# thomasdeppisch/eMagLS

Hardware: AMD Instinct MI355X
Metric: eMagLS filter sets/s (N=4, 2702 dirs, 512 taps) (higher is better)
Workload: dtype f64; 1 GPU; BASELINE config 3: getEMagLsFilters em32 r=4.2cm N=4 complex-SH, 2702 dirs, 512 taps, 48 kHz; one filter set per step, inputs resident in HBM; dirs=2702, taps=512, sim_order=19, bins=512, k_cut=43, designs_resident_per_gpu=128, designs_per_batch=32, batches_in_flight=4, distinct_hrir_sets_resident=20, parallelism=independent jobs per GPU, one RCCL gather

## Files before the change

emagls_amd/_lib.py:

```python
from __future__ import annotations

import ctypes as C
import os

_HERE = os.path.dirname(os.path.abspath(__file__))
LIB_PATH = os.environ.get("EMAGLS_LIB_PATH") or os.path.join(_HERE, "lib", "libemagls.so")

OK, ERR_ARG, ERR_UNSUPPORTED, ERR_HIP, ERR_NUMERIC = 0, 1, 2, 3, 4
BASIS = {"real": 0, "complex": 1}
KIND_LS, KIND_MAGLS, KIND_EMAGLS, KIND_EMAGLS2, KIND_FROM_ATF, KIND_EMA_CH, KIND_MAGLS_2D, KIND_EMA_SH = range(8)
RADIAL = {"tikhonov": 0, "softlimit": 1, "full": 2, "none": 3}
LAYOUT = {"sh": 0, "ch": 1}
MODEL = {"sh": 0, "emagls": 1, "emagls2": 2, "atf": 3, "ema_ch": 5, "ema_sh": 6}

c_dp = C.POINTER(C.c_double)
c_i64 = C.c_int64


class DesignDesc(C.Structure):
    _fields_ = [("kind", C.c_int), ("basis", C.c_int), ("order", C.c_int), ("fs", C.c_double), ("len", c_i64),
                ("nsamp", c_i64), ("ndirs", c_i64), ("mic_radius", C.c_double), ("nmics", c_i64),
                ("f_trans", C.c_double), ("atf_taps", c_i64), ("natf", c_i64), ("custom_basis", C.c_int),
                ("diffuseness", C.c_int), ("sim_order_pad", C.c_int)]

# ... 112 lines not shown
    "emagls_binaural_decode_render_fs_device": (C.c_int, [C.c_void_p, C.c_int, c_i64, c_i64, C.c_void_p, C.c_void_p, C.c_int, c_i64,
                                                          C.c_int, C.c_int, C.c_void_p, c_i64, C.c_void_p, c_i64, C.c_void_p, c_i64,
                                                          C.c_void_p, c_i64, C.c_double, C.c_double, C.c_double, C.c_void_p,
                                                          C.c_void_p, C.c_void_p]),
    "emagls_decode_stream_create": (C.c_int, [c_i64, C.c_void_p, C.c_void_p, C.c_int, c_i64, C.c_int, C.c_int, C.c_int, c_i64,
                                              C.POINTER(C.c_void_p)]),
    "emagls_decode_stream_push": (C.c_int, [C.c_void_p, C.c_void_p, c_i64, C.c_void_p, c_i64, C.c_void_p, c_i64, C.c_void_p, c_i64,
                                            C.c_void_p]),
    "emagls_decode_stream_push_device": (C.c_int, [C.c_void_p, C.c_void_p, c_i64, C.c_void_p, c_i64, C.c_void_p, c_i64, C.c_void_p, c_i64,
                                                   C.c_void_p, C.c_void_p]),
    "emagls_decode_stream_reset": (C.c_int, [C.c_void_p]),
    "emagls_decode_stream_info": (C.c_int, [C.c_void_p, C.POINTER(c_i64), C.POINTER(c_i64), C.POINTER(c_i64), C.POINTER(c_i64),
                                            C.POINTER(C.c_int)]),
    "emagls_decode_stream_destroy": (C.c_int, [C.c_void_p]),
    "emagls_decode_stream_create_bank": (C.c_int, [c_i64, c_i64, C.c_void_p, C.c_void_p, C.c_int, c_i64, C.c_int, C.c_int, C.c_int, c_i64,
                                                   C.POINTER(C.c_void_p)]),
    "emagls_decode_stream_push_sets": (C.c_int, [C.c_void_p, C.c_void_p, c_i64, C.c_void_p, c_i64, C.c_void_p, c_i64, C.c_void_p, c_i64,
                                                 C.c_void_p, c_i64, C.c_void_p]),
    "emagls_decode_stream_push_sets_device": (C.c_int, [C.c_void_p, C.c_void_p, c_i64, C.c_void_p, c_i64, C.c_void_p, c_i64, C.c_void_p,
                                                        c_i64, C.c_void_p, c_i64, C.c_void_p, C.c_void_p]),
    "emagls_decode_stream_sets": (C.c_int, [C.c_void_p, C.POINTER(c_i64)]),
    "emagls_decode_group_create": (C.c_int, [c_i64, c_i64, C.c_void_p, C.c_void_p, C.c_int, c_i64, C.c_int, C.c_int, C.c_int, c_i64, c_i64,
                                             C.POINTER(C.c_void_p)]),
    "emagls_decode_group_push": (C.c_int, [C.c_void_p, C.c_void_p, c_i64, C.c_void_p, c_i64, C.c_void_p, c_i64, C.c_void_p, c_i64,
                                           C.c_void_p, c_i64, C.c_void_p]),
    "emagls_decode_group_push_device": (C.c_int, [C.c_void_p, C.c_void_p, c_i64, C.c_void_p, c_i64, C.c_void_p, c_i64, C.c_void_p, c_i64,
                                                  C.c_void_p, c_i64, C.c_void_p, C.c_void_p]),
    "emagls_decode_group_reset": (C.c_int, [C.c_void_p, c_i64]),
    "emagls_decode_group_info": (C.c_int, [C.c_void_p, C.POINTER(c_i64), C.POINTER(c_i64), C.POINTER(c_i64), C.POINTER(c_i64),
                                           C.POINTER(c_i64), C.POINTER(C.c_int)]),
    "emagls_decode_group_destroy": (C.c_int, [C.c_void_p]),
    "emagls_decode_stream_create_encoded": (C.c_int, [c_i64, C.c_void_p, C.c_int, c_i64, c_i64, C.c_void_p, C.c_void_p, C.c_int, c_i64, C.c_int,
                                                      C.c_int, c_i64, C.POINTER(C.c_void_p)]),
    "emagls_decode_group_create_encoded": (C.c_int, [c_i64, C.c_void_p, C.c_int, c_i64, c_i64, C.c_void_p, C.c_void_p, C.c_int, c_i64, C.c_int,
                                                     C.c_int, c_i64, c_i64, C.POINTER(C.c_void_p)]),
    "emagls_field_stream_create": (C.c_int, [c_i64, c_i64, C.c_void_p, C.c_int, c_i64, c_i64, C.POINTER(C.c_void_p)]),
    "emagls_field_stream_push": (C.c_int, [C.c_void_p, C.c_void_p, c_i64, C.c_void_p]),
    "emagls_field_stream_push_device": (C.c_int, [C.c_void_p, C.c_void_p, c_i64, C.c_void_p, C.c_void_p]),
    "emagls_field_stream_reset": (C.c_int, [C.c_void_p]),
    "emagls_field_stream_info": (C.c_int, [C.c_void_p, C.POINTER(c_i64), C.POINTER(c_i64), C.POINTER(c_i64), C.POINTER(c_i64),
                                           C.POINTER(C.c_int)]),
    "emagls_field_stream_destroy": (C.c_int, [C.c_void_p]),
    "emagls_field_stream_create_bank": (C.c_int, [c_i64, c_i64, c_i64, C.c_void_p, C.c_int, c_i64, c_i64, C.POINTER(C.c_void_p)]),
    "emagls_field_stream_push_sets": (C.c_int, [C.c_void_p, C.c_void_p, c_i64, C.c_void_p, c_i64, C.c_void_p]),
    "emagls_field_stream_push_sets_device": (C.c_int, [C.c_void_p, C.c_void_p, c_i64, C.c_void_p, c_i64, C.c_void_p, C.c_void_p]),
    "emagls_field_stream_sets": (C.c_int, [C.c_void_p, C.POINTER(c_i64)]),
    "emagls_get_magls_filters_dc": (C.c_int, [C.c_void_p, C.c_void_p, c_i64, c_i64, C.c_void_p, C.c_void_p, C.c_int,
                                              C.c_double, c_i64, C.c_int, C.c_int, C.c_void_p, C.c_void_p]),
    "emagls_get_emagls_filters_dc": (C.c_int, [C.c_void_p, C.c_void_p, c_i64, c_i64, C.c_void_p, C.c_void_p, C.c_double,
                                               C.c_void_p, C.c_void_p, c_i64, C.c_int, C.c_double, c_i64, C.c_int, C.c_int,
                                               C.c_void_p, C.c_void_p]),
    "emagls_get_emagls2_filters_dc": (C.c_int, [C.c_void_p, C.c_void_p, c_i64, c_i64, C.c_void_p, C.c_void_p, C.c_double,
                                                C.c_void_p, C.c_void_p, c_i64, C.c_int, C.c_double, c_i64, C.c_int, C.c_int,
                                                C.c_void_p, C.c_void_p]),
    "emagls_get_magls_filters_2d": (C.c_int, [C.c_void_p, C.c_void_p, c_i64, c_i64, C.c_void_p, C.c_int, C.c_double, c_i64, C.c_int,
                                              C.c_void_p, C.c_void_p]),
    "emagls_get_radial_filter": (C.c_int, [C.c_int, C.c_double, C.c_double, c_i64, C.c_int, C.c_int, C.c_double, C.c_double, C.c_void_p]),
    "emagls_apply_radial_filter_rows": (c_i64, [c_i64, c_i64, C.c_int]),
    "emagls_apply_radial_filter": (C.c_int, [C.c_void_p, c_i64, C.c_int, C.c_double, C.c_double, c_i64, C.c_int, C.c_int, C.c_double,
                                             C.c_double, C.c_void_p]),
    "emagls_sh_encode": (C.c_int, [C.c_void_p, c_i64, c_i64, C.c_void_p, C.c_void_p, C.c_int, C.c_int, C.c_void_p]),
    "emagls_ch_basis": (C.c_int, [C.c_int, c_i64, C.c_void_p, C.c_int, C.c_void_p]),
    "emagls_get_smair_matrix": (C.c_int, [C.c_int, C.c_double, c_i64, C.c_int, C.c_double, C.c_void_p, C.c_void_p, c_i64, C.c_int, C.c_int,
                                          C.c_int, C.c_double, C.c_double, C.c_void_p, C.POINTER(C.c_int)]),
    "emagls_rendered_hrtfs": (C.c_int, [C.c_int, C.c_void_p, C.c_void_p, C.c_int, c_i64, c_i64, c_i64, C.c_void_p, C.c_void_p, c_i64, C.c_double,
                                        C.c_int, C.c_int, C.c_double, C.c_void_p, C.c_void_p, c_i64, C.c_void_p, c_i64, c_i64, C.c_void_p,
                                        C.c_void_p, c_i64, c_i64, C.c_void_p, C.c_void_p, C.c_void_p, C.c_void_p, C.c_void_p, C.c_void_p]),
    "emagls_array_irs": (C.c_int, [C.c_double, C.c_double, C.c_int, C.c_void_p, C.c_void_p, c_i64, C.c_void_p, C.c_int, c_i64, c_i64, C.c_void_p,
                                   C.c_void_p, C.c_void_p, C.c_void_p, C.c_void_p, C.c_double, c_i64, c_i64, C.c_void_p]),
    "emagls_array_irs_kernel_time": (C.c_int, [C.POINTER(C.c_double)]),
    "emagls_shoebox_components": (C.c_int, [C.c_void_p, C.c_void_p, C.c_void_p, c_i64, C.c_void_p, C.c_double, C.c_double, C.c_int, c_i64,
                                            C.c_void_p, C.c_void_p, C.c_void_p, C.c_void_p, C.c_void_p]),
    "emagls_array_room_irs": (C.c_int, [C.c_double, C.c_double, C.c_int, C.c_void_p, C.c_void_p, c_i64, C.c_void_p, C.c_int, c_i64, C.c_void_p,
                                        C.c_void_p, C.c_void_p, c_i64, C.c_void_p, C.c_double, C.c_int, C.c_double, c_i64, c_i64, C.c_void_p,
                                        C.c_void_p]),
    "emagls_shoebox_kernel_time": (C.c_int, [C.POINTER(C.c_double)]),
    "emagls_array_irs_spectral": (C.c_int, [C.c_double, C.c_double, C.c_int, C.c_void_p, C.c_void_p, c_i64, C.c_void_p, C.c_int, c_i64, c_i64,
                                            C.c_void_p, C.c_void_p, C.c_void_p, C.c_void_p, C.c_void_p, c_i64, C.c_void_p, C.c_void_p, C.c_void_p,
                                            C.c_void_p, C.c_double, c_i64, c_i64, C.c_void_p]),
    "emagls_shoebox_images": (C.c_int, [C.c_void_p, C.c_void_p, c_i64, C.c_void_p, C.c_double, C.c_double, C.c_int, c_i64, C.c_void_p,
                                        C.c_void_p, C.c_void_p, C.c_void_p, C.c_void_p, C.c_void_p, C.c_void_p]),
    "emagls_array_room_irs_spectral": (C.c_int, [C.c_double, C.c_double, C.c_int, C.c_void_p, C.c_void_p, c_i64, C.c_void_p, C.c_int, c_i64,
                                                 C.c_void_p, C.c_void_p, C.c_void_p, C.c_void_p, c_i64, C.c_void_p, C.c_double, C.c_int, C.c_double,
                                                 c_i64, c_i64, C.c_void_p, C.c_void_p]),
    "emagls_array_irs_point": (C.c_int, [C.c_double, C.c_double, C.c_int, C.c_void_p, C.c_void_p, c_i64, C.c_void_p, C.c_int, c_i64, c_i64,
                                         C.c_void_p, C.c_void_p, C.c_void_p, C.c_void_p, C.c_void_p, c_i64, C.c_void_p, C.c_void_p, C.c_void_p,
                                         C.c_void_p, C.c_void_p, C.c_double, c_i64, c_i64, C.c_void_p]),
    "emagls_shoebox_components_dist": (C.c_int, [C.c_void_p, C.c_void_p, C.c_void_p, c_i64, C.c_void_p, C.c_double, C.c_double, C.c_int, c_i64,
                                                 C.c_void_p, C.c_void_p, C.c_void_p, C.c_void_p, C.c_void_p, C.c_void_p]),
    "emagls_array_room_irs_point": (C.c_int, [C.c_double, C.c_double, C.c_int, C.c_void_p, C.c_void_p, c_i64, C.c_void_p, C.c_int, c_i64,
                                              C.c_void_p, C.c_void_p, C.c_int, C.c_void_p, C.c_void_p, c_i64, C.c_void_p, C.c_double, C.c_int,
                                              C.c_double, c_i64, c_i64, C.c_void_p, C.c_void_p]),
    "emagls_array_irs_directive": (C.c_int, [C.c_double, C.c_double, C.c_int, C.c_void_p, C.c_void_p, c_i64, C.c_void_p, C.c_int, c_i64, c_i64,
                                             C.c_void_p, C.c_void_p, C.c_void_p, C.c_void_p, C.c_void_p, c_i64, C.c_void_p, C.c_void_p, C.c_void_p,
                                             C.c_void_p, C.c_void_p, C.c_void_p, C.c_void_p, C.c_int, C.c_void_p, C.c_double, c_i64, c_i64,
                                             C.c_void_p]),
    "emagls_shoebox_emission": (C.c_int, [C.c_void_p, C.c_void_p, C.c_void_p, c_i64, C.c_void_p, C.c_double, C.c_double, C.c_int, c_i64,
                                          C.c_void_p, C.c_void_p]),
    "emagls_array_room_irs_directive": (C.c_int, [C.c_double, C.c_double, C.c_int, C.c_void_p, C.c_void_p, c_i64, C.c_void_p, C.c_int, c_i64,
                                                  C.c_void_p, C.c_void_p, C.c_int, C.c_void_p, C.c_void_p, c_i64, C.c_void_p, C.c_double, C.c_int,
                                                  C.c_int, C.c_void_p, C.c_int, C.c_void_p, C.c_double, c_i64, c_i64, C.c_void_p, C.c_void_p]),
    "emagls_eq_filter_nfft": (c_i64, [c_i64]),
    "emagls_get_magls_spherical_head_filter": (C.c_int, [C.c_double, C.c_int, C.c_double, c_i64, C.c_void_p, C.c_void_p]),
    "emagls_get_magls_array_diffuse_filter": (C.c_int, [C.c_double, C.c_void_p, C.c_void_p, c_i64, C.c_int, C.c_double, c_i64, C.c_int,
                                                        C.c_void_p, C.c_void_p]),
    "emagls_plan_create": (C.c_int, [C.POINTER(DesignDesc), C.POINTER(C.c_void_p)]),
    "emagls_plan_destroy": (C.c_int, [C.c_void_p]),
    "emagls_plan_set_hrir_grid": (C.c_int, [C.c_void_p, C.c_void_p, C.c_void_p]),
    "emagls_plan_set_mic_grid": (C.c_int, [C.c_void_p, C.c_void_p, C.c_void_p]),
    "emagls_plan_set_hrirs": (C.c_int, [C.c_void_p, C.c_void_p, C.c_void_p]),
    "emagls_plan_set_atfs": (C.c_int, [C.c_void_p, C.c_void_p, C.c_void_p, C.c_void_p]),
    "emagls_plan_execute": (C.c_int, [C.c_void_p]),
    "emagls_plan_synchronize": (C.c_int, [C.c_void_p]),
    "emagls_plan_get_filters": (C.c_int, [C.c_void_p, C.c_void_p, C.c_void_p]),
    "emagls_plan_get_info": (C.c_int, [C.c_void_p, C.POINTER(PlanInfo)]),
    "emagls_plan_sweep_form_in_batch": (C.c_int, [C.c_void_p, C.c_int, C.POINTER(C.c_int)]),
    "emagls_plan_set_profiling": (C.c_int, [C.c_void_p, C.c_int]),
    "emagls_plan_set_streams": (C.c_int, [C.c_void_p, C.c_int]),
    "emagls_plan_num_stages": (C.c_int, [C.c_void_p]),
    "emagls_plan_stage_name": (C.c_char_p, [C.c_void_p, C.c_int]),
    "emagls_plan_stage_times": (C.c_int, [C.c_void_p, c_dp, C.c_int]),
    "emagls_plan_sweep_kernel_time": (C.c_int, [C.c_void_p, c_dp, C.POINTER(C.c_int)]),
    "emagls_plan_debug_buffer": (C.c_int, [C.c_void_p, C.c_char_p, C.c_void_p, C.POINTER(C.c_size_t)]),
    "emagls_plan_stream": (C.c_void_p, [C.c_void_p]),
    "emagls_batch_create": (C.c_int, [C.POINTER(C.c_void_p), C.c_int, C.POINTER(C.c_void_p)]),
    "emagls_batch_execute": (C.c_int, [C.c_void_p]),
    "emagls_batch_synchronize": (C.c_int, [C.c_void_p]),
    "emagls_batch_get_filters": (C.c_int, [C.c_void_p, C.POINTER(C.c_void_p), C.POINTER(C.c_void_p)]),
    "emagls_batch_set_profiling": (C.c_int, [C.c_void_p, C.c_int]),
    "emagls_batch_lane_mode": (C.c_int, [C.c_void_p, C.POINTER(C.c_int)]),
    "emagls_batch_set_stream": (C.c_int, [C.c_void_p, C.c_void_p]),
    "emagls_set_batch_max": (C.c_int, [C.c_int, C.POINTER(C.c_int)]),
    "emagls_batch_shares_atf_side": (C.c_int, [C.c_void_p, C.POINTER(C.c_int)]),
    "emagls_design_hrir_sets": (C.c_int, [C.c_int, C.c_void_p, C.c_void_p, C.c_int64, C.c_int64, C.c_int64, C.c_void_p, C.c_void_p, C.c_double,
                                          C.c_void_p, C.c_void_p, C.c_int64, C.c_int, C.c_double, C.c_int64, C.c_int, C.c_void_p, C.c_void_p]),
    "emagls_from_atf_hrir_sets": (C.c_int, [C.c_void_p, C.c_void_p, C.c_int64, C.c_int64, C.c_int64, C.c_void_p, C.c_void_p, C.c_void_p, C.c_int64,
                                            C.c_int64, C.c_int64, C.c_void_p, C.c_void_p, C.c_double, C.c_int64, C.c_double, C.c_void_p, C.c_void_p,
                                            C.POINTER(C.c_double)]),
    "emagls_jobs_run": (C.c_int, [C.POINTER(Job), C.c_int64, C.c_int, C.c_int, C.c_int]),
    "emagls_design_out_shape": (C.c_int, [C.POINTER(DesignDesc), C.POINTER(c_i64), C.POINTER(c_i64), C.POINTER(C.c_int)]),
    "emagls_jobs_shard": (C.c_int, [C.POINTER(Job), C.c_int64, C.c_int, C.c_int, C.POINTER(C.c_int), C.POINTER(C.c_int), C.POINTER(C.c_int)]),
    "emagls_jobs_run_devices": (C.c_int, [C.POINTER(Job), C.c_int64, C.POINTER(C.c_int), C.c_int, C.c_int, C.c_int, C.c_int]),
    "emagls_jobs_set_profiling": (C.c_int, [C.c_int]),
    "emagls_jobs_sweep_times": (C.c_int, [C.POINTER(C.c_double), C.POINTER(C.c_int), C.c_int, C.POINTER(C.c_int)]),
    "emagls_batch_set_geometry_sharing": (C.c_int, [C.c_void_p, C.c_int]),
    "emagls_batch_shares_geometry": (C.c_int, [C.c_void_p, C.POINTER(C.c_int)]),
    "emagls_batch_geometry_runs": (C.c_int, [C.c_void_p, C.POINTER(C.c_longlong), C.POINTER(C.c_longlong)]),
    "emagls_jobs_geometry_runs": (C.c_int, [C.POINTER(C.c_longlong), C.POINTER(C.c_longlong), C.POINTER(C.c_longlong)]),
    "emagls_jobs_would_share_geometry": (C.c_int, [C.c_void_p, C.c_int, C.POINTER(C.c_int)]),
    "emagls_batch_set_side_stream": (C.c_int, [C.c_void_p, C.c_void_p]),
    "emagls_batch_set_streams": (C.c_int, [C.c_void_p, C.c_int]),
    "emagls_batch_set_stage_order": (C.c_int, [C.c_void_p, C.c_int]),
    "emagls_batch_sweep_time": (C.c_int, [C.c_void_p, C.POINTER(C.c_double)]),
    "emagls_batch_destroy": (C.c_int, [C.c_void_p]),
}


class EmaglsError(RuntimeError):
    def __init__(self, code, msg):
        super().__init__("emagls error %d: %s" % (code, msg))
        self.code = code


_lib = None


def load():
    global _lib
    if _lib is not None:
        return _lib
    if not os.path.exists(LIB_PATH):
        raise ImportError("HIP library not built: %s is missing (run `python -m emagls_amd.build`)" % LIB_PATH)
    lib = C.CDLL(LIB_PATH, mode=C.RTLD_GLOBAL)
    for name, (res, args) in SYMBOLS.items():
        fn = getattr(lib, name)
        fn.restype = res
        fn.argtypes = args
    _lib = lib
    return lib


def check(rc):
    if rc != OK:
        raise EmaglsError(rc, load().emagls_last_error().decode("utf-8", "replace"))
```

emagls_amd/csrc/batch_run.hip:

```cpp
#include "host_internal.hpp"

void emagls_batch_forget(emagls_batch* b, emagls_plan* p) {
    for (auto& q : b->plans) if (q == p) q = nullptr;
}

namespace {
void batch_sweep_stage(emagls_batch& b) {
    const int nb = (int)b.plans.size();
    std::vector<HalfSweepArgs> ha((size_t)nb);
    for (int j = 0; j < nb; ++j) ha[j] = emagls_half_args(*b.plans[j]);
    if (b.atf_share || b.geo_share)
        for (int j = 1; j < nb; ++j) {
            ha[j].G = ha[0].G; ha[j].Yri = ha[0].Yri; ha[j].Mw = ha[0].Mw; ha[j].cond_ok = ha[0].cond_ok;
            ha[j].bsc = ha[0].bsc; ha[j].smap = ha[0].smap;
            ha[j].skip_flag = ha[0].skip_flag;
        }
    const bool reg = b.plans[0]->sweep_persist && reg_sweep_wanted(b.plans.data(), nb);
    for (auto* q : b.plans) q->reg_sweep = reg;
    if (!reg && nb > SWEEP_MULTI_MAX) throw Error(EMAGLS_ERR_UNSUPPORTED, "internal: more than 16 designs in a batch need the register-resident sweep");
    HalfSweepMulti h{};
    h.n = std::min(nb, SWEEP_MULTI_MAX);
    for (int j = 0; j < h.n; ++j) h.a[j] = ha[j];
    emagls_plan& q0 = *b.plans[0];
    const int kk0 = std::max(q0.kcut0, 1);
    if (kk0 >= q0.P) return;
    if (q0.sweep_persist) {
        hipStream_t ss = b.stream;
        {
            SweepGate gate(ss, reg ? reg_sweep_gate_cost((int)q0.D, nb) : 0);
            if (b.lanes) { BatchScope sc(nb, b.stride); launch_zero(q0.get("ll"), q0.bufs["ll"].bytes, ss); }
            else for (auto* q : b.plans) launch_zero(q->get("ll"), q->bufs["ll"].bytes, ss);
            if (reg) {
                if (!b.sweep_args_dev.get()) b.sweep_args_dev.alloc(sizeof(HalfSweepArgs) * (size_t)REG_SWEEP_MAX);
                reg_args_upload(ha.data(), nb, b.sweep_args_dev.get(), b.sweep_args_last, ss);
            }
            if (b.prof_level >= 1) HIP_CHECK(hipEventRecord(b.sweep_ev[0], ss));
            if (reg) launch_sweep_reg(b.sweep_args_dev.get<const HalfSweepArgs>(), ha[0], nb, ss);
            else if (q0.synth) launch_sweep_synth(h, ss); else launch_sweep_persist(h, ss);
            if (b.prof_level >= 1) HIP_CHECK(hipEventRecord(b.sweep_ev[1], ss));
        }
        if (ss != b.stream) b.depend(b.stream, ss);
        return;
    }
    for (int kb = kk0; kb < q0.P; ++kb) launch_sweep_half(h, kb, b.stream);
    launch_sweep_half_finalize(h, q0.P - 1, b.stream);
}

bool batch_defers_hh(const emagls_batch& b) {
    if (!b.lanes || !(b.alone || sw_int<Sw::DEFER_HH>() == 2) || b.geo_share || b.atf_share) return false;
    for (const emagls_plan* p : b.plans) if (!p || !plan_defers_hh_route(*p)) return false;
    return true;
}
void batch_lanes_part(emagls_batch& b, int part, int first, int count, hipStream_t st, int group = 0) {
    emagls_plan& p0 = *b.plans[first];
    const int ns = (part == 0 && b.groups == 1) ? b.nstreams : 1;
    int order = 0;
    if (part == 0 && ns == 1 && sw_on<Sw::STAGGER>()) order = b.groups > 1 ? 1 + group % 2 : (b.order_hint ? 1 + (b.order_hint - 1) % 2 : 0);
    Scoped stream(p0.stream, st);
    Scoped nstreams(p0.nstreams, ns);
    Scoped stage_order(p0.stage_order, order);
    Scoped side0(p0.side[0], ns > 1 ? b.side[0] : p0.side[0]), side1(p0.side[1], ns > 1 ? b.side[1] : p0.side[1]),
        side2(p0.side[2], ns > 1 ? b.side[2] : p0.side[2]);
    Scoped pre_phase(p0.pre_phase, part == 3 ? 2 : (part == 0 && b.defer_hh) ? 1 : 0);
    BatchScope sc(count, b.stride);
    if (part == 0) plan_pre_stage(p0); else if (part == 3) emagls_pre_sweep(p0); else emagls_post_sweep(p0);
}
void mark_executed(emagls_batch& b, int launches) {
    for (auto* p : b.plans) { p->executed = true; p->sweep_launches = launches; }
}
int sweep_launch_count(const emagls_plan& p0) { return p0.sweep_persist ? 1 : p0.P - std::max(p0.kcut0, 1); }
int batch_group_first(const emagls_batch& b, int g) { const int n = (int)b.plans.size(), h = (n + b.groups - 1) / b.groups; return std::min(n, g * h); }
void batch_execute_lanes(emagls_batch& b) {
    const bool replay = b.use_graph && b.eager_runs >= 1 && !(b.groups == 1 && b.nstreams > 1);
    const int n = (int)b.plans.size();
    const int ng = b.groups;
    for (int g = 1; g < ng; ++g) if (!b.side[g - 1]) b.side[g - 1] = emagls::pool_stream_take();
    hipStream_t gs[4] = {b.stream, b.stream, b.stream, b.stream};
    for (int g = 1; g < ng; ++g) gs[g] = b.side[g - 1];
    if (!replay || !b.group[0]) b.defer_hh = batch_defers_hh(b);
    const bool defer = b.defer_hh;
    if (defer) for (int g = 0; g < ng; ++g) if (!b.hh_stream[g]) b.hh_stream[g] = emagls::pool_stream_take();
    if (replay && !b.group[0]) {
        for (int g = 0; g < ng; ++g) {
            const int f = batch_group_first(b, g), c = batch_group_first(b, g + 1) - f;
            b.group[g].capture(gs[g], [&] { batch_lanes_part(b, 0, f, c, gs[g], g); });
            if (defer) b.group_hh[g].capture(b.hh_stream[g], [&] { batch_lanes_part(b, 3, f, c, b.hh_stream[g], g); });
        }
        b.post.capture(b.stream, [&] { batch_lanes_part(b, 2, 0, n, b.stream); });
    }
    b.used = 0;
    for (int g = 1; g < ng; ++g) b.depend(gs[g], b.stream);
    if (replay && ng > 1) {
        hipError_t err[4] = {hipSuccess, hipSuccess, hipSuccess, hipSuccess};
        const int dev = b.device;
        std::vector<std::thread> th;
        for (int g = 1; g < ng; ++g)
            th.emplace_back([&, g] { err[g] = hipSetDevice(dev); if (err[g] == hipSuccess) err[g] = hipGraphLaunch(b.group[g].exec, gs[g]); });
        err[0] = hipGraphLaunch(b.group[0].exec, gs[0]);
        for (auto& t : th) t.join();
        for (int g = 0; g < ng; ++g) HIP_CHECK(err[g]);
    } else {
        for (int g = 0; g < ng; ++g) {
            const int f = batch_group_first(b, g), c = batch_group_first(b, g + 1) - f;
            if (replay) b.group[g].launch(gs[g]); else batch_lanes_part(b, 0, f, c, gs[g], g);
        }
    }
    if (defer) for (int g = 0; g < ng; ++g) b.depend(b.hh_stream[g], gs[g]);
    for (int g = 1; g < ng; ++g) b.depend(b.stream, gs[g]);
    batch_sweep_stage(b);
    if (defer) {
        for (int g = 0; g < ng; ++g) {
            const int f = batch_group_first(b, g), c = batch_group_first(b, g + 1) - f;
            if (replay) b.group_hh[g].launch(b.hh_stream[g]); else batch_lanes_part(b, 3, f, c, b.hh_stream[g], g);
            b.depend(b.stream, b.hh_stream[g]);
        }
    }
    if (replay) b.post.launch(b.stream); else batch_lanes_part(b, 2, 0, n, b.stream);
    mark_executed(b, sweep_launch_count(*b.plans[0]));
    if (!replay) ++b.eager_runs;
}

bool batch_inputs_same(emagls_batch& b, std::initializer_list<const char*> names, uint64_t& checked_version, bool& same) {
    uint64_t ver = 0;
    for (auto* p : b.plans) ver = ver * 1000003ull + p->atf_side_version;
    if (ver == checked_version) return same;
    if (!b.cmp_flag.get()) b.cmp_flag.alloc(16);
    HIP_CHECK(hipStreamSynchronize(b.stream));
    HIP_CHECK(hipMemsetAsync(b.cmp_flag.get(), 0, 16, b.stream));
    emagls_plan& p0 = *b.plans[0];
    for (size_t j = 1; j < b.plans.size(); ++j)
        for (const char* name : names) launch_compare_words(p0.get(name), b.plans[j]->get(name), p0.bufs[name].bytes, b.cmp_flag.get<int>(), b.stream);
    int differ = 0;
    HIP_CHECK(hipMemcpyAsync(&differ, b.cmp_flag.get(), sizeof differ, hipMemcpyDeviceToHost, b.stream));
    HIP_CHECK(hipStreamSynchronize(b.stream));
    checked_version = ver;
    return same = differ == 0;
}
void batch_set_sharing(emagls_batch& b, bool& field, bool share) {
    if (share == field) return;
    for (auto* p : b.plans) drop_plan_graphs(*p);
    drop_batch_graphs(b);
    if (&field == &b.geo_share || &field == &b.geo_ls_shared) batch_geo_forget(b);
    field = share;
}
void batch_run_two_graphs(emagls_batch& b, CapturedGraph& pre, void (*stage)(emagls_batch&, int), int pre_part, int launches) {
    const bool replay = b.use_graph && b.eager_runs >= 1;
    if (replay && !pre) pre.capture(b.stream, [&] { stage(b, pre_part); });
    if (replay && !b.post) b.post.capture(b.stream, [&] { stage(b, 2); });
    b.used = 0;
    if (replay) pre.launch(b.stream); else stage(b, pre_part);
    batch_sweep_stage(b);
    if (replay) b.post.launch(b.stream); else stage(b, 2);
    mark_executed(b, launches);
    if (!replay) ++b.eager_runs;
}
template <typename Pre> void batch_run_per_plan(emagls_batch& b, bool replay, Pre pre, void (*post)(emagls_plan&), int launches) {
    emagls_plan& p0 = *b.plans[0];
    if (replay && !p0.pre) {
        for (auto* p : b.plans) p->pre.capture(p->stream, [&] { pre(*p); });
        if (!p0.sweep_persist) b.group[0].capture(b.stream, [&] { batch_sweep_stage(b); });
    }
    b.used = 0;
    for (auto* p : b.plans) b.depend(p->stream, b.stream);
    for (auto* p : b.plans) {
        if (replay) p->pre.launch(p->stream); else pre(*p);
        b.depend(b.stream, p->stream);
    }
    if (b.atf_share)
        for (size_t j = 1; j < b.plans.size(); ++j) from_atf_ls_rows(*b.plans[j], p0, b.stream);
    if (p0.sweep_persist) batch_sweep_stage(b);
    else if (replay) b.group[0].launch(b.stream); else batch_sweep_stage(b);
    for (auto* p : b.plans) {
        b.depend(p->stream, b.stream);
        post(*p);
        b.depend(b.stream, p->stream);
    }
    mark_executed(b, launches);
    if (!replay) ++b.eager_runs;
}

void batch_atf_decide_sharing(emagls_batch& b) {
    const bool same = batch_inputs_same(b, {"atf", "atf_azi", "atf_zen", "hrir_azi", "hrir_zen"}, b.atf_checked_version, b.atf_inputs_same);
    bool routes_ok = true;
    for (auto* p : b.plans) routes_ok = routes_ok && p->gram_from == 1 && p->sweep_persist == b.plans[0]->sweep_persist;
    batch_set_sharing(b, b.atf_share, same && routes_ok && b.plans.size() > 1);
}
void from_atf_subject_pre_stage(emagls_plan& p) {
    subject_reset(p, p.stream);
    from_atf_subject_stage(p);
}
// ... 473 lines not shown
```

emagls_amd/csrc/capi.hip:

```cpp
#include "host_internal.hpp"

namespace {

struct CachedPlan {
    std::unique_ptr<emagls_plan> plan;
    emagls_design_desc desc{};
    int device = 0;
    bool busy = false;
    uint64_t last_use = 0;
};
std::mutex g_cache_mu;
std::vector<CachedPlan> g_cache;
uint64_t g_cache_tick = 0;

int one_shot(const emagls_design_desc& desc, const double* hL, const double* hR, const double* azi, const double* zen,
             const double* mic_azi, const double* mic_zen, const double* atf, const double* atf_azi, const double* atf_zen,
             void* wL, void* wR, double* mean_dev, const void* Y_hrir = nullptr, const void* Y_mic = nullptr) {
    return guarded([&] {
        int dev = 0;
        HIP_CHECK(hipGetDevice(&dev));
        emagls_plan* p = nullptr;
        std::unique_ptr<emagls_plan> fresh;
        bool cached = false;
        {
// ... 473 lines not shown
            if (!array_kind(p->d.kind) && p->d.kind != EMAGLS_KIND_FROM_ATF && !magls_kind(p->d.kind) && p->d.kind != EMAGLS_KIND_LS)
                throw Error(EMAGLS_ERR_UNSUPPORTED, "batches take eMagLS / eMagLS2 / EMAinCH / EMAinSH plans, LS / MagLS / MagLS-2D plans, or FromAtf plans "
                                                    "(subjects of one ATF set)");
            if ((p->d.kind == EMAGLS_KIND_LS) != (plans[0]->d.kind == EMAGLS_KIND_LS) ||
                (p->d.kind == EMAGLS_KIND_LS && (p->cplx_basis != plans[0]->cplx_basis || p->d.order != plans[0]->d.order || p->d.nsamp != plans[0]->d.nsamp)))
                throw Error(EMAGLS_ERR_ARG, "LS plans share a batch only with LS plans of the same order, basis and HRIR length");
            if ((p->d.kind == EMAGLS_KIND_FROM_ATF) != (plans[0]->d.kind == EMAGLS_KIND_FROM_ATF))
                throw Error(EMAGLS_ERR_ARG, "FromAtf plans cannot share a batch with array designs");
            if (magls_kind(p->d.kind) != magls_kind(plans[0]->d.kind) || (magls_kind(p->d.kind) && p->d.kind != plans[0]->d.kind))
                throw Error(EMAGLS_ERR_ARG, "MagLS plans share a batch only with MagLS plans of the same kind");
            if (magls_kind(p->d.kind) && (p->diffuse != plans[0]->diffuse || p->cplx_basis != plans[0]->cplx_basis || p->d.order != plans[0]->d.order))
                throw Error(EMAGLS_ERR_ARG, "all designs of a batch must have the same shape (order, basis, constraint)");
            if (p->wide) throw Error(EMAGLS_ERR_UNSUPPORTED, "designs with more than 32 channels run one at a time");
            if (p->owner) throw Error(EMAGLS_ERR_ARG, "a plan belongs to another batch (destroy that batch first)");
            if (p->device != plans[0]->device) throw Error(EMAGLS_ERR_ARG, "the plans of a batch must live on one device");
            for (int i = 0; i < j; ++i) if (plans[i] == p) throw Error(EMAGLS_ERR_ARG, "the same plan appears twice in the batch");
            const emagls_plan* q = plans[0];
            if (p->P != q->P || p->kcut0 != q->kcut0 || p->C != q->C || p->nWG_dense != q->nWG_dense || p->D != q->D || p->sweep_persist != q->sweep_persist ||
                p->Dm != q->Dm || p->d.natf != q->d.natf || p->d.atf_taps != q->d.atf_taps || p->d.len != q->d.len)
                throw Error(EMAGLS_ERR_ARG, "all designs of a batch must have the same shape (directions, channels, bins, k_cut)");
            b->plans.push_back(p);
        }
        b->device = b->plans[0]->device;
        DeviceGuard dg(b->device);
        b->stream = StreamPool::get().take();
        b->use_graph = !sw_on<Sw::NO_GRAPH>();
        const bool array_batch = b->plans[0]->d.kind != EMAGLS_KIND_FROM_ATF && !magls_kind(b->plans[0]->d.kind) && b->plans[0]->d.kind != EMAGLS_KIND_LS;
        for (auto* p : b->plans) HIP_CHECK(hipStreamSynchronize(p->stream));
        trace_mark("batch create: plans synchronised");
        if (array_batch) batch_unify_synth(*b);
        trace_mark("batch create: sweep form unified");
        batch_decide_residency(*b);
        trace_mark("batch create: residency decided");
        if (nplans > SWEEP_MULTI_MAX && !(b->plans[0]->synth && b->plans[0]->sweep_persist && reg_sweep_wanted(b->plans.data(), nplans)))
            throw Error(EMAGLS_ERR_UNSUPPORTED, "more than 16 designs per batch: only array designs that take the register-resident sweep (built-in SH basis, "
                                                "microphone grids set, at most 18 antipodal pairs + single microphones, a launch the device can hold)");
        for (auto* p : b->plans) {
            p->nstreams = 1;
            p->prof_level = 0;
            p->sync_stream = b->stream;
            p->owner = b.get();
        }
        b->atf = b->plans[0]->d.kind == EMAGLS_KIND_FROM_ATF;
        b->magls = magls_kind(b->plans[0]->d.kind) || b->plans[0]->d.kind == EMAGLS_KIND_LS;
        if (!b->atf && !b->magls) { batch_unify_synth(*b); batch_try_lanes(*b); }
        trace_mark("batch create: lanes tried");
        *batch = b.release();
    });
}
int emagls_batch_execute(emagls_batch* b) {
    return guarded([&] {
        DeviceGuard dg(b ? b->device : -1);
        if (!b) throw Error(EMAGLS_ERR_ARG, "null pointer");
        batch_execute(*b);
    });
}
int emagls_batch_synchronize(emagls_batch* b) {
    return guarded([&] {
        DeviceGuard dg(b ? b->device : -1);
        if (!b) throw Error(EMAGLS_ERR_ARG, "null pointer");
        HIP_CHECK(hipStreamSynchronize(b->stream));
    });
}
int emagls_batch_get_filters(emagls_batch* b, void* const* wL, void* const* wR) {
    return guarded([&] {
        DeviceGuard dg(b ? b->device : -1);
        if (!b || !wL || !wR) throw Error(EMAGLS_ERR_ARG, "null pointer");
        const size_t n = b->plans.size();
        for (size_t j = 0; j < n; ++j) {
            if (!wL[j] || !wR[j]) throw Error(EMAGLS_ERR_ARG, "null pointer");
            if (!b->plans[j]) throw Error(EMAGLS_ERR_ARG, "a plan of this batch has been destroyed");
            if (!b->plans[j]->executed) throw Error(EMAGLS_ERR_ARG, "batch has not been executed");
        }
        emagls_plan& p0 = *b->plans[0];
        const size_t bytes = (p0.out_cplx ? sizeof(cplx) : sizeof(double)) * (size_t)p0.out_rows * p0.out_cols;
        std::vector<int> flags(NFLAG * n, 0);
        for (int attempt = 0; attempt < 3; ++attempt) {
            if (b->lanes)
                HIP_CHECK(hipMemcpy2DAsync(flags.data(), NFLAG * sizeof(int), p0.get("flag"), b->stride, NFLAG * sizeof(int), n,
                                           hipMemcpyDeviceToHost, b->stream));
            else
                for (size_t j = 0; j < n; ++j)
                    HIP_CHECK(hipMemcpyAsync(&flags[NFLAG * j], b->plans[j]->get("flag"), NFLAG * sizeof(int), hipMemcpyDeviceToHost, b->stream));
            bool scattered = false;
            if (b->lanes && n <= 32 && bytes % 16 == 0) {
                bool dev_dst = true;
                for (size_t j = 0; j < n && dev_dst; ++j)
                    for (void* q : {wL[j], wR[j]}) {
                        hipPointerAttribute_t at{};
                        if (hipPointerGetAttributes(&at, q) != hipSuccess) { (void)hipGetLastError(); dev_dst = false; break; }
                        if (at.type != hipMemoryTypeDevice || at.device != b->device || ((uintptr_t)q & 15)) { dev_dst = false; break; }
                    }
                if (dev_dst) {
                    LanePtrs lp{};
                    for (size_t j = 0; j < n; ++j) { lp.p[2 * j] = wL[j]; lp.p[2 * j + 1] = wR[j]; }
                    launch_scatter_lanes(p0.get("wL"), p0.get("wR"), b->stride, bytes, (int)n, lp, b->stream);
                    scattered = true;
                }
            }
            if (!scattered)
                for (size_t j = 0; j < n; ++j) {
                    HIP_CHECK(hipMemcpyAsync(wL[j], b->plans[j]->get("wL"), bytes, hipMemcpyDefault, b->stream));
                    HIP_CHECK(hipMemcpyAsync(wR[j], b->plans[j]->get("wR"), bytes, hipMemcpyDefault, b->stream));
                }
            HIP_CHECK(hipStreamSynchronize(b->stream));
            bool redo = false;
            for (size_t j = 0; j < n; ++j) redo = plan_recover(*b->plans[j], &flags[NFLAG * j], false) || redo;
            if (!redo) break;
            batch_redo(*b, flags);
        }
        for (auto* q : b->plans)
            if (q->persist_suspended) { q->persist_suspended = false; q->sweep_persist = true; }
        for (size_t j = 0; j < n; ++j) throw_fatal_flags(&flags[NFLAG * j]);
        if (b->geo_cold_pending) { b->geo_kept_version = b->geo_ran_version; b->geo_cold_pending = false; }
    });
}
int emagls_batch_geometry_runs(emagls_batch* b, long long* cold, long long* warm) {
    return guarded([&] {
        if (!b || !cold || !warm) throw Error(EMAGLS_ERR_ARG, "null pointer");
        *cold = b->geo_cold_runs;
        *warm = b->geo_warm_runs;
    });
}
int emagls_batch_lane_mode(emagls_batch* b, int* lanes) {
    return guarded([&] {
        DeviceGuard dg(b ? b->device : -1);
        if (!b || !lanes) throw Error(EMAGLS_ERR_ARG, "null pointer");
        *lanes = b->lanes ? 1 : 0;
    });
}
int emagls_set_batch_max(int max_designs, int* previous) {
    return guarded([&] {
        if (max_designs < 1 || max_designs > REG_SWEEP_MAX) throw Error(EMAGLS_ERR_ARG, "a batch holds 1..32 designs (more than 16: array designs on the register-resident sweep)");
        const int prev = g_batch_max.exchange(max_designs);
        if (previous) *previous = prev;
    });
}
int emagls_batch_set_geometry_sharing(emagls_batch* b, int enable) {
    return guarded([&] {
        DeviceGuard dg(b ? b->device : -1);
        if (!b) throw Error(EMAGLS_ERR_ARG, "null pointer");
        HIP_CHECK(hipStreamSynchronize(b->stream));
        b->geo_want = enable != 0;
        b->geo_checked_version = ~0ull;
        batch_geo_forget(*b);
    });
}
int emagls_batch_shares_geometry(emagls_batch* b, int* shared) {
    return guarded([&] {
        if (!b || !shared) throw Error(EMAGLS_ERR_ARG, "null pointer");
        *shared = b->geo_share ? 1 : 0;
    });
}
int emagls_batch_shares_atf_side(emagls_batch* b, int* shared) {
    return guarded([&] {
        if (!b || !shared) throw Error(EMAGLS_ERR_ARG, "null pointer");
        *shared = b->atf_share ? 1 : 0;
    });
}
int emagls_batch_set_stream(emagls_batch* b, void* stream) {
    return guarded([&] {
        DeviceGuard dg(b ? b->device : -1);
        if (!b || !stream) throw Error(EMAGLS_ERR_ARG, "null pointer");
        HIP_CHECK(hipStreamSynchronize(b->stream));
        if (b->own_stream) emagls::pool_stream_give(b->stream);
        b->stream = (hipStream_t)stream;
        b->own_stream = false;
        for (auto* p : b->plans) if (p) p->sync_stream = b->stream;
    });
}
int emagls_batch_set_streams(emagls_batch* b, int nstreams) {
    return guarded([&] {
        DeviceGuard dg(b ? b->device : -1);
        if (!b) throw Error(EMAGLS_ERR_ARG, "null pointer");
        if (nstreams < 1 || nstreams > 4) throw Error(EMAGLS_ERR_ARG, "nstreams must be 1..4");
        HIP_CHECK(hipStreamSynchronize(b->stream));
        for (int i = 0; i < nstreams - 1; ++i) if (!b->side[i]) b->side[i] = emagls::pool_stream_take();
        if (nstreams != b->nstreams) drop_batch_graphs(*b);
        b->nstreams = nstreams;
    });
}
int emagls_batch_set_stage_order(emagls_batch* b, int order) {
    return guarded([&] {
        DeviceGuard dg(b ? b->device : -1);
        if (!b) throw Error(EMAGLS_ERR_ARG, "null pointer");
        if (order < 0 || order > 2) throw Error(EMAGLS_ERR_ARG, "stage order must be 0, 1 or 2");
        HIP_CHECK(hipStreamSynchronize(b->stream));
        if (order != b->order_hint) drop_batch_graphs(*b);
        b->order_hint = order;
    });
}
int emagls_batch_set_side_stream(emagls_batch* b, void* stream) {
    return guarded([&] {
        DeviceGuard dg(b ? b->device : -1);
        if (!b || !stream) throw Error(EMAGLS_ERR_ARG, "null pointer");
        HIP_CHECK(hipStreamSynchronize(b->stream));
        if (b->side[0] && !b->side0_external) { HIP_CHECK(hipStreamSynchronize(b->side[0])); emagls::pool_stream_give(b->side[0]); }
        b->side[0] = (hipStream_t)stream;
        b->side0_external = true;
    });
}
int emagls_batch_set_profiling(emagls_batch* b, int level) {
    return guarded([&] {
        DeviceGuard dg(b ? b->device : -1);
        if (!b) throw Error(EMAGLS_ERR_ARG, "null pointer");
        HIP_CHECK(hipStreamSynchronize(b->stream));
        if (level >= 1)
            for (auto& e : b->sweep_ev) if (!e) HIP_CHECK(hipEventCreate(&e));
        b->prof_level = level;
    });
}
int emagls_batch_sweep_time(emagls_batch* b, double* ms) {
    return guarded([&] {
        DeviceGuard dg(b ? b->device : -1);
        if (!b || !ms) throw Error(EMAGLS_ERR_ARG, "null pointer");
        if (b->prof_level < 1 || !b->sweep_ev[0]) throw Error(EMAGLS_ERR_ARG, "batch profiling is off");
        HIP_CHECK(hipStreamSynchronize(b->stream));
        float t = 0.f;
        HIP_CHECK(hipEventElapsedTime(&t, b->sweep_ev[0], b->sweep_ev[1]));
        *ms = t;
    });
}
int emagls_batch_destroy(emagls_batch* b) {
    return guarded([&] {
        DeviceGuard dg(b ? b->device : -1);
        delete b;
    });
}

int emagls_get_ls_filters(const double* hL, const double* hR, int64_t nsamp, int64_t ndirs, const double* azi,
                          const double* zen, int order, int basis, void* wL, void* wR) {
    emagls_design_desc d{};
    d.kind = EMAGLS_KIND_LS; d.basis = basis; d.order = order; d.nsamp = nsamp; d.ndirs = ndirs;
    return one_shot(d, hL, hR, azi, zen, nullptr, nullptr, nullptr, nullptr, nullptr, wL, wR, nullptr);
}
int emagls_get_magls_filters(const double* hL, const double* hR, int64_t nsamp, int64_t ndirs, const double* azi,
                             const double* zen, int order, double fs, int64_t len, int basis, void* wL, void* wR) {
    emagls_design_desc d{};
    d.kind = EMAGLS_KIND_MAGLS; d.basis = basis; d.order = order; d.fs = fs; d.len = len; d.nsamp = nsamp; d.ndirs = ndirs;
    return one_shot(d, hL, hR, azi, zen, nullptr, nullptr, nullptr, nullptr, nullptr, wL, wR, nullptr);
}
int emagls_get_emagls_filters(const double* hL, const double* hR, int64_t nsamp, int64_t ndirs, const double* azi,
                              const double* zen, double mic_radius, const double* mic_azi, const double* mic_zen,
                              int64_t nmics, int order, double fs, int64_t len, int basis, void* wL, void* wR) {
    emagls_design_desc d{};
    d.kind = EMAGLS_KIND_EMAGLS; d.basis = basis; d.order = order; d.fs = fs; d.len = len; d.nsamp = nsamp; d.ndirs = ndirs;
    d.mic_radius = mic_radius; d.nmics = nmics;
    if (!mic_azi || !mic_zen) { g_last_error = "null microphone grid"; return EMAGLS_ERR_ARG; }
    return one_shot(d, hL, hR, azi, zen, mic_azi, mic_zen, nullptr, nullptr, nullptr, wL, wR, nullptr);
}
int emagls_get_emagls2_filters(const double* hL, const double* hR, int64_t nsamp, int64_t ndirs, const double* azi,
                               const double* zen, double mic_radius, const double* mic_azi, const double* mic_zen,
                               int64_t nmics, int order, double fs, int64_t len, int basis, void* wL, void* wR) {
    emagls_design_desc d{};
    d.kind = EMAGLS_KIND_EMAGLS2; d.basis = basis; d.order = order; d.fs = fs; d.len = len; d.nsamp = nsamp; d.ndirs = ndirs;
    d.mic_radius = mic_radius; d.nmics = nmics;
    if (!mic_azi || !mic_zen) { g_last_error = "null microphone grid"; return EMAGLS_ERR_ARG; }
    return one_shot(d, hL, hR, azi, zen, mic_azi, mic_zen, nullptr, nullptr, nullptr, wL, wR, nullptr);
}
int emagls_get_emagls_filters_ema_in_ch(const double* hL, const double* hR, int64_t nsamp, int64_t ndirs, const double* azi,
                                        const double* zen, double mic_radius, const double* mic_azi, int64_t nmics, int order,
                                        double fs, int64_t len, int basis, void* wL, void* wR) {
    emagls_design_desc d{};
    d.kind = EMAGLS_KIND_EMA_CH; d.basis = basis; d.order = order; d.fs = fs; d.len = len; d.nsamp = nsamp; d.ndirs = ndirs;
    d.mic_radius = mic_radius; d.nmics = nmics;
    if (!mic_azi || nmics < 1) { g_last_error = "invalid array geometry"; return EMAGLS_ERR_ARG; }
    std::vector<double> mic_zen((size_t)nmics, kPi / 2.0);
    return one_shot(d, hL, hR, azi, zen, mic_azi, mic_zen.data(), nullptr, nullptr, nullptr, wL, wR, nullptr);
}
int emagls_get_emagls_filters_ema_in_sh(const double* hL, const double* hR, int64_t nsamp, int64_t ndirs, const double* azi,
                                        const double* zen, double mic_radius, const double* mic_azi, int64_t nmics, int order,
                                        double fs, int64_t len, int basis, void* wL, void* wR) {
    emagls_design_desc d{};
    d.kind = EMAGLS_KIND_EMA_SH; d.basis = basis; d.order = order; d.fs = fs; d.len = len; d.nsamp = nsamp; d.ndirs = ndirs;
    d.mic_radius = mic_radius; d.nmics = nmics;
    if (!mic_azi || nmics < 1) { g_last_error = "invalid array geometry"; return EMAGLS_ERR_ARG; }
    std::vector<double> mic_zen((size_t)nmics, kPi / 2.0);
    return one_shot(d, hL, hR, azi, zen, mic_azi, mic_zen.data(), nullptr, nullptr, nullptr, wL, wR, nullptr);
}
int emagls_get_emagls_filters_from_atf(const double* hL, const double* hR, int64_t nsamp, int64_t ndirs,
                                       const double* azi, const double* zen, const double* atf_irs, int64_t atf_taps,
                                       int64_t nmics, int64_t natf, const double* atf_azi, const double* atf_zen, double fs,
                                       int64_t filter_len, double f_trans, double* wL, double* wR, double* mean_dev) {
    emagls_design_desc d{};
    d.kind = EMAGLS_KIND_FROM_ATF; d.basis = EMAGLS_BASIS_REAL; d.fs = fs; d.len = filter_len; d.nsamp = nsamp; d.ndirs = ndirs;
    d.nmics = nmics; d.f_trans = f_trans; d.atf_taps = atf_taps; d.natf = natf;
    if (!atf_irs || !atf_azi || !atf_zen) { g_last_error = "null ATF set"; return EMAGLS_ERR_ARG; }
    return one_shot(d, hL, hR, azi, zen, nullptr, nullptr, atf_irs, atf_azi, atf_zen, wL, wR, mean_dev);
}

int emagls_get_magls_filters_dc(const double* hL, const double* hR, int64_t nsamp, int64_t ndirs, const double* azi, const double* zen,
                                int order, double fs, int64_t len, int apply_dc, int basis, void* wL, void* wR) {
    emagls_design_desc d{};
    d.kind = EMAGLS_KIND_MAGLS; d.basis = basis; d.order = order; d.fs = fs; d.len = len; d.nsamp = nsamp; d.ndirs = ndirs;
    d.diffuseness = apply_dc != 0;
    return one_shot(d, hL, hR, azi, zen, nullptr, nullptr, nullptr, nullptr, nullptr, wL, wR, nullptr);
}
static int emagls_array_dc(int kind, const double* hL, const double* hR, int64_t nsamp, int64_t ndirs, const double* azi, const double* zen,
                           double mic_radius, const double* mic_azi, const double* mic_zen, int64_t nmics, int order, double fs, int64_t len,
                           int apply_dc, int basis, void* wL, void* wR) {
    emagls_design_desc d{};
    d.kind = kind; d.basis = basis; d.order = order; d.fs = fs; d.len = len; d.nsamp = nsamp; d.ndirs = ndirs;
    d.mic_radius = mic_radius; d.nmics = nmics; d.diffuseness = apply_dc != 0;
    return one_shot(d, hL, hR, azi, zen, mic_azi, mic_zen, nullptr, nullptr, nullptr, wL, wR, nullptr);
}
int emagls_get_emagls_filters_dc(const double* hL, const double* hR, int64_t nsamp, int64_t ndirs, const double* azi, const double* zen,
// ... 74 lines not shown
```

emagls_amd/csrc/host_internal.hpp:

```cpp
#pragma once
#include <atomic>
#include <chrono>
#include <cstdlib>
#include <cstring>
#include <deque>
#include <map>
#include <memory>
#include <mutex>
#include <shared_mutex>
#include <string>
#include <thread>
#include <utility>
#include <vector>

#include "../../include/emagls.h"
#include "array_model.hpp"
#include "device_mem.hpp"
#include "kernels.hpp"

using namespace emagls;

struct emagls_batch;
void emagls_batch_forget(emagls_batch* b, emagls_plan* p);

// ... 208 lines not shown
    bool synth_want = false, synth = false;
    int synth_units = 0;
    bool reg_sweep = false;
    std::vector<char> sweep_args_last;
    bool synth_block = false;
    const emagls_plan* geo_from = nullptr;
    emagls_batch* owner = nullptr;
    bool have_hrir_grid = false, have_mic_grid = false, have_hrirs = false, have_atfs = false, have_basis = false;
    uint64_t atf_side_version = 0;
    bool diffuse = false;
    bool custom_basis = false;
    bool wide = false;
    int prof_level = 0;
    std::vector<std::string> stage_names;
    std::vector<hipEvent_t> stage_events;
    std::vector<double> stage_ms;
    std::vector<hipEvent_t> sweep_events;
    int sweep_launches = 0;
    bool executed = false;
    CapturedGraph graph;
    int eager_runs = 0;
    bool use_graph = true;
    CapturedGraph pre;
    int nstreams = 1;
    int stage_order = 0;
    int pre_phase = 0;
    bool geo_keep = false;
    bool geo_skip = false;
    uint64_t geo_done_version = ~0ull;
    uint64_t geo_run_version = ~0ull;
    uint64_t solo_runs = 0;
    bool defer_hh = false;
    bool alone = false;
    hipStream_t hh_stream = nullptr;
    hipStream_t sync_stream = nullptr;
    hipStream_t side[3] = {nullptr, nullptr, nullptr};
    bool owns_stream = true;
    void need_sides(int n) { for (int i = 0; i < n - 1 && i < 3; ++i) if (!side[i]) side[i] = StreamPool::get().take(); }
    std::vector<hipEvent_t> sync_events;
    size_t sync_used = 0;
    hipEvent_t next_sync_event() {
        if (sync_used == sync_events.size()) {
            hipEvent_t e;
            HIP_CHECK(hipEventCreateWithFlags(&e, hipEventDisableTiming));
            sync_events.push_back(e);
        }
        return sync_events[sync_used++];
    }
    void depend(hipStream_t waiter, hipStream_t signaller) {
        if (waiter == signaller) return;
        hipEvent_t e = next_sync_event();
        HIP_CHECK(hipEventRecord(e, signaller));
        HIP_CHECK(hipStreamWaitEvent(waiter, e, 0));
    }

    ~emagls_plan() {
        if (owner) emagls_batch_forget(owner, this);
        if (stream) hipStreamSynchronize(stream);
        for (auto st : side) if (st) hipStreamSynchronize(st);
        if (hh_stream) hipStreamSynchronize(hh_stream);
        (void)hipGetLastError();
        for (auto& kv : bufs) if (kv.second.p && kv.second.owned) hipFree(kv.second.p);
        release_slabs();
        for (auto e : stage_events) hipEventDestroy(e);
        for (auto e : sweep_events) hipEventDestroy(e);
        for (auto e : sync_events) hipEventDestroy(e);
        for (auto st : side) StreamPool::get().give(st);
        StreamPool::get().give(hh_stream);
        if (owns_stream) StreamPool::get().give(stream);
    }
    void* alloc(const std::string& name, size_t bytes, bool zero = true) {
        if (bytes == 0) bytes = 16;
        auto it = bufs.find(name);
        if (it != bufs.end()) {
            if (it->second.bytes >= bytes) {
                total_bytes -= (int64_t)(it->second.bytes - bytes);
                it->second.bytes = bytes;
                return it->second.p;
            }
            if (it->second.owned) HIP_CHECK(hipFree(it->second.p));
            total_bytes -= (int64_t)it->second.bytes;
        }
        DevBuf b;
        b.p = slab_take((bytes + 15) / 16 * 16);
        b.bytes = bytes;
        b.owned = false;
        if (zero && !slab_zeroed) HIP_CHECK(hipMemsetAsync(b.p, 0, bytes, stream));
        bufs[name] = b;
        total_bytes += (int64_t)bytes;
        return b.p;
    }
    template <typename T = void> T* get(const std::string& name) {
        auto it = bufs.find(name);
        if (it == bufs.end()) throw Error(EMAGLS_ERR_ARG, "internal: unknown buffer " + name);
        return reinterpret_cast<T*>(it->second.p);
    }
    bool has(const std::string& name) const { return bufs.count(name) != 0; }
    void upload(const std::string& name, const void* src, size_t bytes) {
        auto it = bufs.find(name);
        if (it == bufs.end() || it->second.bytes < bytes) throw Error(EMAGLS_ERR_ARG, "internal: upload size mismatch for " + name);
        HIP_CHECK(hipMemcpyAsync(it->second.p, src, bytes, hipMemcpyDefault, stream));
    }
    void mark(const char* name) {
        if (prof_level < 1) return;
        const size_t i = stage_names.size();
        stage_names.push_back(name);
        if (stage_events.size() <= i) {
            hipEvent_t e;
            HIP_CHECK(hipEventCreate(&e));
            stage_events.push_back(e);
        }
        HIP_CHECK(hipEventRecord(stage_events[i], stream));
    }
};

struct emagls_batch {
    std::vector<emagls_plan*> plans;
    int device = -1;
    bool lanes = false;
    size_t stride = 0;
    hipStream_t stream = nullptr;
    bool own_stream = true;
    bool atf = false, atf_share = false, atf_inputs_same = false;
    uint64_t atf_checked_version = ~0ull;
    bool magls = false;
    bool geo_want = false, geo_share = false, geo_inputs_same = false;
    uint64_t geo_checked_version = ~0ull;
    uint64_t geo_kept_version = ~0ull;
    uint64_t geo_ran_version = ~0ull;
    bool geo_cold_pending = false;
    CapturedGraph warm;
    int last_form = 0;
    long long geo_cold_runs = 0, geo_warm_runs = 0;
    bool geo_ls_shared = false;
    emagls::DevMem yls, zls;
    emagls::DevMem cmp_flag;
    int nstreams = 1;
    hipStream_t side[3] = {nullptr, nullptr, nullptr};
    CapturedGraph group[4];
    int prof_level = 0;
    hipEvent_t sweep_ev[2] = {nullptr, nullptr};
    CapturedGraph post;
    bool side0_external = false;
    int order_hint = 0;
    int groups = 1;
    CapturedGraph group_hh[4];
    hipStream_t hh_stream[4] = {nullptr, nullptr, nullptr, nullptr};
    bool defer_hh = false;
    bool alone = true;
    int eager_runs = 0;
    bool use_graph = true;
    emagls::DevMem sweep_args_dev;
    std::vector<char> sweep_args_last;
    std::vector<hipEvent_t> events;
    size_t used = 0;
    hipEvent_t next_event() {
        if (used == events.size()) {
            hipEvent_t e;
            HIP_CHECK(hipEventCreateWithFlags(&e, hipEventDisableTiming));
            events.push_back(e);
        }
        return events[used++];
    }
    void depend(hipStream_t waiter, hipStream_t signaller) {
        hipEvent_t e = next_event();
        HIP_CHECK(hipEventRecord(e, signaller));
        HIP_CHECK(hipStreamWaitEvent(waiter, e, 0));
    }
    ~emagls_batch() {
        if (stream) hipStreamSynchronize(stream);
        for (auto e : events) hipEventDestroy(e);
        for (int i = 0; i < 4; ++i)
            if (hh_stream[i]) { hipStreamSynchronize(hh_stream[i]); emagls::pool_stream_give(hh_stream[i]); }
        for (auto e : sweep_ev) if (e) hipEventDestroy(e);
        if (stream && own_stream) emagls::pool_stream_give(stream);
        for (int i = 0; i < 3; ++i) if (side[i] && !(i == 0 && side0_external)) { hipStreamSynchronize(side[i]); emagls::pool_stream_give(side[i]); }
        for (auto* p : plans) if (p) { p->sync_stream = nullptr; p->owner = nullptr; }
    }
};

namespace emagls {

struct StreamLoan {
    const std::vector<emagls_plan*>& plans;
    std::vector<hipStream_t> keep;
    StreamLoan(const std::vector<emagls_plan*>& ps, hipStream_t st) : plans(ps) {
        keep.reserve(ps.size());
        for (auto* p : ps) { keep.push_back(p->stream); p->stream = st; }
    }
    StreamLoan(const StreamLoan&) = delete;
    StreamLoan& operator=(const StreamLoan&) = delete;
    ~StreamLoan() { for (size_t j = 0; j < keep.size(); ++j) plans[j]->stream = keep[j]; }
};

template <typename F> int guarded(F&& f) {
    return guarded_call([&] { f(); });
}

constexpr double GRAM_COND_EST = 3.0e3;

inline bool forks_streams(const emagls_plan& p) { return p.nstreams >= 2; }

extern thread_local hipStream_t g_plan_stream_shared;
void plan_routes(emagls_plan& p);
void synth_pairing(const double* azi, const double* zen, int M, int* smap);
void plan_alloc_routes(emagls_plan& p);
void plan_setup(emagls_plan& p);

void stage_prologue(emagls_plan& p, int mode, const int64_t* didx, int64_t Dh);
void execute_ls(emagls_plan& p);
void magls_post_sweep(emagls_plan& p);
bool plan_defers_hh_route(const emagls_plan& p);
void hrir_spectra(emagls_plan& h, const emagls_plan& g, hipStream_t st, bool transposed = true);
FactorArgs hh_factor_args(emagls_plan& h, emagls_plan& g, int* sweeps_out, double* cond_ok);
void hrir_hh_rows(emagls_plan& h, emagls_plan& g, hipStream_t st);
void hrir_hh_back(const FactorArgs& fa, const emagls_plan& g, hipStream_t st);
void hrir_gram_ls_rows(emagls_plan& h, emagls_plan& g, const emagls_plan& src, bool lanes_share, hipStream_t st);
void subject_reset(emagls_plan& p, hipStream_t st);
void emagls_pre_sweep(emagls_plan& p);
HalfSweepArgs emagls_half_args(emagls_plan& p);
struct SweepGate {
    struct Entry { hipEvent_t ev; int slots; };
    struct State { std::deque<Entry> inflight; std::vector<hipEvent_t> pool; int capacity = 0; };
    static std::mutex& mutex();
    static State& state();
    std::unique_lock<std::mutex> lock;
    hipStream_t st;
    int slots;
    SweepGate(hipStream_t s, int slots_per_xcd);
    ~SweepGate();
};
bool reg_sweep_wanted(emagls_plan* const* plans, int n);
void reg_args_upload(const HalfSweepArgs* host, int n, void* dev, std::vector<char>& last, hipStream_t st);
void emagls_post_sweep(emagls_plan& p);
void from_atf_subject_stage(emagls_plan& p);
void from_atf_ls_rows(emagls_plan& p, emagls_plan& sh, hipStream_t st);
void from_atf_post_sweep(emagls_plan& p);
void plan_pre_stage(emagls_plan& p);
void plan_execute(emagls_plan& p);
void drop_plan_graphs(emagls_plan& p);
bool plan_recover(emagls_plan& p, const int* flag, bool apply);
void throw_fatal_flags(const int* flag);

void batch_geo_forget(emagls_batch& b);
bool batch_geo_next_is_warm(const emagls_batch& b);
void batch_execute(emagls_batch& b);
void drop_batch_graphs(emagls_batch& b);
void batch_unify_synth(emagls_batch& b);
void batch_decide_residency(emagls_batch& b);
void batch_try_lanes(emagls_batch& b);
void batch_redo(emagls_batch& b, const std::vector<int>& flags);
void plan_check_flags(emagls_plan& p);

bool same_desc(const emagls_design_desc& a, const emagls_design_desc& b);
extern thread_local int g_batch_max_override;

}
```

emagls_amd/csrc/kernels.hpp:

```cpp
#pragma once
#include <algorithm>
#include <functional>

#include "common.hpp"

namespace emagls {

void launch_zero(void* p, size_t bytes, hipStream_t st);
void launch_compare_words(const void* a, const void* b, size_t bytes, int* differ, hipStream_t st);
void launch_broadcast_lanes(const void* src, size_t bytes, size_t stride, int nlanes, hipStream_t st);
struct LanePtrs { void* p[64]; };
void launch_scatter_lanes(const void* srcL, const void* srcR, size_t stride, size_t bytes, int n, const LanePtrs& dst, hipStream_t st);
void launch_gather_buffers(const LanePtrs& src, const LanePtrs& dst, int nbuf, size_t bytes, hipStream_t st);
struct BufferMoves { const void* src[96]; void* dst[96]; size_t bytes[96]; int n; };
void launch_move_buffers(const BufferMoves& m, hipStream_t st);
void launch_ch_basis(int N, int M, const double* azi, bool cplx_basis, void* out, int ld, hipStream_t st, bool out_real = false);
void launch_sh_coeff(int N, double* tab, hipStream_t st);
inline size_t esz(bool c) { return c ? sizeof(cplx) : sizeof(double); }
inline size_t sh_coeff_count(int N) { return (size_t)2 * (N + 1) * (N + 1) + 2 * (N + 1); }
void launch_sh_basis(int N, int64_t D, const double* azi, const double* zen, const double* tab, bool cplx_basis,
                     void* Y, int64_t ld, hipStream_t st);
void launch_transpose_conj(const void* Y, int64_t D, int64_t S, int64_t ldY, void* Yt, int64_t Dpad, int64_t ldYt,
                           bool is_cplx, bool conj_it, hipStream_t st);

void launch_modal_bn(int N, int64_t nfreq, const double* kr, double kr_scale, double out_scale, void* bn,
                     int64_t stride_k, int64_t stride_n, hipStream_t st, const int* n_valid = nullptr);

void launch_twiddles(int nfft, void* tw, hipStream_t st);
int hrir_dirsum_chunks(int64_t D);
void launch_hrir_grpdelay(const double* hL, const double* hR, int64_t L, int64_t D, int nfft, const void* tw,
                          double* partial, double* grpd, hipStream_t st);
void launch_hrir_fft(const double* hL, const double* hR, int64_t L, int64_t D, const int64_t* didx, int nfft,
                     const void* tw, const double* grpd, int mode, int n_c, int kabs0, void* Hc, double* Habs,
                     int64_t ldD, hipStream_t st, double* HcT = nullptr, int ldT = 0);
void launch_real_fft_gather(const double* x, int64_t L, int64_t ncols, const int64_t* colidx, int nfft, const void* tw,
                            void* out, int64_t ldo, int64_t inner, int64_t ld_inner, hipStream_t st);
void launch_filter_epilogue(const void* W, int C, int nfft, int len, const void* tw, const double* grpd, int conj_mode,
                            int dc_rule, int shift_mode, int out_cplx, void* outL, void* outR, hipStream_t st, int n_ears = 2,
                            double fade_rel = 0.15);
void twiddles_debug(int nfft, void* tw);
void filter_epilogue_debug(const void* W, int C, int nfft, int len, const double* grpd, int conj_mode, int dc_rule, int shift_mode, int out_cplx,
                           int n_ears, double fade_rel, void* outL, void* outR);
void hrir_spectra_debug(const double* hL, const double* hR, int64_t L, int64_t D_src, int64_t D, const int64_t* didx, int nfft, int mode, int n_c, int kabs0,
                        const double* grpd_in, int64_t ldD, int ldT, double* grpd_out, void* phs, void* Hc, double* Habs, double* HcT);
void real_spectra_debug(const double* x, int64_t L, int64_t ncols_src, int64_t ncols, const int64_t* colidx, int nfft, int64_t ldo, int64_t inner,
                        int64_t ld_inner, void* out);

int gram_ksplit(int64_t D, int S);
int64_t gram_dpad(int64_t D, int S);
void launch_gram(const void* Yc, int64_t D, int S, int64_t ld, bool is_cplx, void* Gp, void* G, void* R, int Sh, hipStream_t st);
void launch_cholesky(void* G, int S, bool is_cplx, int* flag, hipStream_t st);
void launch_qform(const void* Yc, const void* R, void* Rinv, int S, int64_t D, int64_t ld, bool is_cplx, void* Q, hipStream_t st);
void launch_zsolve_flagged(void* Z, int ldS, const void* R, const void* Rinv, const double* cond_ok, int S, int C, int P, int k0,
                           hipStream_t st);
void launch_tn(const void* R, const void* E, int S, int C, int ldE, int nOrders, bool is_cplx, void* Tn, int64_t ldS,
               hipStream_t st);
void launch_small_gemm(const void* A, int lda, bool a_cplx, const void* B, int ldb, bool b_cplx, void* Cm, int ldc,
                       bool c_cplx, int M, int N, int K, hipStream_t st);

void launch_magls_m(const void* R, int C, bool is_cplx, int P, void* Mw, double* cond_ok, int* status, hipStream_t st);

struct FactorArgs;
void launch_factor(const FactorArgs& a, int nbins, bool tn_cplx, hipStream_t st, int phases = 3);
void launch_factor_jacobi_gram(const FactorArgs& a, int nbins, hipStream_t st);

void launch_gram_kmat(const void* Gy, const void* E, int S, int ldE, int C, int nOrd, bool is_cplx, void* F, int64_t ldF, double* Kmat, int ldK,
                      hipStream_t st);
void launch_gram_gemm(const void* bn, int nOrd, int P, int kb0, int nbins, double* Cf, int ldC, const double* Kmat, int ldK, int C, double* Apk,
                      int ldA, hipStream_t st);
void launch_gram_solve(const double* Apk, int ldA, int C, int kb0, int nbins, double reg_c, void* Mw, void* R2w, double* sv, int* route,
                       int* sweeps_out, hipStream_t st);
size_t hy_mfma_workspace_doubles(int n_c, int S, bool y_cplx);
int hy_mfma_kpad(int D);
void launch_hy_conj_mfma(const double* HcT, int ldT, int n_c, const void* Yc, int64_t ldY, bool y_cplx, int D, int S, double* Pw, void* out,
                         int ldS, hipStream_t st);
void launch_ls_gram(const void* Hc, int64_t ldH, int n_c, const void* G, int64_t g_stride, int64_t ldD, const void* Mw, int D, int C, int P,
                    int kb_lo, int kb_hi, void* W, hipStream_t st);

struct DenseSweepArgs;
struct HalfSweepArgs;
struct HalfSweepMulti;
void launch_sweep_dense(const DenseSweepArgs& a, int kb, bool x_cplx, hipStream_t st);
int dense_sweep_nwg(int D, int C);
void launch_sweep_half(const HalfSweepMulti& m, int kb, hipStream_t st);
void launch_sweep_half_finalize(const HalfSweepMulti& m, int kb_last, hipStream_t st);
int persist_sweep_nwg(int D);
bool persist_sweep_supported(int D, int C);
size_t persist_sweep_ll_bytes(int D, int C);
void launch_sweep_persist(const HalfSweepMulti& m, hipStream_t st);
int persist_sweep_dpw(int D);
int sweep_cu_budget();
bool persist_sweep_fits(int D, int C, int ndesigns);
bool synth_sweep_fits(int D, int nmics, int nOrd, int ndesigns);
bool synth_sweep_supported(int D, int nmics, int nOrd);
int synth_nord_pad(int nOrd);
void launch_synth_prepare(const void* bn, int nOrd, int P, void* bsc, const void* Zlo, int ldZ, int nOut, int M, const int* smap, double* Pm, hipStream_t st);
void launch_synth_mt(const void* Mw, const double* Pm, int nOut, int M, int k0, int P, const void* W, void* Mt, void* Winit, hipStream_t st);
void launch_synth_winit(const void* W, const void* Pm, int nOut, int M, int k0, int P, void* Winit, hipStream_t st, bool shared_geometry);
void launch_synth_rows(const void* U, int nchunks, const void* Pm, const void* Mw, int nOut, int M, int k_lo, int k_hi, int P, void* W, hipStream_t st,
                       bool shared_geometry = false);
int synth_ls_chunks(int D);
void launch_synth_ls(const void* Hc, int64_t ldH, int n_c, const void* bsc, int nord_pad, const double* dir_azi, const double* dir_zen, const double* mic_azi,
                     const double* mic_zen, const int* smap, int D, int M, int P, int kb_lo, int kb_hi, void* Upart, hipStream_t st, bool shared_geometry = false);
void launch_sweep_synth(const HalfSweepMulti& m, hipStream_t st);
void launch_yls_gram(const void* bsc, int nord_pad, const double* dir_azi, const double* dir_zen, const double* mic_azi, const double* mic_zen,
                     const int* smap, const double* Pm, const void* Mw, int D, int nOut, int kb_lo, int kb_hi, void* Yls, int64_t ldD, hipStream_t st);
void launch_ls_shared_rows(const void* Hc, int64_t ldH, int ls_end, const void* Yls, int64_t ldD, int D, int C, int P, void* W, hipStream_t st);
void synth_cosines_debug(const double* dir_azi, const double* dir_zen, int64_t ndirs, const double* mic_azi, const double* mic_zen, int nmics, double* x2);
void synth_operand_debug(const void* bsc, int nbins, int nord_pad, const double* x, int64_t nx, int gs, void* g_plus, void* g_minus);
int reg_sweep_max_units();
bool reg_sweep_supported(int D, int nmics, int nunits, int nOrd);
size_t reg_sweep_ll_bytes(int D, int nmics);
int reg_sweep_capacity(int D);
int reg_sweep_slots_per_xcd();
int reg_sweep_pick_waves(int D, int ndesigns);
int reg_sweep_gate_cost(int D, int ndesigns);
bool reg_sweep_fits(int D, int nmics, int nunits, int nOrd, int ndesigns);
void launch_sweep_reg(const HalfSweepArgs* args_dev, const HalfSweepArgs& a0, int n, hipStream_t st);
double reg_contract_selftest();
double gram_tile_selftest(bool four);
void store_sweep_args(const HalfSweepArgs* host, int n, HalfSweepArgs* dev, hipStream_t st);
void launch_sweep_finalize(const void* Wpart, void* W, int nWG, int C, int P, int kb_last, hipStream_t st);
void launch_hy_conj(const void* Hc, int64_t ldD, int nrows, const void* Yc, int64_t ldY, bool y_cplx, int D, int S, void* Pw, void* out,
                    int ldS, hipStream_t st);
size_t hy_workspace_elems(int nrows, int ldS);
void launch_ypinv(const void* Q, int64_t ldQ, bool q_cplx, const void* Zb, int ldS, int D, int S, int C, void* Ypinv,
                  int64_t ldD, hipStream_t st);
void launch_ls_apply(const void* Hc, int64_t ldH, int n_c, const void* Zf, bool z_cplx, int64_t ldD, int D, int C, int P,
                     int kb_lo, int kb_hi, void* W, hipStream_t st);
void launch_ls_filters(const double* hL, const double* hR, int64_t L, int D, const void* Yp, bool cplx_basis, int64_t ldD,
                       int C, void* wL, void* wR, hipStream_t st);
void launch_conj_copy(const void* in, void* out, int64_t n, bool is_cplx, hipStream_t st);
void launch_sh_rows_to_complex(void* W, int C, int nrows, int order, hipStream_t st);
void launch_widen(const void* in, int64_t ldi, bool in_cplx, void* out, int64_t ldo, int rows, int cols, bool transpose,
                  bool upper_only, hipStream_t st);

void launch_gram_inverse(const void* R, int S, bool is_cplx, void* M, int* status, hipStream_t st, void* work = nullptr);
void launch_ypinv_gram(const void* Ycm, int64_t ldD, bool is_cplx, const void* M, int S, int D, void* Ypinv, hipStream_t st);
void launch_sweep_wide(const DenseSweepArgs& a, int kb, bool x_cplx, hipStream_t st);
void launch_sweep_wide_finalize(const void* Wpart, void* W, int nWG, int C, int P, int kb_last, hipStream_t st);

void launch_wa_assemble(const void* Tn, const void* bn, int nOrd, int S, int C, int ldS, int P, int kb0, int nbins, void* B, hipStream_t st);
void launch_wa_factor(void* B, void* Vw, int S, int C, int ldS, int nbins, double reg_c, double* tauw, void* R2w, void* Nw, double* sv, int* sweeps,
                      void* Z, hipStream_t st);
struct WaTiling { int leaves, leaf_h, ldT; size_t off_stack, off_vt, off_zt, off_tau, bytes; };
WaTiling wa_tiling(int S, int C, int nbins);
void launch_wa_factor_tiled(void* B, void* Vw, int S, int C, int ldS, int nbins, double reg_c, double* tauw, void* R2w, void* Nw, double* sv,
                            int* sweeps, void* Z, void* ws, hipStream_t st);
void launch_wa_yri(const void* Q, int64_t ldQ, const void* Z, int S, int C, int ldS, int D, int64_t ldD, int nbins, void* Yri, hipStream_t st);
void launch_wa_ls(const void* Hc, int64_t ldH, int n_c, const void* Yri, int64_t ldD, int D, int C, int P, int kb_first, int kb_end, void* W, hipStream_t st);
void launch_wa_lo_gram(const void* Ycm, int M, int nOut, double* Ag, hipStream_t st);
void launch_wa_e(const void* Ycm, int M, int nOut, int S, const void* Minv, void* E, int ldE, hipStream_t st);

void launch_qt(const void* Yc, int64_t ldY, const void* E, int ldE, int D, int S, int C, int nOrders, bool is_cplx, void* QT,
               int64_t ldD, hipStream_t st);
void launch_dspace_g(const void* QT, int64_t ldD, bool is_cplx, const void* bn, int nOrders, int D, int C, int P, int k0, void* G,
                     hipStream_t st, int real_mode = 0, int sh_order = -1, int k_end = -1);
void launch_cond_flags(const double* sv, int C, int P, int hh_end, double* cond_ok, hipStream_t st);
void launch_yri_accurate(const void* Q, int64_t ldQ, bool is_cplx, const void* Z, int ldS, const double* cond_ok, int D, int S,
                         int C, int P, int k0, void* Yri, int64_t ldD, hipStream_t st, const void* Ycm = nullptr, int64_t ldYcm = 0);

void launch_grid_match(const double* aziA, const double* zenA, int64_t nA, const double* aziB, const double* zenB,
                       int64_t nB, double* cartB, int64_t* idx, double* dev_deg, double* mean_dev, hipStream_t st);
void launch_atf_colidx(const int64_t* idx, int64_t nA, int M, int64_t* colidx, hipStream_t st);

double measure_fp64_peak(int which, int reps, bool burst = false, double* mhz = nullptr);

void binaural_decode_real(const double* sig, int64_t n, int C, const double* wL, const double* wR, int64_t len,
                          double* out , hipStream_t st,
                          const cplx* sigc = nullptr );
bool decode_wave_form(int64_t len);
void binaural_decode_complex(const void* sig, bool sig_cplx, int64_t n, int C, const void* wL, const void* wR, bool w_cplx, int64_t len,
                             double* sig2, double* w2L, double* w2R, double* out, double* imag_abs, double* d_tmp, hipStream_t st,
                             int64_t imag_skip = 0 );
void decode_cache_clear();
void launch_abs_sum_cols(const double* x, int64_t n, int64_t skip, int ncols, double* out, hipStream_t st);

int rotate_order(int layout, int64_t C);
void launch_rotate_yaw(const void* in, bool in_cplx, int64_t n, int C, int layout, bool cplx_basis, const double* yaw, bool per_sample,
                       bool transpose, void* out, hipStream_t st, int64_t ld_in = 0, int64_t ld_out = 0, int L = 1, int64_t la = 0,
                       int64_t lo = 0);
int rotate3_max_order();
void launch_rotate3(const void* in, bool in_cplx, int64_t n, int C, bool cplx_basis, const double* yaw, bool yaw_ps, const double* pitch,
                    bool pitch_ps, const double* roll, bool roll_ps, bool transpose, void* out, hipStream_t st, int64_t ld_in = 0,
                    int64_t ld_out = 0, int L = 1, const int64_t* la = nullptr, int64_t lo = 0);
void launch_rotate3_matrix(int N, bool cplx_basis, double yaw, double pitch, double roll, void* out, hipStream_t st);
void rotate3_cache_clear();
struct EncodeBlock { const double* enc; bool enc_cplx; int M; const double* x; int64_t ldx; };
void launch_rotate_yaw_encoded(const EncodeBlock& e, int64_t n, int C, int layout, bool cplx_basis, const double* yaw, bool per_sample, void* out,
                               hipStream_t st, int64_t ld_out = 0, int L = 1, int64_t la = 0, int64_t lo = 0);
void launch_rotate3_encoded(const EncodeBlock& e, int64_t n, int C, bool cplx_basis, const double* yaw, bool yaw_ps, const double* pitch, bool pitch_ps,
                            const double* roll, bool roll_ps, void* out, hipStream_t st, int64_t ld_out = 0, int L = 1, const int64_t* la = nullptr,
                            int64_t lo = 0);
void launch_encode_block(const EncodeBlock& e, int64_t n, int C, void* out, int64_t ld_out, hipStream_t st);
constexpr int64_t kResampleMaxRatio = 65536;
int64_t resample_length(int64_t n, int64_t p, int64_t q);
void launch_resample(const void* in, bool cplx_in, int64_t n, int64_t nch, int64_t p, int64_t q, void* out, hipStream_t st);
void resample_cache_clear();

struct DecodeStreamState {
    int C = 0;
    bool planes2 = false;
    int B = 0, P = 0;
    int S = 1;
    int L = 1;
    cplx* Wf = nullptr;
    cplx* ring = nullptr;
    void* hist = nullptr;
    int* pos = nullptr;
};
bool decode_stream_block_ok(int64_t B);
void launch_decode_stream_filters(const double* wpl, int Cp, int64_t len, int B, int P, int64_t S, cplx* Wf, hipStream_t st);
void launch_partition_spectra(const double* wpl, int Cp, int64_t len, int B, int P, int64_t Z, cplx* Wf, hipStream_t st);
void launch_decode_stream_block(const DecodeStreamState& s, const void* x, bool x_cplx, int64_t ldx, const int* set, int standing, double* out,
                                int64_t ldo, hipStream_t st, int64_t lsx = 0, int lset = 0, int64_t lso = 0);

struct FieldStreamState {
    int nsrc = 0;
    int planes = 0;
    bool out_c = false;
    int B = 0, P = 0;
    cplx* Rf = nullptr;
    cplx* ring = nullptr;
    double* hist = nullptr;
    int* pos = nullptr;
    int S = 1;
    int* tag = nullptr;
    int* sel = nullptr;
};
constexpr int kFieldStreamEntries = 3;
constexpr int kFieldStreamMaxSources = 16;
void launch_field_stream_block(const FieldStreamState& s, const double* src, int64_t lds, const int* set, int64_t lset, void* out, int64_t ldo,
                               hipStream_t st);
constexpr int kFieldStreamLaunches = 2;

void decode_family_cache_clear();

void filter_channels_by_order(const double* sig, int64_t n_in, int64_t n, int C, const double* ir , int nOrd, int64_t len,
                              int64_t skip, double* out , hipStream_t st);

void launch_ema_sh_e0(const void* Ech, int ldS, const void* Ypts, int C, int S, bool cb, void* E0, hipStream_t st);
void launch_rot_points(const double* azi, const double* zen, int D, int npts, double* azr, double* znr, hipStream_t st);
void launch_rot_from_points(const void* A, int64_t ldA, const void* Z, int ldP, int C, int npts, const double* zen, int D, bool cb, void* Rot,
                            hipStream_t st);
void launch_qt_rotate(void* QT, int64_t ldD, int nOrd, int C, int N, int D, const void* Rot, bool cb, hipStream_t st);
void launch_gram_from_g(const void* G, int64_t g_stride, int64_t ldD, int D, int C, int kb0, int nbins, int g0, double* Apk, int ldK,
                        hipStream_t st);

void launch_radial_filter(const void* bn, int nOrd, int P, int type, double regul, double g, bool nyq_abs, bool zero_nan,
                          void* out_kn, void* out_cm, hipStream_t st);
void launch_diffuse_field(const void* bn, int nOrd, int n_lo, int P, double* df_hi, double* df_lo, hipStream_t st);
void launch_array_diffuse(const void* bn, int nOrd, const void* Y, bool y_cplx, int ldY, int S, int M, int nOut, int P,
                          double* df_lo, hipStream_t st);
void launch_eq_spectrum(const double* df_hi, const double* df_lo, const double* df_arr, int P, int mode, void* W, double* W_full,
                        hipStream_t st);
void launch_diffuse_constraint(void* W, const void* G, bool g_cplx, int64_t g_stride, int g0, const void* H, int D, int C, int64_t ldD,
                               int P, hipStream_t st);
void launch_smair(const void* E, bool e_cplx, int ldS, const void* bn, int nOrd, const void* rad, int nRad, int rows, int S, int P, void* out,
                  hipStream_t st);
void launch_sh_encode(const double* sig, int64_t n, int M, const void* Z, int ldZ, int nOut, bool out_cplx, void* out, hipStream_t st);

int rh_num_metrics();
int rh_bins_padded(int P);
int rh_gemm_tiles(int64_t D);
int rh_atf_tiles(int64_t D);
void launch_rh_split(const void* in, int64_t ncols, int64_t len, double* out, hipStream_t st);
void launch_rh_join(const void* F, int64_t n, void* W, hipStream_t st);
void launch_rh_modes(const void* W, int C, int P, int nsets, const void* A, bool a_cplx, int ldA, const void* bn, int nOrd, int S, bool y_cplx,
                     double* Tt, int64_t ldR, hipStream_t st);
void launch_rh_order_rows(const void* W, int C, int P, int nsets, const void* bn, int nOrd, bool q_cplx, double* Tt, int64_t ldR, hipStream_t st);
void launch_rh_interleave(const void* Y, int64_t ldi, int S, int64_t D, double* Yk, int64_t ldo, hipStream_t st);
// ... 76 lines not shown
```

emagls_amd/csrc/plan_run.hip:

```cpp
#include "host_internal.hpp"

namespace {
void stage_hrir_basis(emagls_plan& p) {
    hipStream_t st = p.stream;
    const bool cb = p.cplx_basis;
    if (p.d.kind == EMAGLS_KIND_MAGLS_2D) {
        launch_ch_basis(p.d.order, (int)p.D, p.get<double>("hrir_azi"), cb, p.get("Ycm"), (int)p.ldD, st, !cb);
    } else if (!p.custom_basis) {
        launch_sh_coeff(p.simOrder, p.get<double>("sh_tab"), st);
        launch_sh_basis(p.simOrder, p.D, p.get<double>("hrir_azi"), p.get<double>("hrir_zen"), p.get<double>("sh_tab"), cb,
                        p.get("Ycm"), p.ldD, st);
    }
    launch_transpose_conj(p.get("Ycm"), p.D, p.S, p.ldD, p.get("Yc"), p.Dpad, p.ldS, cb, true, st);
    p.mark("sh_basis");
    launch_gram(p.get("Yc"), p.D, p.S, p.ldS, cb, p.get("Gp"), nullptr, p.get("R"), p.S, st);
    p.mark("gram_mfma");
    launch_cholesky(p.get("R"), p.S, cb, p.get<int>("flag"), st);
    p.mark("cholesky");
    if (p.wide) return;
    launch_qform(p.get("Yc"), p.get("R"), p.get("Rinv"), p.S, p.D, p.ldS, cb, p.get("Q"), st);
    p.mark("qform");
}

void record_sweep_event(emagls_plan& p, size_t i) {
    if (p.sweep_events.size() <= i) {
        hipEvent_t e;
        HIP_CHECK(hipEventCreate(&e));
        p.sweep_events.push_back(e);
    }
    HIP_CHECK(hipEventRecord(p.sweep_events[i], p.stream));
}

PinvWs plan_pinv_ws(emagls_plan& p, const char* Xd, const char* Z, const char* Vws, const char* tauw, const char* R2w, const char* Nw) {
    return PinvWs{p.get<cplx>(Xd), p.get<cplx>(Z), p.get<cplx>(Vws), p.get<double>(tauw), p.get<cplx>(R2w), p.get<cplx>(Nw)};
}
PinvWs plan_lo_ws(emagls_plan& p) { return plan_pinv_ws(p, "Ylo_c", "Zlo", "Vlo", "tau_lo", "R2_lo", "N_lo"); }

void run_pinv_of_R(emagls_plan& p) {
    hipStream_t st = p.stream;
    const bool cb = p.cplx_basis;
    if (p.wide) {
        launch_gram_inverse(p.get("R"), p.S, cb, p.get("Mg"), p.get<int>("flag"), st, p.has("Mgw") ? p.get("Mgw") : nullptr);
        launch_ypinv_gram(p.get("Ycm"), p.ldD, cb, p.get("Mg"), p.S, (int)p.D, p.get("Ypinv"), st);
        p.mark("pinv");
        return;
    }
    launch_widen(p.get("R"), p.S, cb, p.get("Rb"), p.ldS, p.C, p.S, true, true, st);
    pinv_matrix(plan_pinv_ws(p, "Rb", "Zb", "Vws", "tauw", "R2w", "Nw"), p.S, p.C, p.ldS, (double)std::max<int64_t>(p.D, p.C), p.get<double>("sv"), st);
    launch_ypinv(p.get("Q"), p.ldS, cb, p.get("Zb"), p.ldS, (int)p.D, p.S, p.C, p.get("Ypinv"), p.ldD, st);
    p.mark("pinv");
}

void magls_pre_sweep(emagls_plan& p) {
    hipStream_t st = p.stream;
    const bool cb = p.cplx_basis;
    stage_hrir_basis(p);
    run_pinv_of_R(p);
    launch_conj_copy(p.get("Ycm"), p.get("Xc"), (int64_t)p.S * p.ldD, cb, st);
    stage_prologue(p, 0, nullptr, p.D);
    launch_ls_apply(p.get("Hc"), p.ldD, std::min(p.kcut0, p.P), p.get("Ypinv"), cb, p.ldD, (int)p.D, p.C, p.P, 0,
                    std::min(p.kcut0, p.P), p.get("W"), st);
    p.mark("ls_bins");
    if (p.sweep_persist) {
        launch_widen(p.get("Xc"), p.ldD, cb, p.get("Gm"), p.ldD, p.C, (int)p.D, false, false, st);
        launch_magls_m(p.get("R"), p.S, cb, p.P, p.get("Mw"), p.get<double>("cond_ok"), p.get<int>("flag"), st);
        p.mark("sweep_operands");
    }
}
void emagls_run_sweep(emagls_plan& p) {
    hipStream_t s0 = p.stream;
    const int k0 = std::max(p.kcut0, 1);
    HalfSweepMulti m{};
    m.n = 1;
    m.a[0] = emagls_half_args(p);
    p.sweep_launches = 0;
    if (k0 < p.P && p.sweep_persist) {
        emagls_plan* self = &p;
        p.reg_sweep = reg_sweep_wanted(&self, 1);
        SweepGate gate(s0, p.reg_sweep ? reg_sweep_gate_cost((int)p.D, 1) : 0);
        launch_zero(p.get("ll"), p.bufs["ll"].bytes, s0);
        if (p.reg_sweep) reg_args_upload(&m.a[0], 1, p.get("sweep_args"), p.sweep_args_last, s0);
        if (p.prof_level >= 2) record_sweep_event(p, 0);
        if (p.reg_sweep) launch_sweep_reg(p.get<HalfSweepArgs>("sweep_args"), m.a[0], 1, s0);
        else if (p.synth) launch_sweep_synth(m, s0); else launch_sweep_persist(m, s0);
        if (p.prof_level >= 2) record_sweep_event(p, 1);
        p.sweep_launches = 1;
    } else if (k0 < p.P) {
        for (int kb = k0; kb < p.P; ++kb) {
            if (p.prof_level >= 2) record_sweep_event(p, 2 * (size_t)p.sweep_launches);
            launch_sweep_half(m, kb, s0);
            if (p.prof_level >= 2) record_sweep_event(p, 2 * (size_t)p.sweep_launches + 1);
            ++p.sweep_launches;
        }
        launch_sweep_half_finalize(m, p.P - 1, s0);
    }
    p.mark("magls_sweep");
}
void execute_magls(emagls_plan& p) {
    hipStream_t st = p.stream;
    const bool cb = p.cplx_basis;
    magls_pre_sweep(p);
    if (p.sweep_persist) {
        emagls_run_sweep(p);
        magls_post_sweep(p);
        return;
    }
    DenseSweepArgs a{};
    a.D = (int)p.D; a.C = p.C; a.ldD = (int)p.ldD; a.P = p.P;
    a.X = p.get("Xc"); a.x_stride = 0; a.Zd = p.get("Ypinv"); a.z_stride = 0;
    a.Habs = p.get<double>("Habs"); a.ldH = p.ldD; a.kabs0 = p.kcut0;
    a.Wpart = p.get<cplx>("Wpart"); a.W = p.get<cplx>("W"); a.nWG = p.nWG; a.dpw = 0; a.kfirst = p.kcut0;
    p.sweep_launches = 0;
    for (int kb = p.kcut0; kb < p.P; ++kb) {
        if (p.prof_level >= 2) record_sweep_event(p, 2 * (size_t)p.sweep_launches);
        if (p.wide) launch_sweep_wide(a, kb, cb, st); else launch_sweep_dense(a, kb, cb, st);
        if (p.prof_level >= 2) record_sweep_event(p, 2 * (size_t)p.sweep_launches + 1);
        ++p.sweep_launches;
    }
    if (p.kcut0 < p.P) {
        if (p.wide) launch_sweep_wide_finalize(p.get("Wpart"), p.get("W"), p.nWG, p.C, p.P, p.P - 1, st);
        else launch_sweep_finalize(p.get("Wpart"), p.get("W"), p.nWG, p.C, p.P, p.P - 1, st);
    }
    p.mark("magls_sweep");
    magls_post_sweep(p);
}

int jacobi_run_length(const emagls_plan& p) {
    if (const int forced = sw_int<Sw::JACOBI_RUN>()) return forced;
    return (batch_ctx().n >= 2 && p.nstreams <= 1) ? 2 : 1;
}

void ema_sh_operands(emagls_plan& p) {
    const emagls_design_desc& d = p.d;
    const bool cb = p.cplx_basis;
    hipStream_t st = p.stream;
    const int M = (int)d.nmics, N = d.order, nOrd = p.simOrder + 1;
    const int ls_end = std::min(p.kcut0, p.P);
    p.sync_used = 0;
    launch_twiddles(p.nfft, p.get("tw"), st);
    launch_hrir_grpdelay(p.get<double>("hL"), p.get<double>("hR"), d.nsamp, d.ndirs, p.nfft, p.get("tw"), p.get<double>("dirsum"),
                         p.get<double>("grpd"), st);
    launch_hrir_fft(p.get<double>("hL"), p.get<double>("hR"), d.nsamp, p.D, nullptr, p.nfft, p.get("tw"), p.get<double>("grpd"), 0, ls_end,
                    p.kcut0, p.get("Hc"), p.get<double>("Habs"), p.ldD, st);
    if (p.diffuse)
        launch_hrir_fft(p.get<double>("hL"), p.get<double>("hR"), d.nsamp, p.D, nullptr, p.nfft, p.get("tw"), p.get<double>("grpd"), 0, p.P,
                        p.P, p.get("Hfull"), p.get<double>("Habs"), p.ldD, st);
    p.mark("hrir_prologue");
    launch_sh_coeff(p.simOrder, p.get<double>("sh_tab"), st);
    launch_sh_basis(p.simOrder, M, p.get<double>("mic_azi"), p.get<double>("mic_zen"), p.get<double>("sh_tab"), cb, p.get("Ymic_cm"), M, st);
    array_encoder(Encoder::CH_PINV, p.get("Ymic_cm"), M, p.S, p.ldS, cb, N, p.get<double>("mic_azi"), p.get("Ymic_rm"), plan_lo_ws(p), p.get("Ech"), st);
    ema_sh_e0(N, p.C, p.S, p.ldS, cb, p.get<double>("nnm_azi"), p.get<double>("nnm_zen"), p.get<double>("sh_tab_lo"), p.get("Ypts"), p.get("Ech"),
              p.get("E"), st);
    launch_modal_bn(p.simOrder, p.P, p.get<double>("kr"), 1.0, -1.0, p.get("bn"), nOrd, 1, st, p.get<int>("nvalid"));
    p.mark("array_model");
    {
        EmaShRot r{p.get<double>("rot_azi"), p.get<double>("rot_zen"), p.get("Arot"), plan_pinv_ws(p, "Bc", "Zb", "Vb", "tau_b", "R2_b", "N_b"),
                   p.get<double>("sv"), p.get<int>("jsweeps"), p.get("Rot")};
        ema_sh_rotations(r, N, p.C, (int)p.D, cb, p.get<double>("hrir_azi"), p.get<double>("hrir_zen"), p.get<double>("sh_tab_lo"), st);
    }
    p.mark("sh_rotations");
    ema_sh_order_terms(p.simOrder, N, (int)p.D, p.C, p.S, p.ldS, cb, p.get<double>("hrir_azi"), p.get<double>("hrir_zen_eq"), p.get<double>("sh_tab"),
                       p.get("Ycm"), p.ldD, p.get("Yc"), p.Dpad, p.get("E"), p.get("Rot"), p.get("QT"), st);
    launch_dspace_g(p.get("QT"), p.ldD, cb, p.get("bn"), nOrd, (int)p.D, p.C, p.P, p.g0, p.get("G"), st, 0, -1);
    p.mark("order_terms+G");
}
void ema_sh_pre_sweep(emagls_plan& p) {
    ema_sh_operands(p);
    const bool cb = p.cplx_basis;
    hipStream_t st = p.stream;
    const int ls_end = std::min(p.kcut0, p.P);
    const int64_t g_stride = (int64_t)p.C * p.ldD;
    (void)cb;
    const int ldK = round_up(p.C * p.C, 64), gf = 1, nb = p.P - 1;
    launch_gram_from_g(p.get("G"), g_stride, p.ldD, (int)p.D, p.C, gf, nb, p.g0, p.get<double>("Apk"), ldK, st);
    launch_gram_solve(p.get<double>("Apk"), ldK, p.C, gf, nb, SVD_REGUL_CONST, p.get("Mw"), p.get("R2w"), p.get<double>("sv"),
                      p.get<int>("route"), p.get<int>("jsweeps"), st);
    {
        FactorArgs fg{};
        fg.S = p.C; fg.C = p.C; fg.ldS = round_up(p.C, 64); fg.kb0 = gf; fg.P = p.P;
        fg.reg_mode = 0; fg.reg_c = SVD_REGUL_CONST;
        fg.sv = p.get<double>("sv"); fg.route = p.get<int>("route"); fg.status = p.get<int>("flag");
        fg.cond_limit = 10.0 * GRAM_COND_EST;
        fg.sweeps_out = p.get<int>("jsweeps");
        fg.tauw = p.get<double>("tauw"); fg.R2w = p.get<cplx>("R2w"); fg.Nw = p.get<cplx>("Nw"); fg.Mw = p.get<cplx>("Mw");
        fg.jrun = jacobi_run_length(p);
        launch_factor_jacobi_gram(fg, nb, st);
    }
    launch_cond_flags(p.get<double>("sv"), p.C, p.P, 1, p.get<double>("cond_ok"), st);
    p.mark("gram_route");
    if (ls_end > 1)
        launch_ls_gram(p.get("Hc"), p.ldD, ls_end, (const cplx*)p.get("G") - (int64_t)p.g0 * g_stride, g_stride, p.ldD, p.get("Mw"), (int)p.D, p.C,
                       p.P, 1, ls_end, p.get("W"), st);
    p.mark("ls_bins");
}

void execute_ema_sh_wide(emagls_plan& p) {
    hipStream_t st = p.stream;
    const int nb = p.P - 1, ls_end = std::min(p.kcut0, p.P), k0 = std::max(p.kcut0, 1);
    const int64_t g_stride = (int64_t)p.C * p.ldD;
    ema_sh_operands(p);
    cplx* G = p.get<cplx>("G");
    cplx* Yri = p.get<cplx>("Yri");
    HIP_CHECK(hipMemcpyAsync(p.get("Bw"), G, sizeof(cplx) * (size_t)nb * g_stride, hipMemcpyDeviceToDevice, st));
    launch_wa_factor(p.get("Bw"), p.get("Vw"), (int)p.D, p.C, (int)p.ldD, nb, SVD_REGUL_CONST, p.get<double>("tauw"), p.get("R2w"), p.get("Nw"),
                     p.get<double>("sv") + p.C, p.get<int>("jsweeps") + 1, Yri, st);
    p.mark("factor_bins");
    launch_wa_ls(p.get("Hc"), p.ldD, ls_end, Yri, p.ldD, (int)p.D, p.C, p.P, 1, ls_end, p.get("W"), st);
    p.mark("ls_bins");
    DenseSweepArgs a{};
    a.D = (int)p.D; a.C = p.C; a.ldD = (int)p.ldD; a.P = p.P;
    a.X = G - g_stride; a.x_stride = g_stride;
    a.Zd = Yri - g_stride; a.z_stride = g_stride;
    a.Habs = p.get<double>("Habs"); a.ldH = p.ldD; a.kabs0 = p.kcut0;
    a.Wpart = p.get<cplx>("Wpart"); a.W = p.get<cplx>("W"); a.nWG = p.nWG; a.dpw = 0; a.kfirst = k0;
    p.sweep_launches = 0;
    for (int kb = k0; kb < p.P; ++kb) { launch_sweep_wide(a, kb, true, st); ++p.sweep_launches; }
    if (k0 < p.P) launch_sweep_wide_finalize(p.get("Wpart"), p.get("W"), p.nWG, p.C, p.P, p.P - 1, st);
    p.mark("magls_sweep");
    launch_filter_epilogue(p.get("W"), p.C, p.nfft, (int)p.d.len, p.get("tw"), p.get<double>("grpd"), p.req_cplx ? 1 : 0, 1, 0,
                           p.out_cplx ? 1 : 0, p.get("wL"), p.get("wR"), st);
    p.mark("epilogue");
}

void execute_emagls_wide(emagls_plan& p) {
    if (p.d.kind == EMAGLS_KIND_EMA_SH) { execute_ema_sh_wide(p); return; }
    const emagls_design_desc& d = p.d;
    hipStream_t st = p.stream;
    const bool raw = d.kind == EMAGLS_KIND_EMAGLS2;
    const int M = (int)d.nmics, nOrd = p.simOrder + 1, nb = p.P - 1;
    const int ls_end = std::min(p.kcut0, p.P), k0 = std::max(p.kcut0, 1);
    const int64_t g_stride = (int64_t)p.C * p.ldD;
    const bool geo = !p.geo_skip;
    if (geo) {
    launch_sh_coeff(p.simOrder, p.get<double>("sh_tab"), st);
    launch_sh_basis(p.simOrder, p.D, p.get<double>("hrir_azi"), p.get<double>("hrir_zen"), p.get<double>("sh_tab"), false, p.get("Ycm"), p.ldD, st);
    launch_transpose_conj(p.get("Ycm"), p.D, p.S, p.ldD, p.get("Yc"), p.Dpad, p.ldS, false, true, st);
// ... 766 lines not shown
```

emagls_amd/csrc/sweep_reg.hip:

```cpp
#include "device_mem.hpp"
#include "persist_common.hpp"
#include "synth_common.hpp"

#include <algorithm>
#include <map>
#include <mutex>

namespace emagls {

namespace {

constexpr int RG_MLD = 36;

constexpr int DPP_ROR4 = 0x124, DPP_ROR8 = 0x128;
__device__ __forceinline__ int rg_slot_set(int i, int x) { return i < 4 ? 0 : i < 8 ? 1 : x >> 1; }
__device__ __forceinline__ int rg_slot_unit(int i, int x) { return i < 8 ? 4 * (i & 3) + x : 16 + (x & 1); }

template <int NUL>
__device__ __forceinline__ void rg_contract(const cplx (&E)[NUL], const cplx (&O)[NUL], const cplx (&ts)[2], int lane, bool slot8, double* wp) {
    static_assert(NUL == 9, "quad layout of 18 units");
    const int x = lane & 3;
    double ar[2], ai[2];
#pragma unroll
    for (int s = 0; s < 2; ++s) { ar[s] = (x & 1) ? ts[s].y : ts[s].x; ai[s] = (x & 1) ? -ts[s].x : ts[s].y; }
    double aE[5], aO[5];
#pragma unroll
    for (int r = 0; r < 5; ++r) { aE[r] = 0.0; aO[r] = 0.0; }
#pragma unroll
    for (int s = 0; s < 2; ++s)
#pragma unroll
        for (int c = 0; c < 2; ++c) {
            const double a = c ? ai[s] : ar[s];
#pragma unroll
            for (int r = 0; r < 4; ++r) {
                aE[r] = __builtin_amdgcn_mfma_f64_4x4x4f64(a, c ? E[4 * s + r].y : E[4 * s + r].x, aE[r], 0, 0, 0);
                aO[r] = __builtin_amdgcn_mfma_f64_4x4x4f64(a, c ? O[4 * s + r].y : O[4 * s + r].x, aO[r], 0, 0, 0);
            }
        }
    if (slot8) {
#pragma unroll
        for (int s = 0; s < 2; ++s) {
            const bool mine = (x >> 1) == s;
#pragma unroll
            for (int c = 0; c < 2; ++c) {
                const double a = c ? ai[s] : ar[s];
                aE[4] = __builtin_amdgcn_mfma_f64_4x4x4f64(a, mine ? (c ? E[8].y : E[8].x) : 0.0, aE[4], 0, 0, 0);
                aO[4] = __builtin_amdgcn_mfma_f64_4x4x4f64(a, mine ? (c ? O[8].y : O[8].x) : 0.0, aO[4], 0, 0, 0);
            }
        }
    }
    const int nacc = slot8 ? 5 : 4;
#pragma unroll
    for (int r = 0; r < 5; ++r) {
        if (r >= nacc) break;
        aE[r] += dpp_d<DPP_ROR4>(aE[r]); aE[r] += dpp_d<DPP_ROR8>(aE[r]);
        aO[r] += dpp_d<DPP_ROR4>(aO[r]); aO[r] += dpp_d<DPP_ROR8>(aO[r]);
    }
    if (slot8) { aE[4] += dpp_d<DPP_XOR2>(aE[4]); aO[4] += dpp_d<DPP_XOR2>(aO[4]); }
    if ((lane & 12) == 0) {
        const int y = lane >> 4;
#pragma unroll
        for (int r = 0; r < 4; ++r) { wp[8 * (4 * r + x) + y] = aE[r]; wp[8 * (4 * r + x) + 4 + y] = aO[r]; }
        if (slot8 && x < 2) { wp[8 * (16 + x) + y] = aE[4]; wp[8 * (16 + x) + 4 + y] = aO[4]; }
    }
}

template <int U0, int GS, int NUL, int NT>
__device__ __forceinline__ void synth_units(const double* xcol, cplx (&E)[NUL], cplx (&O)[NUL], const cplx* bs, int nord_pad) {
    double x2[GS], pa[GS], pb[GS];
#pragma unroll
    for (int i = 0; i < GS; ++i) x2[i] = xcol[(U0 + i) * NT];
#pragma unroll
    for (int i = 0; i < GS; ++i) { pa[i] = 1.0; pb[i] = 0.5 * x2[i]; E[U0 + i] = mk(0.0, 0.0); O[U0 + i] = mk(0.0, 0.0); }
    const unsigned bs0 = lds_addr(bs);
    d2_t b0, b1, c0, c1;
    auto request = [&](int n, d2_t& q0, d2_t& q1) __attribute__((always_inline)) {
        const int nn = n < nord_pad ? n : nord_pad - 2;
        lds_read16_async(q0, bs0 + 16 * nn, pa[0]); lds_read16_async(q1, bs0 + 16 * nn + 16, pa[0]);
    };
    auto pass = [&](const d2_t& q0, const d2_t& q1) __attribute__((always_inline)) {
#pragma unroll
        for (int i = 0; i < GS; ++i) {
            E[U0 + i].x = fma(q0.x, pa[i], E[U0 + i].x); E[U0 + i].y = fma(q0.y, pa[i], E[U0 + i].y);
            O[U0 + i].x = fma(q1.x, pb[i], O[U0 + i].x); O[U0 + i].y = fma(q1.y, pb[i], O[U0 + i].y);
            pa[i] = fma(x2[i], pb[i], -pa[i]);
            pb[i] = fma(x2[i], pa[i], -pb[i]);
        }
    };
    request(0, b0, b1);
    lds_wait2(b0, b1, pa[0]);
    for (int n = 0; n < nord_pad; n += 4) {
        request(n + 2, c0, c1);
        pass(b0, b1);
        lds_wait2(c0, c1, pb[GS - 1]);
        if (n + 2 >= nord_pad) break;
        request(n + 4, b0, b1);
        pass(c0, c1);
        lds_wait2(b0, b1, pb[GS - 1]);
    }
}

__device__ __forceinline__ int launder(int v) { asm volatile("" : "+v"(v)); return v; }

#define RG_GLOBAL(T, p) ((T __attribute__((address_space(1)))*)(p))
typedef const double __attribute__((address_space(1)))* gcd_t;
typedef const cplx __attribute__((address_space(1)))* gcc_t;
typedef u64 __attribute__((address_space(1)))* gu64_t;
typedef unsigned u32x4_t __attribute__((ext_vector_type(4)));
__device__ __forceinline__ cplx ldg(gcc_t p) { return mk(p->x, p->y); }
__device__ __forceinline__ u64 gll_load(gu64_t p) { return __hip_atomic_load(p, __ATOMIC_RELAXED, __HIP_MEMORY_SCOPE_AGENT); }
__device__ __forceinline__ void gll_put(gu64_t dst, u64 word, bool local) {
    if (local) __hip_atomic_store(dst, word, __ATOMIC_RELAXED, __HIP_MEMORY_SCOPE_WORKGROUP);
    else __hip_atomic_store(dst, word, __ATOMIC_RELAXED, __HIP_MEMORY_SCOPE_AGENT);
}
__device__ __forceinline__ void gll_load16_async(u32x4_t& out, gu64_t p) { asm volatile("global_load_dwordx4 %0, %1, off sc1" : "=v"(out) : "v"(p) : "memory"); }

constexpr int RG_POLL = 12;
__device__ __forceinline__ void rg_wait_loads(u32x4_t (&g)[RG_POLL]) {
    asm volatile("s_waitcnt vmcnt(0)" : "+v"(g[0]), "+v"(g[1]), "+v"(g[2]), "+v"(g[3]), "+v"(g[4]), "+v"(g[5]), "+v"(g[6]), "+v"(g[7]), "+v"(g[8]), "+v"(g[9]),
                 "+v"(g[10]), "+v"(g[11]) :: "memory");
}
constexpr int RG_NUL = 9;
constexpr int RG_NEX = 4 * PS_CMAX;
constexpr int RG_SVC = 256;

template <int NUL, int NW>
__global__ void __launch_bounds__(64 * NW) __attribute__((amdgpu_waves_per_eu(3))) sweep_reg_kernel(const HalfSweepArgs* __restrict__ args, int n, int nWG, int spread, int prio) {
    constexpr int NT = 64 * NW, DPW = 32 * NW;
    constexpr int NU2 = 2 * NUL;
    constexpr int NVW = 8 * NU2;
    constexpr int GA = (NUL + 1) / 2, GB = NUL - GA;
    static_assert(GB >= 1 && NW % 2 == 0 && NT >= RG_SVC, "layout");
    extern __shared__ __attribute__((aligned(16))) char dyn[];
    cplx* ring = reinterpret_cast<cplx*>(dyn);
    cplx* ms = ring + 2 * SY_NORD;
    cplx* WE = ms + PS_CMAX * RG_MLD;
    cplx* WO = WE + 2 * NU2;
    double* vt = reinterpret_cast<double*>(WO + 2 * NU2);
    double* wpart = vt + 2 * RG_NEX;
    double* xs = wpart + NW * NVW;
    __shared__ int s_abort, s_local;

    int design, member;
    if (spread) {
        design = (int)blockIdx.x / nWG;
        member = (int)blockIdx.x - design * nWG;
    } else {
        const int xcd = blockIdx.x & 7, rest = blockIdx.x >> 3;
        const int sub = rest / nWG;
        member = rest - sub * nWG;
        design = xcd + 8 * sub;
    }
    if (design >= n) return;
    if (prio) __builtin_amdgcn_s_setprio(3);
    const HalfSweepArgs& a = args[design];
    const int tid = threadIdx.x;
    const int C = a.C, P = a.P, D = a.D, kfirst = a.kfirst, kabs0 = a.kabs0;
    const int64_t ldH = a.ldH;
    const int nord_pad = a.nord_pad;
    const gcd_t Habs = RG_GLOBAL(const double, a.Habs);
    const gcc_t Mw = RG_GLOBAL(const cplx, a.Mw);
    const gcc_t bsc = RG_GLOBAL(const cplx, a.bsc);
    const gcd_t Winit = RG_GLOBAL(const double, a.Winit);
    cplx __attribute__((address_space(1)))* const Uout = RG_GLOBAL(cplx, a.U);
    long long* const timing = a.timing;
    int* const abort_flag = a.abort_flag;
    const long long wait_ticks = a.wait_ticks;
    const int* smap = a.smap;
    const int npr = smap[32], nsg = smap[33], nun = npr + nsg;
    const gu64_t part_ll = RG_GLOBAL(u64, a.ll);
    const gu64_t xcc_ll = part_ll + (size_t)2 * nWG * RG_NEX * 2;
    if (tid == 0) { s_abort = 0; s_local = 0; }
    const int d0 = member * DPW;
    auto dir_of = [&](int t, int s) __attribute__((always_inline)) { return d0 + 32 * (t >> 6) + 16 * s + ((t & 63) >> 2); };

    {
        const size_t ncplx = (size_t)2 * SY_NORD + PS_CMAX * RG_MLD + 4 * NU2;
        for (size_t i = tid; i < ncplx; i += NT) ring[i] = mk(0, 0);
        for (int i = tid; i < 2 * RG_NEX + NW * NVW; i += NT) vt[i] = 0.0;
        double sd[2], cd[2], daz[2];
#pragma unroll
        for (int s = 0; s < 2; ++s) {
            const int dgi = dir_of(tid, s) < D ? dir_of(tid, s) : D - 1;
            synth_zen(a.dir_zen[dgi], sd[s], cd[s]);
            daz[s] = a.dir_azi[dgi];
        }
#pragma unroll 1
        for (int i = 0; i < NUL; ++i) {
            const int u = rg_slot_unit(i, tid & 3), s = rg_slot_set(i, tid & 3);
            double v = 0.0;
            if (u < nun) {
                const int jm = smap[u < npr ? 2 * u : 2 * npr + (u - npr)];
                double sm, cm;
                synth_zen(a.mic_zen ? a.mic_zen[jm] : 1.5707963267948966, sm, cm);
                v = synth_x2(s ? sd[1] : sd[0], s ? cd[1] : cd[0], sm, cm, (s ? daz[1] : daz[0]) - a.mic_azi[jm]);
            }
            xs[i * NT + tid] = v;
        }
    }
    __syncthreads();

    if (tid < nord_pad) {
        ring[(kfirst & 1) * SY_NORD + tid] = ldg(bsc + (int64_t)kfirst * nord_pad + tid);
        const int k1 = kfirst + 1 < P ? kfirst + 1 : P - 1;
        ring[((kfirst + 1) & 1) * SY_NORD + tid] = ldg(bsc + (int64_t)k1 * nord_pad + tid);
    }
    constexpr int NLM = 4;
    cplx mReg[NLM];
    auto fetch_m = [&](int kbm, int t) __attribute__((always_inline)) {
        const int r = t >> 3, c0 = (t & 7) * 4;
        const gcc_t M = Mw + (int64_t)kbm * C * C + r * C + c0;
#pragma unroll
        for (int i = 0; i < NLM; ++i) mReg[i] = ldg(M + i);
    };
    auto stage_m = [&](int t) __attribute__((always_inline)) {
        const int r = t >> 3, c0 = (t & 7) * 4;
#pragma unroll
        for (int i = 0; i < NLM; ++i) ms[r * RG_MLD + c0 + i] = (r < C && c0 + i < C) ? mReg[i] : mk(0, 0);
    };
    double hCur[2], hNext[2] = {0.0, 0.0};
    auto fetch_h = [&](int kb, double (&h)[2], int t) __attribute__((always_inline)) {
        const int kbg = (kb < P ? kb : P - 1) - kabs0;
        const gcd_t He = Habs + ((int64_t)((t >> 1) & 1) * (P - kabs0) + kbg) * ldH;
#pragma unroll
        for (int s = 0; s < 2; ++s) h[s] = He[dir_of(t, s) < D ? dir_of(t, s) : D - 1];
    };
    fetch_h(kfirst, hCur, tid);
    if (tid < RG_SVC) { fetch_m(kfirst, tid); stage_m(tid); }

    if (tid < 64) {
        const int lane = tid;
        const unsigned xcc = read_xcc_id();
        const unsigned tag0 = 0x58434300u;
        if (lane == 0) gll_put(xcc_ll + member, ((u64)tag0 << 32) | xcc, false);
        bool alive = true, same = true;
        for (int base = 0; base < nWG && alive; base += 64) {
            u64 w = 0;
            alive = ll_wait([&] {
                if (base + lane >= nWG) return true;
                w = gll_load(xcc_ll + base + lane);
                return ll_ok(w, tag0);
            }, abort_flag, wait_ticks);
            same = same && __builtin_amdgcn_ballot_w64(base + lane < nWG && (unsigned)w != xcc) == 0;
        }
        if (lane == 0) {
            s_local = alive && same && a.force_global == 0;
            if (!alive) s_abort = 1;
            if (timing && member == 1) timing[15] = s_local;
        }
    }
    __syncthreads();
    const bool local = s_local != 0;
    if (s_abort) return;

    const bool slot8 = nun > 16 || GB < 2;
    cplx E[NUL], O[NUL];
#pragma unroll
    for (int u = 0; u < NUL; ++u) { E[u] = mk(0, 0); O[u] = mk(0, 0); }

#define RSTAMP(i) do { if (timing && member == 1 && tid == 0 && kb < P) timing[(int64_t)kb * 16 + (i)] = (long long)wall_clock64(); } while (0)
    for (int kb = kfirst; kb <= P; ++kb) {
        const bool first = (kb == kfirst);
        const bool last = (kb == P);
        const bool nyq = (kb == P - 1);
        RSTAMP(7);
        if (!last) {
            const cplx* bs = ring + (kb & 1) * SY_NORD;
            const double* xcol = xs + launder(tid);
            synth_units<0, GA, NUL, NT>(xcol, E, O, bs, nord_pad);
            __builtin_amdgcn_sched_barrier(0);
            if (slot8) synth_units<GA, GB, NUL, NT>(xcol, E, O, bs, nord_pad);
            else synth_units<GA, GB - 1, NUL, NT>(xcol, E, O, bs, nord_pad);
            __builtin_amdgcn_sched_barrier(0);
        }
        RSTAMP(0);
        if (launder(tid) < RG_SVC) {
            const int t = launder(tid);
            const int j = t & (RG_NEX - 1), half = t >> 7;
            if (first) {
                vt[t] = half == 0 ? Winit[j] : 0.0;
            } else {
                const unsigned tag = (unsigned)(kb - 1);
                const gu64_t src = part_ll + ((size_t)((kb - 1) & 1) * nWG * RG_NEX + j) * 2;
                double sum = 0.0;
                const bool alive = ll_wait([&] {
                    bool ok = true;
                    double s = 0.0;
                    for (int base = half; base < nWG; base += 2 * RG_POLL) {
                        u32x4_t g[RG_POLL];
#pragma unroll
                        for (int i = 0; i < RG_POLL; ++i) {
                            const int w = base + 2 * i < nWG ? base + 2 * i : half;
                            gll_load16_async(g[i], src + (size_t)w * RG_NEX * 2);
                        }
                        rg_wait_loads(g);
#pragma unroll
                        for (int i = 0; i < RG_POLL; ++i) {
                            ok = ok && g[i].y == tag && g[i].w == tag;
                            if (base + 2 * i < nWG) s += __hiloint2double((int)g[i].z, (int)g[i].x);
                        }
                    }
                    sum = s;
                    return ok;
                }, abort_flag, wait_ticks);
                vt[t] = sum;
                if (!alive && (t & 63) == 0) s_abort = 1;
            }
        }
        RSTAMP(2);
        __syncthreads();
        if (s_abort) break;
        if (launder(tid) < RG_SVC) {
            const int t = launder(tid);
            const int part = t & 3, pair = t >> 2, e = pair >> 5, c = pair & 31;
            const cplx* vc = reinterpret_cast<const cplx*>(vt) + e * PS_CMAX;
            cplx acc = mk(0, 0);
            if (first) {
                if (part == 0) acc = vc[c];
            } else {
#pragma unroll
                for (int i = 0; i < PS_CMAX / 4; ++i)
                    cfma(acc, vc[part + 4 * i] + vc[RG_NEX / 2 + part + 4 * i], conj(ms[(part + 4 * i) * RG_MLD + c]));
            }
            acc = group_sum<4>(acc);
            const cplx other = shfl_xor_c(acc, 4);
            if (part == 0 && c < C) {
                if (c < 2 * npr) {
                    if ((c & 1) == 0) { WE[e * NU2 + (c >> 1)] = acc + other; WO[e * NU2 + (c >> 1)] = acc - other; }
                } else {
                    WE[e * NU2 + npr + (c - 2 * npr)] = acc; WO[e * NU2 + npr + (c - 2 * npr)] = acc;
                }
                if (member == 0 && !first) {
                    cplx __attribute__((address_space(1)))* dst = Uout + ((int64_t)e * P + (kb - 1)) * PS_CMAX + c;
                    const cplx v = vc[c] + vc[RG_NEX / 2 + c];
                    dst->x = v.x; dst->y = v.y;
                }
            }
        }
        if (last) break;
        __syncthreads();
        RSTAMP(3);
        const bool svc = launder(tid) < RG_SVC;
        if (svc) fetch_m(kb, launder(tid));
        cplx ts[2];
        {
            const int t = launder(tid);
            const int x = t & 3;
            cplx p[2][2];
#pragma unroll
            for (int s = 0; s < 2; ++s) { p[s][0] = mk(0, 0); p[s][1] = mk(0, 0); }
#pragma unroll
            for (int r = 0; r < 4; ++r) {
                const int u = 4 * r + x;
                const cplx we0 = WE[u], wo0 = WO[u], we1 = WE[NU2 + u], wo1 = WO[NU2 + u];
#pragma unroll
                for (int s = 0; s < 2; ++s) {
                    cfma(p[s][0], we0, E[4 * s + r]); cfma(p[s][0], wo0, O[4 * s + r]);
                    cfma(p[s][1], we1, E[4 * s + r]); cfma(p[s][1], wo1, O[4 * s + r]);
                }
            }
            if (slot8) {
                const int u = 16 + (x & 1);
                cplx q0 = mk(0, 0), q1 = mk(0, 0);
                cfma(q0, WE[u], E[8]); cfma(q0, WO[u], O[8]);
                cfma(q1, WE[NU2 + u], E[8]); cfma(q1, WO[NU2 + u], O[8]);
                const bool s1 = (x & 2) != 0;
                const cplx z = mk(0, 0);
                p[0][0] = p[0][0] + (s1 ? z : q0); p[0][1] = p[0][1] + (s1 ? z : q1);
                p[1][0] = p[1][0] + (s1 ? q0 : z); p[1][1] = p[1][1] + (s1 ? q1 : z);
            }
            if (svc) stage_m(t);
            RSTAMP(8);
#pragma unroll
            for (int s = 0; s < 2; ++s) {
                const cplx pe0 = group_sum<4>(p[s][0]), pe1 = group_sum<4>(p[s][1]);
                const cplx pe = (x & 2) ? pe1 : pe0;
                ts[s] = dir_of(t, s) < D ? unit_phase(hCur[s], pe, nyq) : mk(0, 0);
            }
        }
        __builtin_amdgcn_sched_barrier(0);
        {
            const int t = launder(tid);
            rg_contract<NUL>(E, O, ts, t & 63, slot8, wpart + (t >> 6) * NVW);
        }
        {
            const int t = launder(tid);
            fetch_h(kb + 1, hNext, t);
            if (t < nord_pad) ring[(kb & 1) * SY_NORD + t] = ldg(bsc + (int64_t)(kb + 2 < P ? kb + 2 : P - 1) * nord_pad + t);
        }
        __syncthreads();
        RSTAMP(4);
        if (launder(tid) < RG_NEX) {
            const int t = launder(tid);
            const int xe = t >> 6, xr = (t >> 1) & 31, xri = t & 1;
            double v = 0.0;
            if (xr < C) {
                const int xu = xr < 2 * npr ? (xr >> 1) : npr + (xr - 2 * npr);
                const bool xneg = xr < 2 * npr && (xr & 1);
                const double* wE = wpart + 8 * xu + 2 * xe + xri;
                double sE = 0.0, sO = 0.0;
#pragma unroll
                for (int w = 0; w < NW; ++w) { sE += wE[w * NVW]; sO += wE[w * NVW + 4]; }
                v = xneg ? sE - sO : sE + sO;
            }
            const gu64_t dst = part_ll + (((size_t)(kb & 1) * nWG + member) * RG_NEX + t) * 2;
            const u64 bits = (u64)__double_as_longlong(v), tg = (u64)(unsigned)kb << 32;
            gll_put(dst, tg | (bits & 0xffffffffull), local);
            gll_put(dst + 1, tg | (bits >> 32), local);
        }
        RSTAMP(5);
        hCur[0] = hNext[0]; hCur[1] = hNext[1];
    }
#undef RSTAMP
}

__global__ void __launch_bounds__(64) reg_contract_selftest_kernel(const cplx* __restrict__ t, const cplx* __restrict__ g, double* __restrict__ out) {
    const int lane = threadIdx.x, x = lane & 3;
    cplx E[RG_NUL], O[RG_NUL], ts[2];
#pragma unroll
    for (int i = 0; i < RG_NUL; ++i) {
        const int d = 16 * rg_slot_set(i, x) + (lane >> 2), u = rg_slot_unit(i, x);
        E[i] = ldc(g + (d * 18 + u) * 2);
        O[i] = ldc(g + (d * 18 + u) * 2 + 1);
    }
#pragma unroll
    for (int s = 0; s < 2; ++s) ts[s] = ldc(t + (16 * s + (lane >> 2)) * 2 + (x >> 1));
    rg_contract<RG_NUL>(E, O, ts, lane, true, out);
}

__global__ void __launch_bounds__(64) store_args_kernel(HalfSweepMulti m, HalfSweepArgs* dst) {
    const int nw = (int)(sizeof(HalfSweepArgs) / 8);
    for (int j = 0; j < m.n; ++j) {
        const unsigned long long* src = reinterpret_cast<const unsigned long long*>(&m.a[j]);
        unsigned long long* d = reinterpret_cast<unsigned long long*>(dst + j);
        for (int i = threadIdx.x; i < nw; i += 64) d[i] = src[i];
    }
}
static_assert(sizeof(HalfSweepArgs) % 8 == 0, "argument block in whole words");

size_t reg_dyn_bytes(int nul, int nw) {
    const size_t nu2 = 2 * (size_t)nul, nvw = 8 * nu2;
    return sizeof(cplx) * ((size_t)2 * SY_NORD + PS_CMAX * RG_MLD + 4 * nu2) +
           sizeof(double) * (2 * RG_NEX + (size_t)nw * nvw + (size_t)nul * 64 * nw);
}
constexpr int RG_WAVES[] = {4, 6, 8, 10, 12};
const void* reg_kernel_ptr(int nw) {
    switch (nw) {
        case 4: return reinterpret_cast<const void*>(sweep_reg_kernel<RG_NUL, 4>);
        case 6: return reinterpret_cast<const void*>(sweep_reg_kernel<RG_NUL, 6>);
        case 8: return reinterpret_cast<const void*>(sweep_reg_kernel<RG_NUL, 8>);
        case 10: return reinterpret_cast<const void*>(sweep_reg_kernel<RG_NUL, 10>);
        default: return reinterpret_cast<const void*>(sweep_reg_kernel<RG_NUL, 12>);
    }
}
void reg_set_attributes() {
    static PerDeviceOnce attr_once;
    if (attr_once.first())
        for (int nw : RG_WAVES) HIP_CHECK(hipFuncSetAttribute(reg_kernel_ptr(nw), hipFuncAttributeMaxDynamicSharedMemorySize, 150 * 1024));
}
int reg_nwg(int D, int nw) { return (int)ceil_div(D, 32 * nw); }
int reg_occupancy(int nw) {
    static std::mutex mu;
    static std::map<std::pair<int, int>, int> cache;
    int dev = 0;
    HIP_CHECK(hipGetDevice(&dev));
    std::lock_guard<std::mutex> lk(mu);
    auto it = cache.find({dev, nw});
    if (it != cache.end()) return it->second;
    reg_set_attributes();
    int nb = 0;
    if (hipOccupancyMaxActiveBlocksPerMultiprocessor(&nb, reg_kernel_ptr(nw), 64 * nw, reg_dyn_bytes(RG_NUL, nw)) != hipSuccess) { (void)hipGetLastError(); nb = 0; }
    cache[{dev, nw}] = nb;
    return nb;
}
int reg_wg_cost(int nw) { return nw == 4 ? 1 : 3; }

}

int reg_sweep_max_units() { return 2 * RG_NUL; }
bool reg_sweep_supported(int D, int nmics, int nunits, int nOrd) {
    return nmics >= 2 && nmics <= PS_CMAX && nunits >= 1 && nunits <= 2 * RG_NUL && D >= 1 && reg_nwg(D, 12) <= 32 && nOrd <= SY_NORD;
}
size_t reg_sweep_ll_bytes(int D, int nmics) {
    const size_t nwg = (size_t)reg_nwg(D, 4);
    (void)nmics;
    return sizeof(u64) * ((size_t)2 * nwg * RG_NEX * 2 + nwg + 64);
}
int reg_sweep_slots_per_xcd() { return 3 * (sweep_cu_budget() / 8); }
int reg_sweep_pick_waves(int D, int ndesigns) {
    if (ndesigns < 1 || ndesigns > REG_SWEEP_MAX) return 0;
    const int nsub = (int)ceil_div(ndesigns, 8), cus = sweep_cu_budget() / 8;
    if (const int nw = sw_int<Sw::REG_WAVES>()) {
        if ((nw == 4 || nw == 6 || nw == 8 || nw == 10 || nw == 12) && nsub * reg_nwg(D, nw) * reg_wg_cost(nw) <= 3 * cus && reg_occupancy(nw) >= (nw == 4 ? 3 : 1)) return nw;
    }
    for (int nw : RG_WAVES) if (nsub * reg_nwg(D, nw) <= cus && reg_occupancy(nw) >= 1) return nw;
    return (nsub * reg_nwg(D, 4) <= 3 * cus && reg_occupancy(4) >= 3) ? 4 : 0;
}
int reg_sweep_spread_waves(int D, int ndesigns) {
    const int mode = sw_int<Sw::REG_SPREAD>();
    if (mode == 0 || ndesigns < 1 || ndesigns > REG_SWEEP_MAX || sw_int<Sw::REG_WAVES>() != 0) return 0;
    const int cus = sweep_cu_budget(), local = reg_sweep_pick_waves(D, ndesigns);
    for (int nw : RG_WAVES)
        if (ndesigns * reg_nwg(D, nw) <= cus && reg_occupancy(nw) >= 1) return (mode == 1 || local == 0 || nw < local) ? nw : 0;
    return 0;
}
int reg_sweep_gate_cost(int D, int ndesigns) {
    if (const int ns = reg_sweep_spread_waves(D, ndesigns)) return (int)ceil_div((int64_t)ndesigns * reg_nwg(D, ns), 8) * reg_wg_cost(ns);
    const int nw = reg_sweep_pick_waves(D, ndesigns);
    return nw ? (int)ceil_div(ndesigns, 8) * reg_nwg(D, nw) * reg_wg_cost(nw) : 0;
}
int reg_sweep_capacity(int D) {
    int n = 0;
    for (int k = 8; k <= REG_SWEEP_MAX; k += 8) if (reg_sweep_pick_waves(D, k)) n = k;
    return n;
}
bool reg_sweep_fits(int D, int nmics, int nunits, int nOrd, int ndesigns) {
    return reg_sweep_supported(D, nmics, nunits, nOrd) && reg_sweep_pick_waves(D, ndesigns) != 0;
}

void launch_sweep_reg(const HalfSweepArgs* args_dev, const HalfSweepArgs& a0, int n, hipStream_t st) {
    const int ns = reg_sweep_spread_waves(a0.D, n);
    const int nw = ns ? ns : reg_sweep_pick_waves(a0.D, n);
    if (!nw) throw Error(2, "register-resident sweep: the launch cannot be resident");
    const int nWG = reg_nwg(a0.D, nw), spread = ns ? 1 : 0;
    const unsigned nblocks = spread ? (unsigned)(n * nWG) : 8u * (unsigned)nWG * (unsigned)ceil_div(n, 8);
    const size_t dyn = reg_dyn_bytes(RG_NUL, nw);
    reg_set_attributes();
    const int prio = sw_int<Sw::REG_PRIO>();
    switch (nw) {
        case 4: sweep_reg_kernel<RG_NUL, 4><<<dim3(nblocks), 256, dyn, st>>>(args_dev, n, nWG, spread, prio); break;
        case 6: sweep_reg_kernel<RG_NUL, 6><<<dim3(nblocks), 384, dyn, st>>>(args_dev, n, nWG, spread, prio); break;
        case 8: sweep_reg_kernel<RG_NUL, 8><<<dim3(nblocks), 512, dyn, st>>>(args_dev, n, nWG, spread, prio); break;
        case 10: sweep_reg_kernel<RG_NUL, 10><<<dim3(nblocks), 640, dyn, st>>>(args_dev, n, nWG, spread, prio); break;
        default: sweep_reg_kernel<RG_NUL, 12><<<dim3(nblocks), 768, dyn, st>>>(args_dev, n, nWG, spread, prio); break;
    }
    KERNEL_CHECK();
}

double reg_contract_selftest() {
    constexpr int ND = 32, NU = 2 * RG_NUL, NO = 8 * NU;
    cplx h_t[ND * 2], h_g[ND * NU * 2];
    double h_out[NO], want[NO] = {0};
    unsigned long long x = 88172645463325252ull;
    auto rnd = [&] { x ^= x << 13; x ^= x >> 7; x ^= x << 17; return (double)(x % 2000001ull) / 1000000.0 - 1.0; };
    for (cplx& v : h_t) { v.x = rnd(); v.y = rnd(); }
    for (cplx& v : h_g) { v.x = rnd(); v.y = rnd(); }
    for (int d = 0; d < ND; ++d)
        for (int u = 0; u < NU; ++u)
            for (int eo = 0; eo < 2; ++eo)
                for (int e = 0; e < 2; ++e) {
                    const cplx tv = h_t[d * 2 + e], gv = h_g[(d * NU + u) * 2 + eo];
                    want[8 * u + 4 * eo + 2 * e] += tv.x * gv.x + tv.y * gv.y;
                    want[8 * u + 4 * eo + 2 * e + 1] += tv.y * gv.x - tv.x * gv.y;
                }
    DevMem m_t(sizeof h_t), m_g(sizeof h_g), m_out(sizeof h_out);
    cplx *d_t = m_t.get<cplx>(), *d_g = m_g.get<cplx>();
    double* d_out = m_out.get<double>();
    HIP_CHECK(hipMemcpy(d_t, h_t, sizeof h_t, hipMemcpyHostToDevice));
    HIP_CHECK(hipMemcpy(d_g, h_g, sizeof h_g, hipMemcpyHostToDevice));
    HIP_CHECK(hipMemset(d_out, 0, sizeof h_out));
    reg_contract_selftest_kernel<<<1, 64>>>(d_t, d_g, d_out);
    KERNEL_CHECK();
    HIP_CHECK(hipMemcpy(h_out, d_out, sizeof h_out, hipMemcpyDeviceToHost));
    double err = 0.0;
    for (int i = 0; i < NO; ++i) err = std::max(err, std::fabs(h_out[i] - want[i]));
    return err;
}

void store_sweep_args(const HalfSweepArgs* host, int n, HalfSweepArgs* dev, hipStream_t st) {
    for (int first = 0; first < n; first += SWEEP_MULTI_MAX) {
        HalfSweepMulti m{};
        m.n = std::min(SWEEP_MULTI_MAX, n - first);
        for (int j = 0; j < m.n; ++j) m.a[j] = host[first + j];
        store_args_kernel<<<1, 64, 0, st>>>(m, dev + first);
        KERNEL_CHECK();
    }
}

}
```

emagls_amd/csrc/switches.hpp:

```cpp
#pragma once
#include <climits>
#include <cmath>

namespace emagls {

#define EMAGLS_SWITCHES(X) \
    X(PLAN_CACHE,        INT,  4,     0, INT_MAX,   PROCESS, "shapes the one-shot entry points keep alive (0 = off)") \
    X(BATCH_MAX,         INT,  8,     1, 32,        PROCESS, "initial limit of designs per batch, read at load time (emagls_set_batch_max changes it at run time; the job scheduler sets it per chunk)") \
    X(BATCH_GROUPS,      INT,  2,     1, 4,         CALL,    "lane groups of a batch of more than 8 designs before its sweep (1 = one launch sequence)") \
    X(BATCH_LANES,       ON0,  1,     0, 1,         CALL,    "=0: batches in stream mode (per-plan pipelines) instead of lane mode") \
    X(DEBUG_LANES,       ON1,  0,     0, 1,         CALL,    "=1: why a batch was refused lane mode or common routes, on stderr") \
    X(STAGGER,           ON0,  1,     0, 1,         PROCESS, "=0: both lane groups of a batch issue the stages before the sweep in one order (default: complementary orders)") \
    X(DEFER_HH,          INT,  1,     0, 2,         PROCESS, "the orthonormal route of the low bins next to the sweep: 0 never, 1 batches and designs that have the device to themselves, 2 every lane batch") \
    X(GEO_KEEP,          ON0,  1,     0, 1,         PROCESS, "=0: sharing batches run their geometry stages on every execute") \
    X(GEO_LS_SHARED,     ON0,  1,     0, 1,         CALL,    "=0: sharing batches carry every HRIR set's least-squares rows through the factors instead of one kept Y_reg_inv per bin") \
    X(GRAM_LDS,          ON0,  1,     0, 1,         PROCESS, "=0: lane batches take the K-split Gram kernel + reduce instead of the LDS-staged one") \
    X(GRAM_MFMA4,        ON1,  0,     0, 1,         CALL,    "=1: the Gram tile on the 4 x 4 x 4 MFMA shape (measured slower; the tests' second form)") \
    X(XCD_RUNS,          ON0,  1,     0, 1,         PROCESS, "=0: gram_lds, gemm_tn_f64, synth_ls take their tiles in dispatch order instead of XCD-aware runs") \
    X(GRAM_ROUTE,        ON0,  1,     0, 1,         CALL,    "=0: no Gram route (all bins Householder + Jacobi)") \
    X(GRAM_COND_EST,     REAL, 3e3,   -HUGE_VAL, HUGE_VAL, CALL, "conditioning estimate below which the Gram route starts (the device check stays at 3e4)") \
    X(JACOBI_RUN,        INT,  0,     1, INT_MAX,   PROCESS, "bins per Jacobi workgroup on the Gram route (0: single bins where the stages are forked, runs of 2 in lane groups)") \
    X(REAL_INTERNAL,     ON0,  1,     0, 1,         CALL,    "=0: complex-basis eMagLS / eMagLS2 designs on the complex-arithmetic pipeline") \
    X(NO_GRAPH,          ON1,  0,     0, 1,         CALL,    "=1: eager launches instead of hipGraph replay (plans and batches, when they are created)") \
    X(STREAMS,           INT,  0,     1, 4,         CALL,    "streams of a single plan (0: one, until emagls_plan_set_streams)") \
    X(ONESHOT_STREAMS,   INT,  1,     1, 3,         CALL,    "streams of the one-shot plans of array designs") \
    X(SWEEP_PERSIST,     ON0,  1,     0, 1,         CALL,    "=0: launch-per-bin sweep instead of the persistent one") \
    X(PERSIST_GLOBAL,    ON1,  0,     0, 1,         CALL,    "=1: write-through granules even when a design sits on one XCD") \
    X(SWEEP_SYNTH,       ON0,  1,     0, 1,         CALL,    "=0: array designs on materialised operands instead of the synthesising sweep (when a plan is created)") \
    X(SWEEP_TWIN,        ON0,  1,     0, 1,         CALL,    "=0: launches of 9-16 designs as two independent workgroups per CU instead of twin workgroups") \
    X(SWEEP_REG,         INT,  1,     0, 2,         CALL,    "register-resident sweep: 0 never (the slab form), 1 for launches of more than 8 designs, 2 always") \
    X(REG_WAVES,         INT,  0,     INT_MIN, INT_MAX, CALL, "waves per workgroup of the register-resident sweep (4, 6, 8, 10, 12 whenever it fits; 0: the smallest count with which every workgroup owns a CU)") \
    X(REG_SPREAD,        INT,  2,     0, 2,         CALL,    "a launch's designs spread over all XCDs: 0 never, 1 whenever it fits, 2 when it needs fewer waves per workgroup than the one-XCD layout") \
    X(REG_PRIO,          INT,  1,     INT_MIN, INT_MAX, PROCESS, "=0: the register-resident sweep's waves at the default issue priority") \
    X(SWEEP_FETCH,       INT,  0,     0, 4,         PROCESS, "where the persistent sweep requests the next bin's operands") \
    X(SWEEP_WAIT_MS,     INT,  20,    1, INT_MAX,   PROCESS, "wall-clock limit of a wait for peers inside a resident sweep, in ms") \
    X(SWEEP_TIMING,      ON1,  0,     0, 1,         CALL,    "=1: in-kernel wall-clock stamps of the persistent sweep (when a plan is created)") \
    X(CU_BUDGET,         INT,  0,     0, INT_MAX,   CALL,    "CUs the resident sweeps may count on when their residency is decided (0: the device's)") \
    X(SYNTH_PAIRS,       ON0,  1,     0, 1,         PROCESS, "=0: synthesising sweep without antipodal microphone pairs") \
    X(SYNTH_SPLIT,       INT,  67,    INT_MIN, INT_MAX, PROCESS, "synthesising sweep: per cent of the producers' unit groups evaluated before barrier B1") \
    X(SYNTH_PRIO,        INT,  5,     0, 5,         PROCESS, "synthesising sweep: issue priorities (5: the chains of the two designs of an XCD tilted against the age order; 0: all chains 3, producers 0)") \
    X(STREAM_POOL,       ON0,  1,     0, 1,         PROCESS, "=0: destroy streams instead of recycling them (exposes a HIP runtime crash in long sessions)") \
    X(STREAM_WARM,       INT,  8,     0, INT_MAX,   PROCESS, "streams the pool parks before it hands the first one out") \
    X(POOL_GB,           INT,  128,   0, INT_MAX,   PROCESS, "device memory the block pool keeps for the next plans and arenas, in GB") \
    X(JOBS_FORK,         INT,  3,     1, 4,         PROCESS, "job scheduler: streams of a job list that is a single chunk (1 = lane groups as for chunks in flight)") \
    X(JOBS_RESIDENT,     INT,  0,     0, INT_MAX,   CALL,    "job scheduler: designs whose plans and batches stay resident between calls (0: max(256, 2 x batch x in flight))") \
    X(JOBS_AUTO_SHARE,   ON0,  1,     0, 1,         PROCESS, "=0: job scheduler shares no geometry unless the caller asks") \
    X(JOBS_TRACE,        ON1,  0,     0, 1,         PROCESS, "=1: time stamps of every chunk's steps and of block pool misses on stderr") \
    X(HRIR_FFT_WAVE,     ON0,  1,     0, 1,         CALL,    "=0: the HRIR prologue at nfft = 1024 on the LDS radix-2^2 transform instead of wave-private transforms") \
    X(HRIR_FFT_LDS_KB,   INT,  0,     40, 158,      CALL,    "LDS budget of the LDS-form HRIR transform's sub-tiles (0: 83, 110 at nfft = 2048)") \
    X(DECODE_FUSED,      ON0,  1,     0, 1,         CALL,    "=0: binauralDecode on the hipFFT passes for every filter length") \
    X(DECODE_REGFFT,     ON0,  1,     0, 1,         CALL,    "=0: the fused decode kernel on LDS transform passes also up to 512 taps") \
    X(DECODE_WAVE,       ON0,  1,     0, 1,         CALL,    "=0: the half-wave two-factor decode form also at 257-512 taps") \
    X(DECODE_FILTER_FFT, ONH,  0,     0, 1,         CALL,    "=hipfft: the filter side of the decode's wave form through hipFFT") \
    X(WA_REG,            ON0,  1,     0, 1,         CALL,    "=0: the 33-64-channel path's Householder kernels walk the columns through L2") \
    X(WA_TALL,           ON0,  1,     0, 1,         CALL,    "=0: the plain Householder kernels for problems of more than 448 rows instead of the LDS-reflector forms") \
    X(WA_YRI_MFMA,       ON0,  1,     0, 1,         CALL,    "=0: the 33-64-channel path's Y_reg_inv_k product on the vector pipe") \
    X(WA_JACOBI_FLAG,    REAL, 1e-14, -HUGE_VAL, HUGE_VAL, PROCESS, "the 33-64-channel path's Jacobi: another sweep follows one in which some rotation had |gamma| > x sqrt(alpha beta)") \
    X(WA_LEAF_ROWS,      INT,  0,     INT_MIN, INT_MAX, PROCESS, "tiled QR: upper bound of the leaf height, 1024 .. 4096 (anything else: 3072)")

enum class Sw : int {
#define X(name, kind, def, lo, hi, when, doc) name,
    EMAGLS_SWITCHES(X)
#undef X
    COUNT
};
enum class SwKind { ON0, ON1, ONH, INT, REAL };
constexpr SwKind sw_kind(Sw s) {
    constexpr SwKind kinds[] = {
#define X(name, kind, def, lo, hi, when, doc) SwKind::kind,
        EMAGLS_SWITCHES(X)
#undef X
    };
    return kinds[(int)s];
}

double sw_value(Sw s);

template <Sw S> inline bool sw_on() {
    static_assert(sw_kind(S) == SwKind::ON0 || sw_kind(S) == SwKind::ON1 || sw_kind(S) == SwKind::ONH, "not a flag");
    return sw_value(S) != 0.0;
}
template <Sw S> inline int sw_int() { static_assert(sw_kind(S) == SwKind::INT, "not an integer switch"); return (int)sw_value(S); }
template <Sw S> inline double sw_real() { static_assert(sw_kind(S) == SwKind::REAL, "not a real switch"); return sw_value(S); }

}
```

emagls_amd/plan.py:

```python
from __future__ import annotations

import ctypes as C

import numpy as np

from . import _lib as L


class Plan:
    def __init__(self, kind, basis="real", order=4, fs=48000.0, length=512, nsamp=128, ndirs=0, mic_radius=0.0, nmics=0,
                 f_trans=0.0, atf_taps=0, natf=0, custom_basis=False, diffuseness=False, sim_order_pad=0):
        self._lib = L.load()
        self.desc = L.DesignDesc(kind, L.BASIS[basis], order, fs, length, nsamp, ndirs, mic_radius, nmics, f_trans,
                                 atf_taps, natf, 1 if custom_basis else 0, 1 if diffuseness else 0, int(sim_order_pad))
        self._cplx = basis == "complex"
        self._h = C.c_void_p()
        L.check(self._lib.emagls_plan_create(C.byref(self.desc), C.byref(self._h)))
        self._keep = []

    def close(self):
        if self._h:
            self._lib.emagls_plan_destroy(self._h)
            self._h = C.c_void_p()

    def __del__(self):
        try:
            self.close()
        except Exception:
            pass

    def _p(self, a):
        a = np.asfortranarray(np.asarray(a, dtype=np.float64))
        self._keep.append(a)
        return a.ctypes.data_as(C.c_void_p)

    def set_hrir_grid(self, azi, zen):
        L.check(self._lib.emagls_plan_set_hrir_grid(self._h, self._p(azi), self._p(zen)))

    def set_mic_grid(self, azi, zen=None):
        L.check(self._lib.emagls_plan_set_mic_grid(self._h, self._p(azi), self._p(zen) if zen is not None else None))

    def set_basis(self, Y_hrir, Y_mic=None):
        dt = np.complex128 if self._cplx else np.float64

        def ptr(a):
            a = np.asfortranarray(np.asarray(a, dtype=dt))
            self._keep.append(a)
            return a.ctypes.data_as(C.c_void_p)
        L.check(self._lib.emagls_plan_set_basis(self._h, ptr(Y_hrir), ptr(Y_mic) if Y_mic is not None else None))

    def set_hrirs(self, hL, hR):
        L.check(self._lib.emagls_plan_set_hrirs(self._h, self._p(hL), self._p(hR)))

    def set_atfs(self, atf, azi, zen):
        L.check(self._lib.emagls_plan_set_atfs(self._h, self._p(atf), self._p(azi), self._p(zen)))

    def execute(self):
        L.check(self._lib.emagls_plan_execute(self._h))

    def synchronize(self):
        L.check(self._lib.emagls_plan_synchronize(self._h))

    def info(self):
        i = L.PlanInfo()
        L.check(self._lib.emagls_plan_get_info(self._h, C.byref(i)))
        return i

    def get_filters(self):
        i = self.info()
        dt = np.complex128 if i.out_is_complex else np.float64
        wL = np.zeros((i.out_rows, i.out_cols), dtype=dt, order="F")
        wR = np.zeros((i.out_rows, i.out_cols), dtype=dt, order="F")
        L.check(self._lib.emagls_plan_get_filters(self._h, wL.ctypes.data_as(C.c_void_p), wR.ctypes.data_as(C.c_void_p)))
        return wL, wR

    def set_profiling(self, level):
        L.check(self._lib.emagls_plan_set_profiling(self._h, int(level)))

    def set_streams(self, n):
        L.check(self._lib.emagls_plan_set_streams(self._h, int(n)))

    def stage_times(self):
        n = self._lib.emagls_plan_num_stages(self._h)
        ms = (C.c_double * max(n, 1))()
        L.check(self._lib.emagls_plan_stage_times(self._h, ms, n))
        return [(self._lib.emagls_plan_stage_name(self._h, i).decode(), ms[i]) for i in range(1, n)]

    def sweep_kernel_time(self):
        tot = C.c_double(0.0)
        n = C.c_int(0)
        L.check(self._lib.emagls_plan_sweep_kernel_time(self._h, C.byref(tot), C.byref(n)))
        return tot.value, n.value

    def debug(self, name, dtype, shape=None):
        nb = C.c_size_t(0)
        L.check(self._lib.emagls_plan_debug_buffer(self._h, name.encode(), None, C.byref(nb)))
        buf = np.empty(nb.value // np.dtype(dtype).itemsize, dtype=dtype)
        nb2 = C.c_size_t(buf.nbytes)
        L.check(self._lib.emagls_plan_debug_buffer(self._h, name.encode(), buf.ctypes.data_as(C.c_void_p), C.byref(nb2)))
        return buf.reshape(shape) if shape is not None else buf

    @property
    def stream(self):
        return self._lib.emagls_plan_stream(self._h)


class Batch:

    def __init__(self, plans):
        self._lib = L.load()
        self.plans = list(plans)
        arr = (C.c_void_p * len(self.plans))(*[p._h for p in self.plans])
        self._h = C.c_void_p()
        L.check(self._lib.emagls_batch_create(arr, len(self.plans), C.byref(self._h)))

    def execute(self):
        L.check(self._lib.emagls_batch_execute(self._h))

    def synchronize(self):
        L.check(self._lib.emagls_batch_synchronize(self._h))

    def get_filters(self):
        outs = []
        i = self.plans[0].info()
        dt = np.complex128 if i.out_is_complex else np.float64
        for p in self.plans:
            outs.append((np.zeros((i.out_rows, i.out_cols), dtype=dt, order="F"), np.zeros((i.out_rows, i.out_cols), dtype=dt, order="F")))
        n = len(self.plans)
        pl = (C.c_void_p * n)(*[o[0].ctypes.data for o in outs])
        pr = (C.c_void_p * n)(*[o[1].ctypes.data for o in outs])
        L.check(self._lib.emagls_batch_get_filters(self._h, pl, pr))
        return outs

    def set_profiling(self, level):
        L.check(self._lib.emagls_batch_set_profiling(self._h, int(level)))

    def lane_mode(self):
        v = C.c_int(0)
        L.check(self._lib.emagls_batch_lane_mode(self._h, C.byref(v)))
        return bool(v.value)

    def set_stream(self, hip_stream):
        L.check(self._lib.emagls_batch_set_stream(self._h, C.c_void_p(int(hip_stream))))

    def shares_atf_side(self):
        v = C.c_int(0)
        L.check(self._lib.emagls_batch_shares_atf_side(self._h, C.byref(v)))
        return bool(v.value)

    def share_geometry(self, enable=True):
        L.check(self._lib.emagls_batch_set_geometry_sharing(self._h, int(bool(enable))))

    def shares_geometry(self):
        v = C.c_int(0)
        L.check(self._lib.emagls_batch_shares_geometry(self._h, C.byref(v)))
        return bool(v.value)

    def geometry_runs(self):
        cold, warm = C.c_longlong(0), C.c_longlong(0)
        L.check(self._lib.emagls_batch_geometry_runs(self._h, C.byref(cold), C.byref(warm)))
        return cold.value, warm.value

    def set_streams(self, n):
        L.check(self._lib.emagls_batch_set_streams(self._h, int(n)))

    def set_stage_order(self, order):
        L.check(self._lib.emagls_batch_set_stage_order(self._h, int(order)))

    def set_side_stream(self, hip_stream):
        L.check(self._lib.emagls_batch_set_side_stream(self._h, C.c_void_p(int(hip_stream))))

    def sweep_time_ms(self):
        ms = C.c_double(0.0)
        L.check(self._lib.emagls_batch_sweep_time(self._h, C.byref(ms)))
        return ms.value

    def get_filters_into(self, ptrs_l, ptrs_r):
        n = len(self.plans)
        pl = (C.c_void_p * n)(*ptrs_l)
        pr = (C.c_void_p * n)(*ptrs_r)
        L.check(self._lib.emagls_batch_get_filters(self._h, pl, pr))

    def close(self):
        if self._h:
            self._lib.emagls_batch_destroy(self._h)
            self._h = C.c_void_p()

    def __del__(self):
        try:
            self.close()
        except Exception:
            pass
```

include/emagls.h:

```cpp
#ifndef EMAGLS_H
#define EMAGLS_H

#include <stddef.h>
#include <stdint.h>

#ifdef __cplusplus
extern "C" {
#endif

#define EMAGLS_OK 0
#define EMAGLS_ERR_ARG 1
#define EMAGLS_ERR_UNSUPPORTED 2
#define EMAGLS_ERR_HIP 3
#define EMAGLS_ERR_NUMERIC 4

#define EMAGLS_BASIS_REAL 0
#define EMAGLS_BASIS_COMPLEX 1

#define EMAGLS_KIND_LS 0
#define EMAGLS_KIND_MAGLS 1
#define EMAGLS_KIND_EMAGLS 2
#define EMAGLS_KIND_EMAGLS2 3
#define EMAGLS_KIND_FROM_ATF 4
#define EMAGLS_KIND_EMA_CH 5
// ... 297 lines not shown
                     void* out);
int emagls_array_irs_kernel_time(double* ms);

int emagls_array_irs_spectral(double fs, double mic_radius, int order, const double* mic_azi, const double* mic_zen, int64_t nmics,
                              const void* enc, int enc_is_complex, int64_t nch, int64_t nsrc, const int64_t* comp_ptr, const double* comp_azi,
                              const double* comp_zen, const double* comp_delay, const double* comp_gain, int64_t nsurf,
                              const double* surf_refl, const int32_t* comp_exp, const double* air_atten, const double* comp_path,
                              double pre_delay, int64_t nfft, int64_t nr, void* out);

int emagls_shoebox_components(const double* room_dim, const double* wall_refl, const double* array_pos, int64_t nsrc, const double* src_pos,
                              double fs, double max_delay, int max_order, int64_t capacity, int64_t* comp_ptr, double* comp_azi,
                              double* comp_zen, double* comp_delay, double* comp_gain);
int emagls_array_room_irs(double fs, double mic_radius, int order, const double* mic_azi, const double* mic_zen, int64_t nmics,
                          const void* enc, int enc_is_complex, int64_t nch, const double* room_dim, const double* wall_refl,
                          const double* array_pos, int64_t nsrc, const double* src_pos, double max_delay, int max_order, double pre_delay,
                          int64_t nfft, int64_t nr, int64_t* comp_count, void* out);
int emagls_shoebox_images(const double* room_dim, const double* array_pos, int64_t nsrc, const double* src_pos, double fs, double max_delay,
                          int max_order, int64_t capacity, int64_t* comp_ptr, double* comp_azi, double* comp_zen, double* comp_delay,
                          double* comp_gain, int32_t* comp_exp, double* comp_path);
int emagls_array_room_irs_spectral(double fs, double mic_radius, int order, const double* mic_azi, const double* mic_zen, int64_t nmics,
                                   const void* enc, int enc_is_complex, int64_t nch, const double* room_dim, const double* wall_refl_spec,
                                   const double* air_atten, const double* array_pos, int64_t nsrc, const double* src_pos, double max_delay,
                                   int max_order, double pre_delay, int64_t nfft, int64_t nr, int64_t* comp_count, void* out);
int emagls_shoebox_kernel_time(double* ms);

int emagls_array_irs_point(double fs, double mic_radius, int order, const double* mic_azi, const double* mic_zen, int64_t nmics,
                           const void* enc, int enc_is_complex, int64_t nch, int64_t nsrc, const int64_t* comp_ptr, const double* comp_azi,
                           const double* comp_zen, const double* comp_delay, const double* comp_gain, int64_t nsurf,
                           const double* surf_refl, const int32_t* comp_exp, const double* air_atten, const double* comp_path,
                           const double* comp_dist, double pre_delay, int64_t nfft, int64_t nr, void* out);
int emagls_shoebox_components_dist(const double* room_dim, const double* wall_refl, const double* array_pos, int64_t nsrc,
                                   const double* src_pos, double fs, double max_delay, int max_order, int64_t capacity, int64_t* comp_ptr,
                                   double* comp_azi, double* comp_zen, double* comp_delay, double* comp_gain, double* comp_dist);
int emagls_array_room_irs_point(double fs, double mic_radius, int order, const double* mic_azi, const double* mic_zen, int64_t nmics,
                                const void* enc, int enc_is_complex, int64_t nch, const double* room_dim, const double* wall_refl,
                                int wall_is_spectral, const double* air_atten, const double* array_pos, int64_t nsrc, const double* src_pos,
                                double max_delay, int max_order, double pre_delay, int64_t nfft, int64_t nr, int64_t* comp_count, void* out);

int emagls_array_irs_directive(double fs, double mic_radius, int order, const double* mic_azi, const double* mic_zen, int64_t nmics,
                               const void* enc, int enc_is_complex, int64_t nch, int64_t nsrc, const int64_t* comp_ptr, const double* comp_azi,
                               const double* comp_zen, const double* comp_delay, const double* comp_gain, int64_t nsurf,
                               const double* surf_refl, const int32_t* comp_exp, const double* air_atten, const double* comp_path,
                               const double* comp_dist, const double* comp_emit, const double* src_rot, int dir_order, const double* dir_coef,
                               double pre_delay, int64_t nfft, int64_t nr, void* out);
int emagls_shoebox_emission(const double* room_dim, const double* wall_refl, const double* array_pos, int64_t nsrc, const double* src_pos,
                            double fs, double max_delay, int max_order, int64_t capacity, int64_t* comp_ptr, double* comp_emit);
int emagls_array_room_irs_directive(double fs, double mic_radius, int order, const double* mic_azi, const double* mic_zen, int64_t nmics,
                                    const void* enc, int enc_is_complex, int64_t nch, const double* room_dim, const double* wall_refl,
                                    int wall_is_spectral, const double* air_atten, const double* array_pos, int64_t nsrc, const double* src_pos,
                                    double max_delay, int max_order, int point_source, const double* src_rot, int dir_order,
                                    const double* dir_coef, double pre_delay, int64_t nfft, int64_t nr, int64_t* comp_count, void* out);


typedef struct emagls_plan emagls_plan;

typedef struct emagls_design_desc {
    int kind;
    int basis;
    int order;
    double fs;
    int64_t len;
    int64_t nsamp;
    int64_t ndirs;
    double mic_radius;
    int64_t nmics;
    double f_trans;
    int64_t atf_taps;
    int64_t natf;
    int custom_basis;
    int diffuseness;
    int sim_order_pad;
} emagls_design_desc;

typedef struct emagls_plan_info {
    int nfft, num_pos_freqs, k_cut , sim_order, num_sh_sim, num_channels;
    int out_is_complex;
    int64_t out_rows, out_cols;
    double grp_delay_l, grp_delay_r;
    double mean_grid_dev_deg;
    int num_sweep_launches;
    int64_t device_bytes;
    int gram_from, hh_end, hh_orders, g_first;
    int sim_order_own;
    int sweep_form, sweep_units;
} emagls_plan_info;

int emagls_plan_create(const emagls_design_desc* desc, emagls_plan** plan);
int emagls_plan_destroy(emagls_plan* plan);
int emagls_plan_set_hrir_grid(emagls_plan* plan, const double* azi, const double* zen);
int emagls_plan_set_mic_grid(emagls_plan* plan, const double* azi, const double* zen);
int emagls_plan_set_hrirs(emagls_plan* plan, const double* hL, const double* hR);
int emagls_plan_set_basis(emagls_plan* plan, const void* Y_hrir, const void* Y_mic);
int emagls_plan_set_atfs(emagls_plan* plan, const double* atf_irs, const double* atf_azi, const double* atf_zen);
int emagls_plan_execute(emagls_plan* plan);
int emagls_plan_synchronize(emagls_plan* plan);
int emagls_plan_get_filters(emagls_plan* plan, void* wL, void* wR);
int emagls_plan_get_info(emagls_plan* plan, emagls_plan_info* info);
int emagls_plan_sweep_form_in_batch(emagls_plan* plan, int designs, int* form);
int emagls_plan_set_streams(emagls_plan* plan, int nstreams);
int emagls_plan_set_profiling(emagls_plan* plan, int level);
int emagls_plan_num_stages(emagls_plan* plan);
const char* emagls_plan_stage_name(emagls_plan* plan, int stage);
int emagls_plan_stage_times(emagls_plan* plan, double* ms, int n);
int emagls_plan_sweep_kernel_time(emagls_plan* plan, double* total_ms, int* launches);
int emagls_plan_debug_buffer(emagls_plan* plan, const char* name, void* dst, size_t* nbytes);
void* emagls_plan_stream(emagls_plan* plan);

typedef struct emagls_batch emagls_batch;
int emagls_batch_create(emagls_plan** plans, int nplans, emagls_batch** batch);
int emagls_set_batch_max(int max_designs, int* previous);
int emagls_batch_set_geometry_sharing(emagls_batch* batch, int enable);
int emagls_batch_shares_geometry(emagls_batch* batch, int* shared);
int emagls_batch_geometry_runs(emagls_batch* batch, long long* cold, long long* warm);
typedef struct emagls_job {
    emagls_design_desc desc;
    const double* hL;
    const double* hR;
    const double* hrir_azi;
    const double* hrir_zen;
    const double* mic_azi;
    const double* mic_zen;
    const double* atf;
    const double* atf_azi;
    const double* atf_zen;
    void* wL;
    void* wR;
} emagls_job;
#define EMAGLS_JOBS_SHARE_GEOMETRY 1
#define EMAGLS_JOBS_INDEPENDENT 2
int emagls_jobs_run(const emagls_job* jobs, int64_t njobs, int batch_size, int in_flight, int flags);
int emagls_jobs_shard(const emagls_job* jobs, int64_t njobs, int world, int max_batch, int* rank_of_job, int* order_in_rank, int* sim_order_pad);
int emagls_jobs_run_devices(const emagls_job* jobs, int64_t njobs, const int* devices, int ndevices, int batch_size, int in_flight, int flags);
int emagls_design_out_shape(const emagls_design_desc* desc, int64_t* rows, int64_t* cols, int* is_complex);
int emagls_jobs_set_profiling(int level);
int emagls_jobs_sweep_times(double* ms, int* designs, int capacity, int* count);
int emagls_jobs_geometry_runs(long long* independent, long long* cold, long long* warm);
int emagls_jobs_would_share_geometry(const emagls_job* jobs, int njobs, int* share);

int emagls_design_hrir_sets(int kind, const double* hL, const double* hR, int64_t nsamp, int64_t ndirs, int64_t nsets,
                            const double* hrir_azi, const double* hrir_zen, double mic_radius, const double* mic_azi, const double* mic_zen,
                            int64_t nmics, int order, double fs, int64_t len, int basis, void* wL, void* wR);
int emagls_from_atf_hrir_sets(const double* hL, const double* hR, int64_t nsamp, int64_t ndirs, int64_t nsets, const double* hrir_azi,
                              const double* hrir_zen, const double* atf_irs, int64_t atf_taps, int64_t nmics, int64_t natf, const double* atf_azi,
                              const double* atf_zen, double fs, int64_t filter_len, double f_trans, double* wL, double* wR, double* mean_dev);
int emagls_batch_shares_atf_side(emagls_batch* batch, int* shared);
int emagls_batch_execute(emagls_batch* batch);
int emagls_batch_synchronize(emagls_batch* batch);
int emagls_batch_get_filters(emagls_batch* batch, void* const* wL, void* const* wR);
int emagls_batch_set_profiling(emagls_batch* batch, int level);
int emagls_batch_lane_mode(emagls_batch* batch, int* lanes);
int emagls_batch_set_stream(emagls_batch* batch, void* hip_stream);
int emagls_batch_set_side_stream(emagls_batch* batch, void* hip_stream);
int emagls_batch_sweep_time(emagls_batch* batch, double* ms);
int emagls_batch_set_streams(emagls_batch* batch, int nstreams);
int emagls_batch_set_stage_order(emagls_batch* batch, int order);
int emagls_batch_destroy(emagls_batch* batch);

#ifdef __cplusplus
}
#endif
#endif
```

Measured before the change: 4256 filter sets/s.

## Group several geometry-sharing HRIR sets per workgroup in register-resident sweep

```diff
diff --git a/emagls_amd/_lib.py b/emagls_amd/_lib.py
--- a/emagls_amd/_lib.py
+++ b/emagls_amd/_lib.py
@@ -288,6 +288,8 @@
     "emagls_batch_set_streams": (C.c_int, [C.c_void_p, C.c_int]),
     "emagls_batch_set_stage_order": (C.c_int, [C.c_void_p, C.c_int]),
     "emagls_batch_sweep_time": (C.c_int, [C.c_void_p, C.POINTER(C.c_double)]),
+    "emagls_batch_sweep_layout": (C.c_int, [C.c_void_p, C.POINTER(C.c_int), C.POINTER(C.c_int), C.POINTER(C.c_int)]),
+    "emagls_reg_sweep_layout": (C.c_int, [C.c_int, C.c_int, C.c_int, C.POINTER(C.c_int), C.POINTER(C.c_int), C.POINTER(C.c_int), C.POINTER(C.c_int)]),
     "emagls_batch_destroy": (C.c_int, [C.c_void_p]),
 }
 
diff --git a/emagls_amd/csrc/batch_run.hip b/emagls_amd/csrc/batch_run.hip
--- a/emagls_amd/csrc/batch_run.hip
+++ b/emagls_amd/csrc/batch_run.hip
@@ -27,7 +27,7 @@
     if (q0.sweep_persist) {
         hipStream_t ss = b.stream;
         {
-            SweepGate gate(ss, reg ? reg_sweep_gate_cost((int)q0.D, nb) : 0);
+            SweepGate gate(ss, reg ? reg_sweep_gate_cost((int)q0.D, nb, b.geo_share) : 0);
             if (b.lanes) { BatchScope sc(nb, b.stride); launch_zero(q0.get("ll"), q0.bufs["ll"].bytes, ss); }
             else for (auto* q : b.plans) launch_zero(q->get("ll"), q->bufs["ll"].bytes, ss);
             if (reg) {
@@ -35,7 +35,7 @@
                 reg_args_upload(ha.data(), nb, b.sweep_args_dev.get(), b.sweep_args_last, ss);
             }
             if (b.prof_level >= 1) HIP_CHECK(hipEventRecord(b.sweep_ev[0], ss));
-            if (reg) launch_sweep_reg(b.sweep_args_dev.get<const HalfSweepArgs>(), ha[0], nb, ss);
+            if (reg) b.sweep_layout = launch_sweep_reg(b.sweep_args_dev.get<const HalfSweepArgs>(), ha[0], nb, b.geo_share, ss);
             else if (q0.synth) launch_sweep_synth(h, ss); else launch_sweep_persist(h, ss);
             if (b.prof_level >= 1) HIP_CHECK(hipEventRecord(b.sweep_ev[1], ss));
         }
diff --git a/emagls_amd/csrc/capi.hip b/emagls_amd/csrc/capi.hip
--- a/emagls_amd/csrc/capi.hip
+++ b/emagls_amd/csrc/capi.hip
@@ -649,6 +649,24 @@
         *shared = b->geo_share ? 1 : 0;
     });
 }
+int emagls_batch_sweep_layout(emagls_batch* b, int* waves, int* sets_per_workgroup, int* workgroups) {
+    return guarded([&] {
+        if (!b || !waves || !sets_per_workgroup || !workgroups) throw Error(EMAGLS_ERR_ARG, "null pointer");
+        const emagls::RegSweepLayout& L = b->sweep_layout;
+        const int n = (int)b->plans.size();
+        *waves = L.nw;
+        *sets_per_workgroup = L.nw ? L.g : 0;
+        *workgroups = !L.nw ? 0 : L.spread ? n * L.nwg : (int)((n + L.g - 1) / L.g) * L.nwg;
+    });
+}
+int emagls_reg_sweep_layout(int directions, int designs, int share, int* waves, int* sets_per_workgroup, int* workgroups_per_group, int* spread) {
+    return guarded([&] {
+        if (!waves || !sets_per_workgroup || !workgroups_per_group || !spread) throw Error(EMAGLS_ERR_ARG, "null pointer");
+        if (directions < 1 || designs < 1 || designs > REG_SWEEP_MAX) throw Error(EMAGLS_ERR_ARG, "emagls_reg_sweep_layout: directions < 1 or designs outside 1..32");
+        const emagls::RegSweepLayout L = emagls::reg_sweep_layout(directions, designs, share != 0);
+        *waves = L.nw; *sets_per_workgroup = L.nw ? L.g : 0; *workgroups_per_group = L.nwg; *spread = L.spread;
+    });
+}
 int emagls_batch_shares_atf_side(emagls_batch* b, int* shared) {
     return guarded([&] {
         if (!b || !shared) throw Error(EMAGLS_ERR_ARG, "null pointer");
diff --git a/emagls_amd/csrc/host_internal.hpp b/emagls_amd/csrc/host_internal.hpp
--- a/emagls_amd/csrc/host_internal.hpp
+++ b/emagls_amd/csrc/host_internal.hpp
@@ -384,6 +384,7 @@
     bool use_graph = true;
     emagls::DevMem sweep_args_dev;
     std::vector<char> sweep_args_last;
+    emagls::RegSweepLayout sweep_layout{0, 0, 0, 0};
     std::vector<hipEvent_t> events;
     size_t used = 0;
     hipEvent_t next_event() {
diff --git a/emagls_amd/csrc/kernels.hpp b/emagls_amd/csrc/kernels.hpp
--- a/emagls_amd/csrc/kernels.hpp
+++ b/emagls_amd/csrc/kernels.hpp
@@ -114,9 +114,11 @@
 int reg_sweep_capacity(int D);
 int reg_sweep_slots_per_xcd();
 int reg_sweep_pick_waves(int D, int ndesigns);
-int reg_sweep_gate_cost(int D, int ndesigns);
+struct RegSweepLayout { int nw, g, nwg, spread; };
+RegSweepLayout reg_sweep_layout(int D, int ndesigns, bool share);
+int reg_sweep_gate_cost(int D, int ndesigns, bool share);
 bool reg_sweep_fits(int D, int nmics, int nunits, int nOrd, int ndesigns);
-void launch_sweep_reg(const HalfSweepArgs* args_dev, const HalfSweepArgs& a0, int n, hipStream_t st);
+RegSweepLayout launch_sweep_reg(const HalfSweepArgs* args_dev, const HalfSweepArgs& a0, int n, bool share, hipStream_t st);
 double reg_contract_selftest();
 double gram_tile_selftest(bool four);
 void store_sweep_args(const HalfSweepArgs* host, int n, HalfSweepArgs* dev, hipStream_t st);
diff --git a/emagls_amd/csrc/plan_run.hip b/emagls_amd/csrc/plan_run.hip
--- a/emagls_amd/csrc/plan_run.hip
+++ b/emagls_amd/csrc/plan_run.hip
@@ -77,11 +77,11 @@
     if (k0 < p.P && p.sweep_persist) {
         emagls_plan* self = &p;
         p.reg_sweep = reg_sweep_wanted(&self, 1);
-        SweepGate gate(s0, p.reg_sweep ? reg_sweep_gate_cost((int)p.D, 1) : 0);
+        SweepGate gate(s0, p.reg_sweep ? reg_sweep_gate_cost((int)p.D, 1, false) : 0);
         launch_zero(p.get("ll"), p.bufs["ll"].bytes, s0);
         if (p.reg_sweep) reg_args_upload(&m.a[0], 1, p.get("sweep_args"), p.sweep_args_last, s0);
         if (p.prof_level >= 2) record_sweep_event(p, 0);
-        if (p.reg_sweep) launch_sweep_reg(p.get<HalfSweepArgs>("sweep_args"), m.a[0], 1, s0);
+        if (p.reg_sweep) launch_sweep_reg(p.get<HalfSweepArgs>("sweep_args"), m.a[0], 1, false, s0);
         else if (p.synth) launch_sweep_synth(m, s0); else launch_sweep_persist(m, s0);
         if (p.prof_level >= 2) record_sweep_event(p, 1);
         p.sweep_launches = 1;
diff --git a/emagls_amd/csrc/sweep_reg.hip b/emagls_amd/csrc/sweep_reg.hip
--- a/emagls_amd/csrc/sweep_reg.hip
+++ b/emagls_amd/csrc/sweep_reg.hip
@@ -5,6 +5,7 @@
 #include <algorithm>
 #include <map>
 #include <mutex>
+#include <tuple>
 
 namespace emagls {
 
@@ -122,62 +123,85 @@
 }
 constexpr int RG_NUL = 9;
 constexpr int RG_NEX = 4 * PS_CMAX;
+constexpr int RG_GROUP_DEFAULT = 4;
 constexpr int RG_SVC = 256;
 
-template <int NUL, int NW>
-__global__ void __launch_bounds__(64 * NW) __attribute__((amdgpu_waves_per_eu(3))) sweep_reg_kernel(const HalfSweepArgs* __restrict__ args, int n, int nWG, int spread, int prio) {
+template <int NUL, int NW, int G>
+__device__ __forceinline__ void sweep_reg_body(const HalfSweepArgs* __restrict__ args, int n, int nWG, int spread, int prio) {
     constexpr int NT = 64 * NW, DPW = 32 * NW;
     constexpr int NU2 = 2 * NUL;
     constexpr int NVW = 8 * NU2;
     constexpr int GA = (NUL + 1) / 2, GB = NUL - GA;
+    constexpr int NSL = G == 1 ? 1 : NT / RG_SVC;
+    constexpr int SPT = G / NSL;
+    constexpr int SETD = 8 * NU2 + 2 * RG_NEX + NW * NVW;
     static_assert(GB >= 1 && NW % 2 == 0 && NT >= RG_SVC, "layout");
+    static_assert(NSL * SPT == G && RG_NEX * G <= NT && SETD % 2 == 0, "sets of a group over the service slices");
     extern __shared__ __attribute__((aligned(16))) char dyn[];
     cplx* ring = reinterpret_cast<cplx*>(dyn);
     cplx* ms = ring + 2 * SY_NORD;
-    cplx* WE = ms + PS_CMAX * RG_MLD;
-    cplx* WO = WE + 2 * NU2;
-    double* vt = reinterpret_cast<double*>(WO + 2 * NU2);
-    double* wpart = vt + 2 * RG_NEX;
-    double* xs = wpart + NW * NVW;
+    double* sets = reinterpret_cast<double*>(ms + PS_CMAX * RG_MLD);
+    auto WEs = [&](int s) __attribute__((always_inline)) { return reinterpret_cast<cplx*>(sets + s * SETD); };
+    auto WOs = [&](int s) __attribute__((always_inline)) { return WEs(s) + 2 * NU2; };
+    auto vts = [&](int s) __attribute__((always_inline)) { return reinterpret_cast<double*>(WOs(s) + 2 * NU2); };
+    auto wparts = [&](int s) __attribute__((always_inline)) { return vts(s) + 2 * RG_NEX; };
+    double* xs = sets + G * SETD;
     __shared__ int s_abort, s_local;
 
-    int design, member;
+    int group, member;
     if (spread) {
-        design = (int)blockIdx.x / nWG;
-        member = (int)blockIdx.x - design * nWG;
+        group = (int)blockIdx.x / nWG;
+        member = (int)blockIdx.x - group * nWG;
     } else {
         const int xcd = blockIdx.x & 7, rest = blockIdx.x >> 3;
         const int sub = rest / nWG;
         member = rest - sub * nWG;
-        design = xcd + 8 * sub;
-    }
-    if (design >= n) return;
+        group = xcd + 8 * sub;
+    }
+    const int set0 = G * group;
+    if (set0 >= n) return;
     if (prio) __builtin_amdgcn_s_setprio(3);
-    const HalfSweepArgs& a = args[design];
+    const HalfSweepArgs& a = args[set0];
+    auto arg = [&](int s) __attribute__((always_inline)) -> const HalfSweepArgs& { return args[(G == 1 || set0 + s < n) ? set0 + s : n - 1]; };
     const int tid = threadIdx.x;
     const int C = a.C, P = a.P, D = a.D, kfirst = a.kfirst, kabs0 = a.kabs0;
     const int64_t ldH = a.ldH;
     const int nord_pad = a.nord_pad;
-    const gcd_t Habs = RG_GLOBAL(const double, a.Habs);
     const gcc_t Mw = RG_GLOBAL(const cplx, a.Mw);
     const gcc_t bsc = RG_GLOBAL(const cplx, a.bsc);
-    const gcd_t Winit = RG_GLOBAL(const double, a.Winit);
-    cplx __attribute__((address_space(1)))* const Uout = RG_GLOBAL(cplx, a.U);
-    long long* const timing = a.timing;
+    long long* const timing = (G == 1 || group == 0) ? a.timing : nullptr;
     int* const abort_flag = a.abort_flag;
     const long long wait_ticks = a.wait_ticks;
     const int* smap = a.smap;
     const int npr = smap[32], nsg = smap[33], nun = npr + nsg;
-    const gu64_t part_ll = RG_GLOBAL(u64, a.ll);
-    const gu64_t xcc_ll = part_ll + (size_t)2 * nWG * RG_NEX * 2;
+    const gu64_t xcc_ll = RG_GLOBAL(u64, a.ll) + (size_t)2 * nWG * RG_NEX * 2;
+    const int sl = G == 1 ? 0 : __builtin_amdgcn_readfirstlane(tid / RG_SVC);
+    gu64_t sv_ll[SPT];
+    gcd_t sv_Winit[SPT];
+    cplx __attribute__((address_space(1)))* sv_U[SPT];
+    bool sv_live[SPT];
+#pragma unroll
+    for (int q = 0; q < SPT; ++q) {
+        const HalfSweepArgs& as = arg(sl + NSL * q);
+        sv_ll[q] = RG_GLOBAL(u64, as.ll);
+        sv_Winit[q] = RG_GLOBAL(const double, as.Winit);
+        sv_U[q] = RG_GLOBAL(cplx, as.U);
+        sv_live[q] = G == 1 || set0 + sl + NSL * q < n;
+    }
+    const int pub = G == 1 ? 0 : __builtin_amdgcn_readfirstlane(tid / RG_NEX) % G;
+    const gu64_t pub_ll = RG_GLOBAL(u64, arg(pub).ll);
+    const bool pub_live = G == 1 || set0 + pub < n;
+    auto raise_all = [&]() __attribute__((always_inline)) {
+        if (G > 1 && tid < G && set0 + tid < n) __hip_atomic_store(args[set0 + tid].abort_flag, 1, __ATOMIC_RELAXED, __HIP_MEMORY_SCOPE_AGENT);
+    };
     if (tid == 0) { s_abort = 0; s_local = 0; }
     const int d0 = member * DPW;
     auto dir_of = [&](int t, int s) __attribute__((always_inline)) { return d0 + 32 * (t >> 6) + 16 * s + ((t & 63) >> 2); };
 
     {
-        const size_t ncplx = (size_t)2 * SY_NORD + PS_CMAX * RG_MLD + 4 * NU2;
+        const size_t ncplx = (size_t)2 * SY_NORD + PS_CMAX * RG_MLD;
         for (size_t i = tid; i < ncplx; i += NT) ring[i] = mk(0, 0);
-        for (int i = tid; i < 2 * RG_NEX + NW * NVW; i += NT) vt[i] = 0.0;
+        for (int i = tid; i < G * SETD; i += NT) sets[i] = 0.0;
         double sd[2], cd[2], daz[2];
 #pragma unroll
         for (int s = 0; s < 2; ++s) {
@@ -218,13 +242,18 @@
 #pragma unroll
         for (int i = 0; i < NLM; ++i) ms[r * RG_MLD + c0 + i] = (r < C && c0 + i < C) ? mReg[i] : mk(0, 0);
     };
-    double hCur[2], hNext[2] = {0.0, 0.0};
-    auto fetch_h = [&](int kb, double (&h)[2], int t) __attribute__((always_inline)) {
+    double hCur[G][2], hNext[G][2];
+    auto fetch_h = [&](int kb, double (&h)[G][2], int t) __attribute__((always_inline)) {
         const int kbg = (kb < P ? kb : P - 1) - kabs0;
-        const gcd_t He = Habs + ((int64_t)((t >> 1) & 1) * (P - kabs0) + kbg) * ldH;
-#pragma unroll
-        for (int s = 0; s < 2; ++s) h[s] = He[dir_of(t, s) < D ? dir_of(t, s) : D - 1];
+#pragma unroll
+        for (int g = 0; g < G; ++g) {
+            const gcd_t He = RG_GLOBAL(const double, arg(g).Habs) + ((int64_t)((t >> 1) & 1) * (P - kabs0) + kbg) * ldH;
+#pragma unroll
+            for (int s = 0; s < 2; ++s) h[g][s] = He[dir_of(t, s) < D ? dir_of(t, s) : D - 1];
+        }
     };
+#pragma unroll
+    for (int g = 0; g < G; ++g) { hNext[g][0] = 0.0; hNext[g][1] = 0.0; }
     fetch_h(kfirst, hCur, tid);
     if (tid < RG_SVC) { fetch_m(kfirst, tid); stage_m(tid); }
 
@@ -251,7 +280,7 @@
     }
     __syncthreads();
     const bool local = s_local != 0;
-    if (s_abort) return;
+    if (s_abort) { raise_all(); return; }
 
     const bool slot8 = nun > 16 || GB < 2;
     cplx E[NUL], O[NUL];
@@ -274,66 +303,84 @@
             __builtin_amdgcn_sched_barrier(0);
         }
         RSTAMP(0);
-        if (launder(tid) < RG_SVC) {
+        if (launder(tid) < RG_SVC * NSL) {
             const int t = launder(tid);
-            const int j = t & (RG_NEX - 1), half = t >> 7;
+            const int sv = G == 1 ? t : t & (RG_SVC - 1);
+            const int j = sv & (RG_NEX - 1), half = sv >> 7;
             if (first) {
-                vt[t] = half == 0 ? Winit[j] : 0.0;
+#pragma unroll
+                for (int q = 0; q < SPT; ++q) vts(sl + NSL * q)[sv] = half == 0 ? sv_Winit[q][j] : 0.0;
             } else {
                 const unsigned tag = (unsigned)(kb - 1);
-                const gu64_t src = part_ll + ((size_t)((kb - 1) & 1) * nWG * RG_NEX + j) * 2;
-                double sum = 0.0;
+                const size_t off = ((size_t)((kb - 1) & 1) * nWG * RG_NEX + j) * 2;
+                double sum[SPT];
                 const bool alive = ll_wait([&] {
                     bool ok = true;
-                    double s = 0.0;
+                    double s[SPT];
+#pragma unroll
+                    for (int q = 0; q < SPT; ++q) s[q] = 0.0;
                     for (int base = half; base < nWG; base += 2 * RG_POLL) {
-                        u32x4_t g[RG_POLL];
-#pragma unroll
-                        for (int i = 0; i < RG_POLL; ++i) {
-                            const int w = base + 2 * i < nWG ? base + 2 * i : half;
-                            gll_load16_async(g[i], src + (size_t)w * RG_NEX * 2);
-                        }
-                        rg_wait_loads(g);
-#pragma unroll
-                        for (int i = 0; i < RG_POLL; ++i) {
-                            ok = ok && g[i].y == tag && g[i].w == tag;
-                            if (base + 2 * i < nWG) s += __hiloint2double((int)g[i].z, (int)g[i].x);
-                        }
+                        u32x4_t g[SPT][RG_POLL];
+#pragma unroll
+                        for (int q = 0; q < SPT; ++q)
+#pragma unroll
+                            for (int i = 0; i < RG_POLL; ++i) {
+                                const int w = base + 2 * i < nWG ? base + 2 * i : half;
+                                gll_load16_async(g[q][i], sv_ll[q] + off + (size_t)w * RG_NEX * 2);
+                            }
+#pragma unroll
+                        for (int q = 0; q < SPT; ++q) rg_wait_loads(g[q]);
+#pragma unroll
+                        for (int q = 0; q < SPT; ++q)
+#pragma unroll
+                            for (int i = 0; i < RG_POLL; ++i) {
+                                ok = ok && g[q][i].y == tag && g[q][i].w == tag;
+                                if (base + 2 * i < nWG) s[q] += __hiloint2double((int)g[q][i].z, (int)g[q][i].x);
+                            }
                     }
-                    sum = s;
+#pragma unroll
+                    for (int q = 0; q < SPT; ++q) sum[q] = s[q];
                     return ok;
                 }, abort_flag, wait_ticks);
-                vt[t] = sum;
+#pragma unroll
+                for (int q = 0; q < SPT; ++q) vts(sl + NSL * q)[sv] = sum[q];
                 if (!alive && (t & 63) == 0) s_abort = 1;
             }
         }
         RSTAMP(2);
         __syncthreads();
         if (s_abort) break;
-        if (launder(tid) < RG_SVC) {
+        if (launder(tid) < RG_SVC * NSL) {
             const int t = launder(tid);
-            const int part = t & 3, pair = t >> 2, e = pair >> 5, c = pair & 31;
-            const cplx* vc = reinterpret_cast<const cplx*>(vt) + e * PS_CMAX;
-            cplx acc = mk(0, 0);
-            if (first) {
-                if (part == 0) acc = vc[c];
-            } else {
-#pragma unroll
-                for (int i = 0; i < PS_CMAX / 4; ++i)
-                    cfma(acc, vc[part + 4 * i] + vc[RG_NEX / 2 + part + 4 * i], conj(ms[(part + 4 * i) * RG_MLD + c]));
-            }
-            acc = group_sum<4>(acc);
-            const cplx other = shfl_xor_c(acc, 4);
-            if (part == 0 && c < C) {
-                if (c < 2 * npr) {
-                    if ((c & 1) == 0) { WE[e * NU2 + (c >> 1)] = acc + other; WO[e * NU2 + (c >> 1)] = acc - other; }
+            const int sv = G == 1 ? t : t & (RG_SVC - 1);
+            const int part = sv & 3, pair = sv >> 2, e = pair >> 5, c = pair & 31;
+#pragma unroll
+            for (int q = 0; q < SPT; ++q) {
+                const int set = sl + NSL * q;
+                const cplx* vc = reinterpret_cast<const cplx*>(vts(set)) + e * PS_CMAX;
+                cplx* WE = WEs(set);
+                cplx* WO = WOs(set);
+                cplx acc = mk(0, 0);
+                if (first) {
+                    if (part == 0) acc = vc[c];
                 } else {
-                    WE[e * NU2 + npr + (c - 2 * npr)] = acc; WO[e * NU2 + npr + (c - 2 * npr)] = acc;
+#pragma unroll
+                    for (int i = 0; i < PS_CMAX / 4; ++i)
+                        cfma(acc, vc[part + 4 * i] + vc[RG_NEX / 2 + part + 4 * i], conj(ms[(part + 4 * i) * RG_MLD + c]));
                 }
-                if (member == 0 && !first) {
-                    cplx __attribute__((address_space(1)))* dst = Uout + ((int64_t)e * P + (kb - 1)) * PS_CMAX + c;
-                    const cplx v = vc[c] + vc[RG_NEX / 2 + c];
-                    dst->x = v.x; dst->y = v.y;
+                acc = group_sum<4>(acc);
+                const cplx other = shfl_xor_c(acc, 4);
+                if (part == 0 && c < C) {
+                    if (c < 2 * npr) {
+                        if ((c & 1) == 0) { WE[e * NU2 + (c >> 1)] = acc + other; WO[e * NU2 + (c >> 1)] = acc - other; }
+                    } else {
+                        WE[e * NU2 + npr + (c - 2 * npr)] = acc; WO[e * NU2 + npr + (c - 2 * npr)] = acc;
+                    }
+                    if (member == 0 && !first && sv_live[q]) {
+                        cplx __attribute__((address_space(1)))* dst = sv_U[q] + ((int64_t)e * P + (kb - 1)) * PS_CMAX + c;
+                        const cplx v = vc[c] + vc[RG_NEX / 2 + c];
+                        dst->x = v.x; dst->y = v.y;
+                    }
                 }
             }
         }
@@ -342,46 +389,54 @@
         RSTAMP(3);
         const bool svc = launder(tid) < RG_SVC;
         if (svc) fetch_m(kb, launder(tid));
-        cplx ts[2];
+        cplx ts[G][2];
         {
             const int t = launder(tid);
             const int x = t & 3;
-            cplx p[2][2];
-#pragma unroll
-            for (int s = 0; s < 2; ++s) { p[s][0] = mk(0, 0); p[s][1] = mk(0, 0); }
-#pragma unroll
-            for (int r = 0; r < 4; ++r) {
-                const int u = 4 * r + x;
-                const cplx we0 = WE[u], wo0 = WO[u], we1 = WE[NU2 + u], wo1 = WO[NU2 + u];
-#pragma unroll
-                for (int s = 0; s < 2; ++s) {
-                    cfma(p[s][0], we0, E[4 * s + r]); cfma(p[s][0], wo0, O[4 * s + r]);
-                    cfma(p[s][1], we1, E[4 * s + r]); cfma(p[s][1], wo1, O[4 * s + r]);
+            cplx p[G][2][2];
+#pragma unroll
+            for (int g = 0; g < G; ++g) {
+                const cplx* WE = WEs(g);
+                const cplx* WO = WOs(g);
+#pragma unroll
+                for (int s = 0; s < 2; ++s) { p[g][s][0] = mk(0, 0); p[g][s][1] = mk(0, 0); }
+#pragma unroll
+                for (int r = 0; r < 4; ++r) {
+                    const int u = 4 * r + x;
+                    const cplx we0 = WE[u], wo0 = WO[u], we1 = WE[NU2 + u], wo1 = WO[NU2 + u];
+#pragma unroll
+                    for (int s = 0; s < 2; ++s) {
+                        cfma(p[g][s][0], we0, E[4 * s + r]); cfma(p[g][s][0], wo0, O[4 * s + r]);
+                        cfma(p[g][s][1], we1, E[4 * s + r]); cfma(p[g][s][1], wo1, O[4 * s + r]);
+                    }
                 }
-            }
-            if (slot8) {
-                const int u = 16 + (x & 1);
-                cplx q0 = mk(0, 0), q1 = mk(0, 0);
-                cfma(q0, WE[u], E[8]); cfma(q0, WO[u], O[8]);
-                cfma(q1, WE[NU2 + u], E[8]); cfma(q1, WO[NU2 + u], O[8]);
-                const bool s1 = (x & 2) != 0;
-                const cplx z = mk(0, 0);
-                p[0][0] = p[0][0] + (s1 ? z : q0); p[0][1] = p[0][1] + (s1 ? z : q1);
-                p[1][0] = p[1][0] + (s1 ? q0 : z); p[1][1] = p[1][1] + (s1 ? q1 : z);
+                if (slot8) {
+                    const int u = 16 + (x & 1);
+                    cplx q0 = mk(0, 0), q1 = mk(0, 0);
+                    cfma(q0, WE[u], E[8]); cfma(q0, WO[u], O[8]);
+                    cfma(q1, WE[NU2 + u], E[8]); cfma(q1, WO[NU2 + u], O[8]);
+                    const bool s1 = (x & 2) != 0;
+                    const cplx z = mk(0, 0);
+                    p[g][0][0] = p[g][0][0] + (s1 ? z : q0); p[g][0][1] = p[g][0][1] + (s1 ? z : q1);
+                    p[g][1][0] = p[g][1][0] + (s1 ? q0 : z); p[g][1][1] = p[g][1][1] + (s1 ? q1 : z);
+                }
             }
             if (svc) stage_m(t);
             RSTAMP(8);
 #pragma unroll
-            for (int s = 0; s < 2; ++s) {
-                const cplx pe0 = group_sum<4>(p[s][0]), pe1 = group_sum<4>(p[s][1]);
-                const cplx pe = (x & 2) ? pe1 : pe0;
-                ts[s] = dir_of(t, s) < D ? unit_phase(hCur[s], pe, nyq) : mk(0, 0);
-            }
+            for (int g = 0; g < G; ++g)
+#pragma unroll
+                for (int s = 0; s < 2; ++s) {
+                    const cplx pe0 = group_sum<4>(p[g][s][0]), pe1 = group_sum<4>(p[g][s][1]);
+                    const cplx pe = (x & 2) ? pe1 : pe0;
+                    ts[g][s] = dir_of(t, s) < D ? unit_phase(hCur[g][s], pe, nyq) : mk(0, 0);
+                }
         }
         __builtin_amdgcn_sched_barrier(0);
         {
             const int t = launder(tid);
-            rg_contract<NUL>(E, O, ts, t & 63, slot8, wpart + (t >> 6) * NVW);
+#pragma unroll
+            for (int g = 0; g < G; ++g) rg_contract<NUL>(E, O, ts[g], t & 63, slot8, wparts(g) + (t >> 6) * NVW);
         }
         {
             const int t = launder(tid);
@@ -390,28 +445,41 @@
         }
         __syncthreads();
         RSTAMP(4);
-        if (launder(tid) < RG_NEX) {
-            const int t = launder(tid);
+        if (launder(tid) < RG_NEX * G) {
+            const int t = G == 1 ? launder(tid) : launder(tid) & (RG_NEX - 1);
             const int xe = t >> 6, xr = (t >> 1) & 31, xri = t & 1;
             double v = 0.0;
             if (xr < C) {
                 const int xu = xr < 2 * npr ? (xr >> 1) : npr + (xr - 2 * npr);
                 const bool xneg = xr < 2 * npr && (xr & 1);
-                const double* wE = wpart + 8 * xu + 2 * xe + xri;
+                const double* wE = wparts(pub) + 8 * xu + 2 * xe + xri;
                 double sE = 0.0, sO = 0.0;
 #pragma unroll
                 for (int w = 0; w < NW; ++w) { sE += wE[w * NVW]; sO += wE[w * NVW + 4]; }
                 v = xneg ? sE - sO : sE + sO;
             }
-            const gu64_t dst = part_ll + (((size_t)(kb & 1) * nWG + member) * RG_NEX + t) * 2;
-            const u64 bits = (u64)__double_as_longlong(v), tg = (u64)(unsigned)kb << 32;
-            gll_put(dst, tg | (bits & 0xffffffffull), local);
-            gll_put(dst + 1, tg | (bits >> 32), local);
+            if (pub_live) {
+                const gu64_t dst = pub_ll + (((size_t)(kb & 1) * nWG + member) * RG_NEX + t) * 2;
+                const u64 bits = (u64)__double_as_longlong(v), tg = (u64)(unsigned)kb << 32;
+                gll_put(dst, tg | (bits & 0xffffffffull), local);
+                gll_put(dst + 1, tg | (bits >> 32), local);
+            }
         }
         RSTAMP(5);
-        hCur[0] = hNext[0]; hCur[1] = hNext[1];
+#pragma unroll
+        for (int g = 0; g < G; ++g) { hCur[g][0] = hNext[g][0]; hCur[g][1] = hNext[g][1]; }
     }
 #undef RSTAMP
+    if (s_abort) raise_all();
+}
+
+template <int NUL, int NW>
+__global__ void __launch_bounds__(64 * NW) __attribute__((amdgpu_waves_per_eu(3))) sweep_reg_kernel(const HalfSweepArgs* __restrict__ args, int n, int nWG, int spread, int prio) {
+    sweep_reg_body<NUL, NW, 1>(args, n, nWG, spread, prio);
+}
+template <int NUL, int NW, int G>
+__global__ void __launch_bounds__(64 * NW) __attribute__((amdgpu_waves_per_eu(2))) sweep_reg_group_kernel(const HalfSweepArgs* __restrict__ args, int n, int nWG, int spread, int prio) {
+    sweep_reg_body<NUL, NW, G>(args, n, nWG, spread, prio);
 }
 
 __global__ void __launch_bounds__(64) reg_contract_selftest_kernel(const cplx* __restrict__ t, const cplx* __restrict__ g, double* __restrict__ out) {
@@ -438,13 +506,17 @@
 }
 static_assert(sizeof(HalfSweepArgs) % 8 == 0, "argument block in whole words");
 
-size_t reg_dyn_bytes(int nul, int nw) {
+size_t reg_dyn_bytes(int nul, int nw, int g = 1) {
     const size_t nu2 = 2 * (size_t)nul, nvw = 8 * nu2;
-    return sizeof(cplx) * ((size_t)2 * SY_NORD + PS_CMAX * RG_MLD + 4 * nu2) +
-           sizeof(double) * (2 * RG_NEX + (size_t)nw * nvw + (size_t)nul * 64 * nw);
+    return sizeof(cplx) * ((size_t)2 * SY_NORD + PS_CMAX * RG_MLD + (size_t)g * 4 * nu2) +
+           sizeof(double) * ((size_t)g * (2 * RG_NEX + (size_t)nw * nvw) + (size_t)nul * 64 * nw);
 }
 constexpr int RG_WAVES[] = {4, 6, 8, 10, 12};
-const void* reg_kernel_ptr(int nw) {
+constexpr int RG_GROUP_NW = 8;
+constexpr int RG_GROUPS[] = {2, 4};
+const void* reg_kernel_ptr(int nw, int g = 1) {
+    if (g == 2) return reinterpret_cast<const void*>(sweep_reg_group_kernel<RG_NUL, RG_GROUP_NW, 2>);
+    if (g == 4) return reinterpret_cast<const void*>(sweep_reg_group_kernel<RG_NUL, RG_GROUP_NW, 4>);
     switch (nw) {
         case 4: return reinterpret_cast<const void*>(sweep_reg_kernel<RG_NUL, 4>);
         case 6: return reinterpret_cast<const void*>(sweep_reg_kernel<RG_NUL, 6>);
@@ -455,22 +527,24 @@
 }
 void reg_set_attributes() {
     static PerDeviceOnce attr_once;
-    if (attr_once.first())
+    if (attr_once.first()) {
         for (int nw : RG_WAVES) HIP_CHECK(hipFuncSetAttribute(reg_kernel_ptr(nw), hipFuncAttributeMaxDynamicSharedMemorySize, 150 * 1024));
+        for (int g : RG_GROUPS) HIP_CHECK(hipFuncSetAttribute(reg_kernel_ptr(RG_GROUP_NW, g), hipFuncAttributeMaxDynamicSharedMemorySize, 150 * 1024));
+    }
 }
 int reg_nwg(int D, int nw) { return (int)ceil_div(D, 32 * nw); }
-int reg_occupancy(int nw) {
+int reg_occupancy(int nw, int g = 1) {
     static std::mutex mu;
-    static std::map<std::pair<int, int>, int> cache;
+    static std::map<std::tuple<int, int, int>, int> cache;
     int dev = 0;
     HIP_CHECK(hipGetDevice(&dev));
     std::lock_guard<std::mutex> lk(mu);
-    auto it = cache.find({dev, nw});
+    auto it = cache.find({dev, nw, g});
     if (it != cache.end()) return it->second;
     reg_set_attributes();
     int nb = 0;
-    if (hipOccupancyMaxActiveBlocksPerMultiprocessor(&nb, reg_kernel_ptr(nw), 64 * nw, reg_dyn_bytes(RG_NUL, nw)) != hipSuccess) { (void)hipGetLastError(); nb = 0; }
-    cache[{dev, nw}] = nb;
+    if (hipOccupancyMaxActiveBlocksPerMultiprocessor(&nb, reg_kernel_ptr(nw, g), 64 * nw, reg_dyn_bytes(RG_NUL, nw, g)) != hipSuccess) { (void)hipGetLastError(); nb = 0; }
+    cache[{dev, nw, g}] = nb;
     return nb;
 }
 int reg_wg_cost(int nw) { return nw == 4 ? 1 : 3; }
@@ -504,10 +578,28 @@
         if (ndesigns * reg_nwg(D, nw) <= cus && reg_occupancy(nw) >= 1) return (mode == 1 || local == 0 || nw < local) ? nw : 0;
     return 0;
 }
-int reg_sweep_gate_cost(int D, int ndesigns) {
-    if (const int ns = reg_sweep_spread_waves(D, ndesigns)) return (int)ceil_div((int64_t)ndesigns * reg_nwg(D, ns), 8) * reg_wg_cost(ns);
-    const int nw = reg_sweep_pick_waves(D, ndesigns);
-    return nw ? (int)ceil_div(ndesigns, 8) * reg_nwg(D, nw) * reg_wg_cost(nw) : 0;
+RegSweepLayout reg_sweep_layout(int D, int ndesigns, bool share) {
+    RegSweepLayout L{0, 1, 0, 0};
+    const int ns = reg_sweep_spread_waves(D, ndesigns);
+    L.nw = ns ? ns : reg_sweep_pick_waves(D, ndesigns);
+    if (!L.nw) return L;
+    L.spread = ns ? 1 : 0;
+    L.nwg = reg_nwg(D, L.nw);
+    const int mode = sw_int<Sw::REG_GROUP>();
+    int g = 0;
+    if (share && mode == 0 && RG_GROUP_DEFAULT > 1 && !ns && L.nw == 12) g = RG_GROUP_DEFAULT;
+    if (share && (mode == 2 || mode == 4)) g = mode;
+    if (g) {
+        const int nsub = (int)ceil_div((int)ceil_div(ndesigns, g), 8);
+        if (nsub * reg_nwg(D, RG_GROUP_NW) <= sweep_cu_budget() / 8 && reg_occupancy(RG_GROUP_NW, g) >= 1) L = RegSweepLayout{RG_GROUP_NW, g, reg_nwg(D, RG_GROUP_NW), 0};
+    }
+    return L;
+}
+int reg_sweep_gate_cost(int D, int ndesigns, bool share) {
+    const RegSweepLayout L = reg_sweep_layout(D, ndesigns, share);
+    if (!L.nw) return 0;
+    if (L.spread) return (int)ceil_div((int64_t)ndesigns * L.nwg, 8) * reg_wg_cost(L.nw);
+    return (int)ceil_div((int)ceil_div(ndesigns, L.g), 8) * L.nwg * reg_wg_cost(L.nw);
 }
 int reg_sweep_capacity(int D) {
     int n = 0;
@@ -518,16 +610,17 @@
     return reg_sweep_supported(D, nmics, nunits, nOrd) && reg_sweep_pick_waves(D, ndesigns) != 0;
 }
 
-void launch_sweep_reg(const HalfSweepArgs* args_dev, const HalfSweepArgs& a0, int n, hipStream_t st) {
-    const int ns = reg_sweep_spread_waves(a0.D, n);
-    const int nw = ns ? ns : reg_sweep_pick_waves(a0.D, n);
+RegSweepLayout launch_sweep_reg(const HalfSweepArgs* args_dev, const HalfSweepArgs& a0, int n, bool share, hipStream_t st) {
+    const RegSweepLayout L = reg_sweep_layout(a0.D, n, share);
+    const int nw = L.nw, nWG = L.nwg, spread = L.spread;
     if (!nw) throw Error(2, "register-resident sweep: the launch cannot be resident");
-    const int nWG = reg_nwg(a0.D, nw), spread = ns ? 1 : 0;
-    const unsigned nblocks = spread ? (unsigned)(n * nWG) : 8u * (unsigned)nWG * (unsigned)ceil_div(n, 8);
-    const size_t dyn = reg_dyn_bytes(RG_NUL, nw);
+    const unsigned nblocks = spread ? (unsigned)(n * nWG) : 8u * (unsigned)nWG * (unsigned)ceil_div((int)ceil_div(n, L.g), 8);
+    const size_t dyn = reg_dyn_bytes(RG_NUL, nw, L.g);
     reg_set_attributes();
     const int prio = sw_int<Sw::REG_PRIO>();
-    switch (nw) {
+    if (L.g == 2) sweep_reg_group_kernel<RG_NUL, RG_GROUP_NW, 2><<<dim3(nblocks), 64 * RG_GROUP_NW, dyn, st>>>(args_dev, n, nWG, spread, prio);
+    else if (L.g == 4) sweep_reg_group_kernel<RG_NUL, RG_GROUP_NW, 4><<<dim3(nblocks), 64 * RG_GROUP_NW, dyn, st>>>(args_dev, n, nWG, spread, prio);
+    else switch (nw) {
         case 4: sweep_reg_kernel<RG_NUL, 4><<<dim3(nblocks), 256, dyn, st>>>(args_dev, n, nWG, spread, prio); break;
         case 6: sweep_reg_kernel<RG_NUL, 6><<<dim3(nblocks), 384, dyn, st>>>(args_dev, n, nWG, spread, prio); break;
         case 8: sweep_reg_kernel<RG_NUL, 8><<<dim3(nblocks), 512, dyn, st>>>(args_dev, n, nWG, spread, prio); break;
@@ -535,6 +628,7 @@
         default: sweep_reg_kernel<RG_NUL, 12><<<dim3(nblocks), 768, dyn, st>>>(args_dev, n, nWG, spread, prio); break;
     }
     KERNEL_CHECK();
+    return L;
 }
 
 double reg_contract_selftest() {
diff --git a/emagls_amd/csrc/switches.hpp b/emagls_amd/csrc/switches.hpp
--- a/emagls_amd/csrc/switches.hpp
+++ b/emagls_amd/csrc/switches.hpp
@@ -31,6 +31,7 @@
     X(SWEEP_REG,         INT,  1,     0, 2,         CALL,    "register-resident sweep: 0 never (the slab form), 1 for launches of more than 8 designs, 2 always") \
     X(REG_WAVES,         INT,  0,     INT_MIN, INT_MAX, CALL, "waves per workgroup of the register-resident sweep (4, 6, 8, 10, 12 whenever it fits; 0: the smallest count with which every workgroup owns a CU)") \
     X(REG_SPREAD,        INT,  2,     0, 2,         CALL,    "a launch's designs spread over all XCDs: 0 never, 1 whenever it fits, 2 when it needs fewer waves per workgroup than the one-XCD layout") \
+    X(REG_GROUP,         INT,  0,     0, 4,         CALL,    "HRIR sets of one geometry per workgroup of the register-resident sweep (one operand for all of them): 0 four where a launch would need twelve-wave workgroups, 1 never, 2 / 4 that many wherever the designs share a geometry and it fits") \
     X(REG_PRIO,          INT,  1,     INT_MIN, INT_MAX, PROCESS, "=0: the register-resident sweep's waves at the default issue priority") \
     X(SWEEP_FETCH,       INT,  0,     0, 4,         PROCESS, "where the persistent sweep requests the next bin's operands") \
     X(SWEEP_WAIT_MS,     INT,  20,    1, INT_MAX,   PROCESS, "wall-clock limit of a wait for peers inside a resident sweep, in ms") \
diff --git a/emagls_amd/plan.py b/emagls_amd/plan.py
--- a/emagls_amd/plan.py
+++ b/emagls_amd/plan.py
@@ -175,6 +175,11 @@
         L.check(self._lib.emagls_batch_sweep_time(self._h, C.byref(ms)))
         return ms.value
 
+    def sweep_layout(self):
+        nw, g, nwg = C.c_int(0), C.c_int(0), C.c_int(0)
+        L.check(self._lib.emagls_batch_sweep_layout(self._h, C.byref(nw), C.byref(g), C.byref(nwg)))
+        return nw.value, g.value, nwg.value
+
     def get_filters_into(self, ptrs_l, ptrs_r):
         n = len(self.plans)
         pl = (C.c_void_p * n)(*ptrs_l)
diff --git a/include/emagls.h b/include/emagls.h
--- a/include/emagls.h
+++ b/include/emagls.h
@@ -473,6 +473,8 @@
 int emagls_batch_set_stream(emagls_batch* batch, void* hip_stream);
 int emagls_batch_set_side_stream(emagls_batch* batch, void* hip_stream);
 int emagls_batch_sweep_time(emagls_batch* batch, double* ms);
+int emagls_batch_sweep_layout(emagls_batch* batch, int* waves, int* sets_per_workgroup, int* workgroups);
+int emagls_reg_sweep_layout(int directions, int designs, int share, int* waves, int* sets_per_workgroup, int* workgroups_per_group, int* spread);
 int emagls_batch_set_streams(emagls_batch* batch, int nstreams);
 int emagls_batch_set_stage_order(emagls_batch* batch, int order);
 int emagls_batch_destroy(emagls_batch* batch);
```

Result: slower. 4160 filter sets/s (-2.3%).
